# KaranSankla/Lidar_Object_Detection

Hardware: AMD Instinct MI355X
Metric: LiDAR points/sec projected+instance-labelled (higher is better)
Workload: dtype f64

## Files before the change

include/lpf.h:

```cpp
#ifndef LPF_H
#define LPF_H

#include <stddef.h>
#include <stdint.h>

#ifdef __cplusplus
extern "C" {
#endif

#define LPF_MAX_MASKS 32
#define LPF_ABI_VERSION 8
#define LPF_MAX_MASKS_WIDE 256
#define LPF_MAX_CAMS 4

typedef enum lpf_status {
    LPF_OK = 0,
    LPF_ERR_ARG = -1,
    LPF_ERR_HIP = -2,
    LPF_ERR_STATE = -3,
    LPF_ERR_NOMEM = -4,
    LPF_ERR_IO = -5
} lpf_status;

typedef struct lpf_ctx lpf_ctx;
// ... 323 lines not shown
    double  *avg_depth;
    double  *near_bbox2d;
    int32_t *front;
    double  *bbox2d;
    double  *front_avg_depth;
    int32_t *kept_pos;
    int32_t *frame_counts;
    double  *corners_velo;
    int32_t  on_device, reserved;
} lpf_box_views_outputs;
int lpf_box_views(lpf_ctx *ctx, int F, const lpf_box_views_input *in, const lpf_box_views_outputs *out);

int lpf_resize_masks_u8(lpf_ctx *ctx, const uint8_t *src, int n, int h, int w, uint8_t *dst, int on_device);

int lpf_erode_masks_u8(lpf_ctx *ctx, const uint8_t *src, int n, int h, int w, int iters, uint8_t *dst, int on_device);

int lpf_prepare_boxes(lpf_ctx *ctx, const double *corners_cam0, int nbox, const double T_cam_to_velo[16],
                      uint8_t *visible, double *corners_velo, double *bbox2d, int32_t *front);

typedef struct lpf_graph lpf_graph;
int  lpf_graph_begin(lpf_ctx *ctx);
int  lpf_graph_end(lpf_ctx *ctx, lpf_graph **out);
int  lpf_graph_launch(lpf_ctx *ctx, lpf_graph *g);
void lpf_graph_destroy(lpf_graph *g);

int lpf_profile_enable(lpf_ctx *ctx, int on);
int lpf_profile_read(lpf_ctx *ctx, double *k1_ms_sum, int64_t *k1_launches, int reset);
int lpf_profile_overhead(lpf_ctx *ctx, double *empty_bracket_ms);

int lpf_get_stats(lpf_ctx *ctx, int64_t *out, int n, int reset);

int lpf_allreduce_metrics(lpf_ctx *ctx, int64_t *vec, int n, int op, void *rccl_comm);

typedef struct lpf_first_match_input {
    const void   *masks;
    const double *colors;
    int32_t M;
    int32_t mh, mw;
    int32_t f32;
    int32_t on_device;
    int32_t reserved;
} lpf_first_match_input;
typedef struct lpf_first_match_outputs {
    int32_t *first_mask;
    int64_t *car_idx;
    int32_t *car_mask;
    float   *car_xyz;
    double  *car_rgb;
    int64_t *bg_idx;
    float   *bg_xyz;
    int64_t *n_valid, *n_car, *n_bg;
    int64_t *mask_count;
    int32_t  on_device, reserved;
} lpf_first_match_outputs;
int lpf_first_match(lpf_ctx *ctx, const float *pts, const int64_t *frame_off, int F, int pts_on_device,
                    const lpf_first_match_input *in, const lpf_first_match_outputs *out);
typedef struct lpf_first_match_rle_input {
    const lpf_rle_masks *masks;
    const double *colors;
    int32_t mh, mw;
    int32_t colors_on_device;
    int32_t reserved;
} lpf_first_match_rle_input;
int lpf_first_match_rle(lpf_ctx *ctx, const float *pts, const int64_t *frame_off, int F, int pts_on_device,
                        const lpf_first_match_rle_input *in, const lpf_first_match_outputs *out);

typedef struct lpf_reader lpf_reader;
int  lpf_reader_create(lpf_ctx *ctx, lpf_reader **out, int n_buffers, int64_t max_points);
int  lpf_reader_submit(lpf_reader *rd, const char *path);
int  lpf_reader_next(lpf_reader *rd, const float **d_pts, const float **h_pts, int64_t *n_points);
int  lpf_reader_wait(lpf_reader *rd);
void lpf_reader_destroy(lpf_reader *rd);

enum lpf_boxes_state {
    LPF_BOXES_PARSED = 0,
    LPF_BOXES_ABSENT = 1,
    LPF_BOXES_OTHER = 2,
    LPF_BOXES_NONE = 3
};
int  lpf_reader_submit_frame(lpf_reader *rd, const char *scan_path, const char *boxes_path);
int  lpf_reader_boxes(lpf_reader *rd, const double **corners_cam0, const int32_t **index, int *nbox, int *state);
int  lpf_parse_boxes_json(const char *path, double *corners_cam0, int32_t *index, int cap, int *nbox, int *state);

#ifdef __cplusplus
}
#endif
#endif
```

lidar_object_detection_amd/_build.py:

```python
import hashlib
import os
import shutil
import subprocess

_HERE = os.path.dirname(os.path.abspath(__file__))
CSRC = os.path.join(_HERE, "csrc")
LIB = os.path.join(_HERE, "liblpf.so")
LAB_LIB = os.path.join(_HERE, "liblpf_lab.so")
SOURCES = ("lpf_api.hip", "lpf_kernels.hip.h", "lpf_reader.hip.h", "lpf_wide.hip.h", "lpf_cams.hip.h", "lpf_cams_wide.hip.h",
           "lpf_frame_wide.hip.h", "lpf_depth_maps.hip.h", "lpf_depth_overlays.hip.h",
           "lpf_match2d.hip.h", "lpf_inside.hip.h", "lpf_box_points.hip.h", "lpf_box_views.hip.h", "lpf_assign.hip.h",
           "lpf_first_match.hip.h", "lpf_rle.hip.h", "lpf_ids.hip.h")
ARCH = "gfx950"

FLAGS = ["--offload-arch=" + ARCH, "-O3", "-std=c++17", "-fPIC", "-shared", "-pthread", "-ldl",
         "-ffp-contract=off", "-fno-fast-math", "-Wall", "-Wno-unused-function"]


def hipcc():
    exe = shutil.which("hipcc") or "/opt/rocm/bin/hipcc"
    if not os.path.exists(exe):
        raise RuntimeError("hipcc not found (looked on PATH and in /opt/rocm/bin)")
    return exe


HEADER = os.path.join(os.path.dirname(_HERE), "include", "lpf.h")
_MARKER = b"LPF_BUILD_ID="


def source_id(lab=False):
    h = hashlib.sha256()
    for path in [os.path.join(CSRC, s) for s in SOURCES] + [HEADER]:
        with open(path, "rb") as f:
            h.update(os.path.basename(path).encode() + b"\0" + f.read() + b"\0")
    h.update(" ".join(FLAGS + (["-DLPF_LAB"] if lab else [])).encode())
    return h.hexdigest()[:16]


def library_id(lib):
    try:
        with open(lib, "rb") as f:
            data = f.read()
    except OSError:
        return None
    i = data.find(_MARKER)
    if i < 0:
        return None
    tail = data[i + len(_MARKER):i + len(_MARKER) + 16]
    return tail.decode("ascii", "replace") if len(tail) == 16 and all(c in b"0123456789abcdef" for c in tail) else None


def needs_build(lib=None):
    lib = lib or LIB
    return library_id(lib) != source_id(lab=os.path.abspath(lib) == os.path.abspath(LAB_LIB))


def torch_lib_dir():
    try:
        import importlib.util
        spec = importlib.util.find_spec("torch")
        tl = os.path.join(os.path.dirname(spec.origin), "lib") if spec and spec.origin else None
    except Exception:
        tl = None
    return tl if tl and os.path.exists(os.path.join(tl, "libamdhip64.so")) else None


def build(force=False, verbose=False, lab=False):
    lib = LAB_LIB if lab else LIB
    if not force and not needs_build(lib):
        return lib
    work = os.path.join(_HERE, "build", "lab" if lab else "lib")
    os.makedirs(os.path.join(work, "stub"), exist_ok=True)
    obj = os.path.join(work, "lpf_api.o")
    compile_flags = [f for f in FLAGS if f not in ("-shared", "-pthread", "-ldl")]
    cmds = [[hipcc()] + compile_flags + (["-DLPF_LAB"] if lab else []) + ['-DLPF_BUILD_ID_STR="%s"' % source_id(lab),
                                                                          "-c", os.path.join(CSRC, "lpf_api.hip"), "-o", obj]]
    if verbose:
        print(" ".join(cmds[0]))
    subprocess.check_call(cmds[0], cwd=CSRC)
    undefined = subprocess.run(["nm", "-u", obj], check=True, capture_output=True, text=True).stdout.split()
    names = sorted({n for n in undefined if n.startswith(("hip", "__hip"))})
    stub_c = os.path.join(work, "stub", "stub.c")
    with open(stub_c, "w") as f:
        f.write("/* link-time stand-in for the HIP runtime: only its SONAME is recorded in liblpf.so */\n")
        f.write("".join("void %s(void) {}\n" % n for n in names))
    subprocess.check_call(["gcc", "-shared", "-fPIC", "-Wl,-soname,libamdhip64.so", stub_c, "-o", os.path.join(work, "stub", "libamdhip64.so")])
    rpath = ":".join([d for d in (torch_lib_dir(), "/opt/rocm/lib") if d])
    link = [hipcc(), "--offload-arch=" + ARCH, "-shared", "-fPIC", "-no-hip-rt", obj, "-L" + os.path.join(work, "stub"), "-lamdhip64",
            "-Wl,-rpath," + rpath, "-Wl,--disable-new-dtags", "-pthread", "-ldl", "-o", lib]
    if verbose:
        print(" ".join(link))
    subprocess.check_call(link)
    return lib


# ... 4 lines not shown
```

lidar_object_detection_amd/_native.py:

```python
import collections
import ctypes
import os
import sys
import weakref

import numpy as np

from . import _build
from .idmap import IdMasks
from .rle import RleMasks

LPF_MAX_MASKS = 32
LPF_ASSIGN_MAX = 1024
LPF_MAX_MASKS_WIDE = 256
_P = ctypes.c_void_p
_I64 = ctypes.c_int64


class LpfError(RuntimeError):

    def __init__(self, code, msg):
        super().__init__("liblpf error %d: %s" % (code, msg))
        self.code = code

# ... 212 lines not shown
    M = max([r.shape[0] for r in frames], default=0)
    sel = np.full((F, M), LPF_ID_NONE, np.int32)
    for f, r in enumerate(frames):
        sel[f, :r.shape[0]] = check_sel(r.sel, "%s: frame %d" % (who, f))
    if F == 0:
        return None, sel, 0, M, 2, False
    dts = {np.dtype(r.id_dtype) for r in frames}
    if len(dts) != 1:
        raise ValueError("%s: the frames' maps have differing ID dtypes %s: one dtype per call" % (who, sorted(d.name for d in dts)))
    dt = dts.pop()
    dev = [r.on_device for r in frames]
    if any(dev) != all(dev):
        raise ValueError("%s: host and GPU maps in one call: one place per call" % who)
    if not dev[0]:
        maps = np.ascontiguousarray(frames[0].ids[None] if F == 1 else np.stack([r.ids for r in frames]), dtype=dt)
        return maps, sel, F, M, dt.itemsize, False
    t0 = frames[0].ids
    for f, r in enumerate(frames):
        if not r.ids.is_cuda or not r.ids.is_contiguous() or r.ids.data_ptr() != t0.data_ptr() + f * H * W * dt.itemsize:
            raise ValueError("%s: GPU maps must be the frames of ONE contiguous [F,H,W] tensor (IdMasks(t[f], sel)), or F = 1: frame %d "
                             "is not where frame 0 + %d frames is" % (who, f, f))
    return [r.ids for r in frames], sel, F, M, dt.itemsize, True


def _ids_input(maps, sel, F, M, id_bytes, on_device, erode_iters):
    if F == 0:
        ptr = None
    elif on_device:
        ptr = maps[0].data_ptr()
    else:
        ptr = maps.ctypes.data
    return IdMasksInput(ptr, sel.ctypes.data if sel.size else None, F, M, id_bytes, int(erode_iters), 1 if on_device else 0, 0)


MaskForm = collections.namedtuple("MaskForm", "name cls where mixes batch struct")
MASK_FORMS = (
    MaskForm("rle", RleMasks, "the runs say where the masks are",
             "the list mixes RleMasks and arrays: one form per call (.to_dense() or RleMasks.from_dense)",
             lambda *a: LpfContext.rle_batch(*a), RleMasksInput.of),
    MaskForm("ids", IdMasks, "the map says where the masks are",
             "the list mixes IdMasks with another form of masks: one form per call (.to_dense())", ids_batch, _ids_input))


def compact_frames(masks, who, forms):
    frames = list(masks) if isinstance(masks, (list, tuple)) else [masks]
    for form in (f for name in forms for f in MASK_FORMS if f.name == name):
        if any(isinstance(m, form.cls) for m in frames):
            if not all(isinstance(m, form.cls) for m in frames):
                raise ValueError("%s: %s" % (who, form.mixes))
            return form, frames
    return None


def compact_mask_batch(masks, F, H, W, rects=None, erode_iters=0, binarize="astype", max_masks=LPF_MAX_MASKS_WIDE, who="run_wide",
                       default_binarize="astype", *, forms):
    found = compact_frames(masks, who, forms)
    if found is None:
        return None
    form, frames = found
    noun = form.cls.__name__
    if rects is not None:
        raise ValueError("%s: rects given with %s (%s)" % (who, noun, form.where))
    if binarize != default_binarize:
        raise ValueError("%s: binarize=%r with %s (a pixel is a member or it is not)" % (who, binarize, noun))
    _check_erode_iters(erode_iters)
    tables = form.batch(frames, H, W, max_masks, who)
    if tables[2] != F:
        raise ValueError("%s: %s for %d frames, the batch has %d" % (who, noun, tables[2], F))
    struct = form.struct(*tables, erode_iters)
    gpu = tables[0][0] if getattr(struct, "on_device", 0) else None
    return MaskBatch(None, tables[3], False, gpu is not None, None, form.name, struct, tables[:2], gpu)


class FrameJob(ctypes.Structure):
    _fields_ = [("pts", _P), ("n_points", _I64), ("masks", _P), ("mask_rects", _P), ("corners_cam0", _P), ("T_cam_to_velo", _P),
                ("n_masks", ctypes.c_int32), ("n_boxes", ctypes.c_int32), ("filter_visible", ctypes.c_int32), ("oriented", ctypes.c_int32),
                ("out", Outputs)]


class FrameJobWide(ctypes.Structure):
    _fields_ = [("pts", _P), ("n_points", _I64), ("masks", _P), ("mask_rects", _P), ("corners_cam0", _P), ("T_cam_to_velo", _P),
                ("n_masks", ctypes.c_int32), ("n_boxes", ctypes.c_int32), ("filter_visible", ctypes.c_int32), ("oriented", ctypes.c_int32),
                ("out", WideOutputs)]


_libs = {}


def library_path():
    env = os.environ.get("LPF_LIBRARY")
    if env:
        if os.environ.get("LPF_LAB") != "1":
            raise LpfError(-3, "LPF_LIBRARY=%s is set but this is not a lab run (LPF_LAB=1; bench.py --lab ...): refusing to load another "
                               "library in place of %s" % (env, _build.LIB))
        return env
    return _build.LIB


def _own(path):
    for lib, lab in ((_build.LIB, False), (_build.LAB_LIB, True)):
        if os.path.abspath(path) == os.path.abspath(lib):
            return lab
    return None


def load(path=None):
    path = os.path.abspath(path or library_path())
    if path in _libs:
        return _libs[path]
    lab = _own(path)
    if lab is not None and _build.needs_build(path):
        have = _build.library_id(path)
        try:
            import fcntl
            with open(path + ".lock", "w") as lk:
                fcntl.flock(lk, fcntl.LOCK_EX)
                if _build.needs_build(path):
                    _build.build(lab=lab)
        except Exception as e:
            raise LpfError(-2, "%s is %s and cannot be rebuilt here (%s): run `python -c 'import __graft_entry__ as g; g.build()'` "
                               "(hipcc --offload-arch=gfx950); there is no CPU path" % (
                                   path, "missing" if not os.path.exists(path) else "stale (built from sources %s, these are %s)" % (have, _build.source_id(lab)), e))
    if not os.path.exists(path):
        raise LpfError(-2, "%s is missing: run `python -c 'import __graft_entry__ as g; g.build()'` "
                           "(hipcc --offload-arch=gfx950); there is no CPU path" % path)
    lib = ctypes.CDLL(path)
    build_id = None
    if hasattr(lib, "lpf_build_id"):
        lib.lpf_build_id.restype = ctypes.c_char_p
        build_id = (lib.lpf_build_id() or b"").decode()
    if lab is not None and build_id != _build.source_id(lab):
        raise LpfError(-2, "%s reports build id %s, the sources beside it are %s: refusing a library that is not built from them" % (
            path, build_id, _build.source_id(lab)))
    lib._lpf_info = {"path": path, "build_id": build_id}
    if hasattr(lib, "lpf_host_alloc"):
        lib.lpf_host_alloc.restype = _P
        lib.lpf_host_alloc.argtypes = [ctypes.c_size_t]
        lib.lpf_host_free.restype = None
        lib.lpf_host_free.argtypes = [_P]
    lib.lpf_last_error.restype = ctypes.c_char_p
    lib.lpf_last_error.argtypes = [_P]
    lib.lpf_create.argtypes = [ctypes.POINTER(_P), ctypes.c_int]
    lib.lpf_destroy.argtypes = [_P]
    lib.lpf_destroy.restype = None
    lib.lpf_set_stream.argtypes = [_P, _P]
    lib.lpf_use_own_stream.argtypes = [_P]
    lib.lpf_wait_for_stream.argtypes = [_P, _P]
    lib.lpf_release_to_stream.argtypes = [_P, _P]
    lib.lpf_sync.argtypes = [_P]
    lib.lpf_set_pipelined.argtypes = [_P, ctypes.c_int]
    if hasattr(lib, "lpf_set_geometry"):
        lib.lpf_set_geometry.argtypes = [_P, ctypes.c_int]
        lib.lpf_lab_role_clock.argtypes = [_P, _P, ctypes.c_int]
        lib.lpf_lab_set_range_limits.argtypes = [_P, ctypes.c_longlong, ctypes.c_int]
        lib.lpf_lab_last_ranges.argtypes = [_P]
    lib.lpf_allreduce_metrics.argtypes = [_P, _P, ctypes.c_int, ctypes.c_int, _P]
    lib.lpf_set_camera.argtypes = [_P, _P, _P, ctypes.c_int, ctypes.c_int, ctypes.c_double, ctypes.c_double]
    lib.lpf_set_masks_u8.argtypes = [_P, _P, ctypes.c_int, ctypes.c_int, ctypes.c_int, ctypes.c_int]
    lib.lpf_set_mask_rects.argtypes = [_P, _P, ctypes.c_int, ctypes.c_int, ctypes.c_int]
    lib.lpf_set_masks_rle.argtypes = [_P, ctypes.POINTER(RleMasksInput)]
    lib.lpf_set_masks_ids.argtypes = [_P, ctypes.POINTER(IdMasksInput)]
    lib.lpf_run_wide_ids.argtypes = [_P, _P, _P, ctypes.c_int, ctypes.c_int, ctypes.POINTER(IdMasksInput), ctypes.POINTER(WideOutputs)]
    lib.lpf_set_erosion_element.argtypes = [_P, ctypes.c_int]
    lib.lpf_resize_masks_u8.argtypes = [_P, _P, ctypes.c_int, ctypes.c_int, ctypes.c_int, _P, ctypes.c_int]
    lib.lpf_erode_masks_u8.argtypes = [_P, _P, ctypes.c_int, ctypes.c_int, ctypes.c_int, ctypes.c_int, _P, ctypes.c_int]
    lib.lpf_set_masks_f32.argtypes = [_P, _P, ctypes.c_int, ctypes.c_int, ctypes.c_int, ctypes.c_int, ctypes.c_int]
    lib.lpf_set_label_image.argtypes = [_P, _P, ctypes.c_int, ctypes.c_int, ctypes.c_int]
    lib.lpf_get_label_image.argtypes = [_P, _P, ctypes.c_int]
    lib.lpf_set_boxes.argtypes = [_P, _P, _P, ctypes.c_int, ctypes.c_int]
    lib.lpf_set_boxes_ex.argtypes = [_P, _P, ctypes.c_int, _P, ctypes.c_int, ctypes.c_int]
    lib.lpf_set_boxes_cam0.argtypes = [_P, _P, ctypes.c_int, _P, ctypes.c_int, _P, ctypes.c_int, ctypes.c_int, _P, _P, _P, _P]
    lib.lpf_run.argtypes = [_P, _P, _I64, ctypes.c_int, ctypes.POINTER(Outputs)]
    lib.lpf_run_batch.argtypes = [_P, _P, _P, ctypes.c_int, ctypes.c_int, ctypes.POINTER(Outputs)]
    lib.lpf_run_frame.argtypes = [_P, ctypes.POINTER(FrameJob)]
    lib.lpf_run_frame_wide.argtypes = [_P, ctypes.POINTER(FrameJobWide)]
    lib.lpf_run_wide.argtypes = [_P, _P, _P, ctypes.c_int, ctypes.c_int, ctypes.POINTER(WideInput), ctypes.POINTER(WideOutputs)]
    lib.lpf_depth_maps.argtypes = [_P, _P, _P, ctypes.c_int, ctypes.c_int, ctypes.POINTER(WideInput), ctypes.POINTER(DepthMapsOutputs)]
    lib.lpf_depth_overlays.argtypes = [_P, ctypes.c_int, ctypes.POINTER(DepthOverlayInput), ctypes.POINTER(DepthOverlayOutputs)]
    lib.lpf_match_2d.argtypes = [_P, ctypes.c_int, ctypes.POINTER(Match2dInput), ctypes.POINTER(Match2dOutputs)]
    lib.lpf_assign_costs.argtypes = [_P, ctypes.c_int, ctypes.POINTER(AssignInput), ctypes.POINTER(AssignOutputs)]
    lib.lpf_assign_2d.argtypes = [_P, ctypes.c_int, ctypes.POINTER(Match2dInput), ctypes.POINTER(Assign2dParams), ctypes.POINTER(Assign2dOutputs)]
    lib.lpf_inside_masks.argtypes = [_P, _P, _P, ctypes.c_int, ctypes.c_int, ctypes.POINTER(InsideInput), ctypes.POINTER(InsideOutputs)]
    lib.lpf_box_points.argtypes = [_P, _P, _P, ctypes.c_int, ctypes.c_int, ctypes.POINTER(BoxPointsInput), ctypes.POINTER(BoxPointsOutputs)]
    lib.lpf_box_views.argtypes = [_P, ctypes.c_int, ctypes.POINTER(BoxViewsInput), ctypes.POINTER(BoxViewsOutputs)]
    lib.lpf_first_match.argtypes = [_P, _P, _P, ctypes.c_int, ctypes.c_int, ctypes.POINTER(FirstMatchInput), ctypes.POINTER(FirstMatchOutputs)]
    lib.lpf_depth_maps_rle.argtypes = [_P, _P, _P, ctypes.c_int, ctypes.c_int, ctypes.POINTER(RleMasksInput), ctypes.POINTER(DepthMapsOutputs)]
    lib.lpf_first_match_rle.argtypes = [_P, _P, _P, ctypes.c_int, ctypes.c_int, ctypes.POINTER(FirstMatchRleInput),
                                        ctypes.POINTER(FirstMatchOutputs)]
    lib.lpf_run_cams.argtypes = [_P, _P, _P, ctypes.c_int, ctypes.c_int, ctypes.POINTER(CamInput), ctypes.c_int, ctypes.POINTER(Outputs)]
    lib.lpf_run_cams_wide.argtypes = [_P, _P, _P, ctypes.c_int, ctypes.c_int, ctypes.POINTER(CamInput), ctypes.c_int, ctypes.POINTER(WideOutputs)]
    lib.lpf_points_in_boxes.argtypes = [_P, _P, _I64, ctypes.c_int, _P, ctypes.c_int, ctypes.c_int, _P, ctypes.c_int]
    lib.lpf_depth_image.argtypes = [_P, _P, _I64, ctypes.c_int, _P, _P]
    lib.lpf_prepare_boxes.argtypes = [_P, _P, ctypes.c_int, _P, _P, _P, _P, _P]
    lib.lpf_graph_begin.argtypes = [_P]
    lib.lpf_graph_end.argtypes = [_P, ctypes.POINTER(_P)]
    lib.lpf_graph_launch.argtypes = [_P, _P]
    lib.lpf_graph_destroy.argtypes = [_P]
    lib.lpf_graph_destroy.restype = None
    lib.lpf_get_stats.argtypes = [_P, _P, ctypes.c_int, ctypes.c_int]
    lib.lpf_profile_enable.argtypes = [_P, ctypes.c_int]
    lib.lpf_profile_read.argtypes = [_P, ctypes.POINTER(ctypes.c_double), ctypes.POINTER(_I64), ctypes.c_int]
    lib.lpf_profile_overhead.argtypes = [_P, ctypes.POINTER(ctypes.c_double)]
    lib.lpf_reader_create.argtypes = [_P, ctypes.POINTER(_P), ctypes.c_int, _I64]
    lib.lpf_reader_submit.argtypes = [_P, ctypes.c_char_p]
    lib.lpf_reader_next.argtypes = [_P, ctypes.POINTER(_P), ctypes.POINTER(_P), ctypes.POINTER(_I64)]
    lib.lpf_reader_submit_frame.argtypes = [_P, ctypes.c_char_p, ctypes.c_char_p]
    lib.lpf_reader_boxes.argtypes = [_P, ctypes.POINTER(_P), ctypes.POINTER(_P), ctypes.POINTER(ctypes.c_int), ctypes.POINTER(ctypes.c_int)]
    lib.lpf_parse_boxes_json.argtypes = [ctypes.c_char_p, _P, _P, ctypes.c_int, ctypes.POINTER(ctypes.c_int), ctypes.POINTER(ctypes.c_int)]
    lib.lpf_reader_wait.argtypes = [_P]
    lib.lpf_reader_destroy.argtypes = [_P]
    lib.lpf_reader_destroy.restype = None
    _libs[path] = lib
    return lib


EXPORTED = ("lpf_abi_version", "lpf_build_id", "lpf_host_alloc", "lpf_host_free", "lpf_create", "lpf_destroy", "lpf_last_error", "lpf_set_stream", "lpf_use_own_stream", "lpf_wait_for_stream",
            "lpf_release_to_stream", "lpf_sync",
            "lpf_set_pipelined", "lpf_allreduce_metrics",
            "lpf_set_camera", "lpf_set_masks_u8", "lpf_set_masks_f32", "lpf_set_mask_rects", "lpf_set_label_image",
            "lpf_get_label_image", "lpf_set_boxes", "lpf_set_boxes_ex", "lpf_set_boxes_cam0", "lpf_run", "lpf_run_batch", "lpf_run_frame",
            "lpf_points_in_boxes", "lpf_prepare_boxes", "lpf_depth_image", "lpf_resize_masks_u8", "lpf_erode_masks_u8", "lpf_get_stats", "lpf_profile_enable", "lpf_profile_read", "lpf_profile_overhead",
            "lpf_graph_begin", "lpf_graph_end", "lpf_graph_launch", "lpf_graph_destroy",
            "lpf_reader_create", "lpf_reader_submit", "lpf_reader_next", "lpf_reader_wait", "lpf_reader_destroy",
            "lpf_reader_submit_frame", "lpf_reader_boxes", "lpf_parse_boxes_json", "lpf_run_wide", "lpf_run_cams",
            "lpf_run_cams_wide", "lpf_run_frame_wide", "lpf_depth_maps", "lpf_depth_overlays", "lpf_match_2d",
            "lpf_inside_masks", "lpf_set_erosion_element", "lpf_box_points", "lpf_box_views", "lpf_assign_costs", "lpf_assign_2d",
            "lpf_first_match", "lpf_set_masks_rle", "lpf_depth_maps_rle", "lpf_first_match_rle", "lpf_set_masks_ids", "lpf_run_wide_ids")

BOXES_PARSED, BOXES_ABSENT, BOXES_OTHER, BOXES_NONE = 0, 1, 2, 3


def parse_boxes_file(path):
    lib = load()
    path = os.fspath(path)
    try:
        cap = os.path.getsize(path) // 64 + 1
    except OSError:
        cap = 0
    corners, index = np.empty((cap, 8, 3), np.float64), np.empty(cap, np.int32)
    n, st = ctypes.c_int(0), ctypes.c_int(0)
    rc = lib.lpf_parse_boxes_json(path.encode(), corners.ctypes.data if cap else None, index.ctypes.data if cap else None, cap,
                                  ctypes.byref(n), ctypes.byref(st))
    if rc != 0:
        raise LpfError(rc, "lpf_parse_boxes_json(%s): %d boxes, room for %d" % (path, n.value, cap))
    if st.value != BOXES_PARSED:
        return st.value, np.empty(0, np.int32), np.empty((0, 8, 3), np.float64)
    return BOXES_PARSED, index[:n.value], corners[:n.value]


def _is_torch(x):
    return type(x).__module__.startswith("torch")


def _dev_ptr(t, dtype_name=None):
    if t is None:
        return None
    if not t.is_cuda or not t.is_contiguous():
        raise ValueError("device buffers must be contiguous torch tensors on the GPU")
    if dtype_name is not None and str(t.dtype) != "torch." + dtype_name:
        raise ValueError("expected torch.%s, got %s" % (dtype_name, t.dtype))
    return t.data_ptr()


def _ptr(a):
    if a is None:
        return None
    if _is_torch(a):
        return _dev_ptr(a) if a.numel() else None
    return a.ctypes.data if a.size else None


class Scan:
    __slots__ = ("path", "n", "points", "dev_ptr", "_reader", "_ticket", "boxes_state", "box_index", "boxes_cam0")

    def __init__(self, path, n, points, dev_ptr, reader, ticket, boxes_state=BOXES_NONE, box_index=None, boxes_cam0=None):
        self.path, self.n, self.points, self.dev_ptr, self._reader, self._ticket = path, n, points, dev_ptr, reader, ticket
        self.boxes_state, self.box_index, self.boxes_cam0 = boxes_state, box_index, boxes_cam0

    def _check_live(self):
        if self._reader._ticket != self._ticket or self._reader._h is None:
            raise LpfError(-3, "this Scan's buffers were recycled (a later scan has been fetched from its reader)")


class ScanReader:

    def __init__(self, ctx, paths, n_buffers=3, max_points=1 << 21, box_paths=None):
        self._ctx, self._lib = ctx, ctx._lib
        self._h = None
        self._ticket = 0
        self._paths = [os.fspath(p) for p in paths]
        self._box_paths = None if box_paths is None else [None if b is None else os.fspath(b) for b in box_paths]
        if self._box_paths is not None and len(self._box_paths) != len(self._paths):
            raise ValueError("box_paths: one entry per scan")
        self._next_submit = 0
        self._delivered = 0
        self._depth = int(n_buffers)
        h = _P()
        ctx._check(self._lib.lpf_reader_create(ctx._h, ctypes.byref(h), int(n_buffers), int(max_points)))
        self._h = h
        ctx._readers.add(self)
        self._top_up()

    def _top_up(self):
        while self._next_submit < len(self._paths) and self._next_submit - self._delivered < self._depth:
            bp = self._box_paths[self._next_submit] if self._box_paths is not None else None
            self._ctx._check(self._lib.lpf_reader_submit_frame(self._h, self._paths[self._next_submit].encode(), bp.encode() if bp else None))
            self._next_submit += 1

    def __iter__(self):
        return self

    def __len__(self):
        return len(self._paths)

    def __next__(self):
        if self._h is None or self._delivered >= len(self._paths):
            raise StopIteration
        path = self._paths[self._delivered]
        d, hp, n = _P(), _P(), _I64(0)
        self._ticket += 1
        rc = self._lib.lpf_reader_next(self._h, ctypes.byref(d), ctypes.byref(hp), ctypes.byref(n))
        self._delivered += 1
        self._top_up()
        self._ctx._check(rc)
        cnt = int(n.value)
        if cnt:
            buf = (ctypes.c_float * (cnt * 4)).from_address(hp.value)
            pts = np.frombuffer(buf, dtype=np.float32).reshape(cnt, 4)
        else:
            pts = np.zeros((0, 4), np.float32)
        state, bidx, bcam = BOXES_NONE, None, None
        if self._box_paths is not None:
            pc, pi, nb, st = _P(), _P(), ctypes.c_int(0), ctypes.c_int(BOXES_NONE)
            self._ctx._check(self._lib.lpf_reader_boxes(self._h, ctypes.byref(pc), ctypes.byref(pi), ctypes.byref(nb), ctypes.byref(st)))
            state = int(st.value)
            if state == BOXES_PARSED:
                b = int(nb.value)
                if b:
                    bcam = np.frombuffer((ctypes.c_double * (b * 24)).from_address(pc.value), dtype=np.float64).reshape(b, 8, 3).copy()
                    bidx = np.frombuffer((ctypes.c_int32 * b).from_address(pi.value), dtype=np.int32).copy()
                else:
                    bcam, bidx = np.empty((0, 8, 3), np.float64), np.empty(0, np.int32)
        return Scan(path, cnt, pts, d.value, self, self._ticket, state, bidx, bcam)

    def wait(self):
        self._ctx._check(self._lib.lpf_reader_wait(self._h))

    def close(self):
        if self._h is not None:
            self._lib.lpf_reader_destroy(self._h)
            self._h = None

    def __enter__(self):
        return self

    def __exit__(self, *a):
        self.close()

    def __del__(self):
        try:
            self.close()
        except Exception:
            pass


class LpfContext:

    def __init__(self, device=0, library=None):
        self._lib = load(library)
        self.library = dict(self._lib._lpf_info)
        h = _P()
        rc = self._lib.lpf_create(ctypes.byref(h), int(device))
        if rc != 0:
            raise LpfError(rc, (self._lib.lpf_last_error(None) or b"").decode())
        self._h = h
        self._readers = weakref.WeakSet()
        self.device = int(device)
        self.W = self.H = 0
        self.M = 0
        self.F_masks = 0
        self.box_off = None
        self._depth = 1
        self.erosion_kernel_size = 3
        self._pin = {}
        self._lent = collections.deque(maxlen=4)

    def _check(self, rc):
        if rc != 0:
            raise LpfError(rc, (self._lib.lpf_last_error(self._h) or b"").decode())

    def close(self):
        if getattr(self, "_h", None):
            for r in list(getattr(self, "_readers", ())):
                r.close()
            self._lib.lpf_destroy(self._h)
            self._h = None
            for p, _, _ in self._pin.values():
                self._lib.lpf_host_free(p)
            self._pin = {}

    def __del__(self):
        try:
            self.close()
        except Exception:
            pass

    def __enter__(self):
        return self

    def __exit__(self, *a):
        self.close()

    def set_stream(self, stream_ptr):
        if stream_ptr is None:
            self._check(self._lib.lpf_use_own_stream(self._h))
        else:
            self._check(self._lib.lpf_set_stream(self._h, _P(int(stream_ptr))))

    def wait_for_stream(self, stream_ptr):
        self._check(self._lib.lpf_wait_for_stream(self._h, _P(int(stream_ptr))))

    def release_to_stream(self, stream_ptr):
        self._check(self._lib.lpf_release_to_stream(self._h, _P(int(stream_ptr))))

    def _call_in_order(self, device, fn, *args):
        if device is None:
            self._check(fn(self._h, *args))
            return
        import torch
        ts = torch.cuda.current_stream(device).cuda_stream
        self.wait_for_stream(ts)
        self._check(fn(self._h, *args))
        self.release_to_stream(ts)

    def sync(self):
        self._check(self._lib.lpf_sync(self._h))
        self._lent.clear()

    PIPELINED = {False: 0, 0: 0, None: 0, "off": 0, "fused": 2, 2: 2, "fused-pack": 4, 4: 4}

    def set_pipelined(self, on="fused-pack"):
        if on is True:
            raise ValueError('set_pipelined(True) meant the stream-pipelined modes 1 / 3, removed in ABI 5: use "fused" or "fused-pack"')
        if on not in self.PIPELINED:
            raise ValueError('set_pipelined: False, "fused" or "fused-pack"')
        self._check(self._lib.lpf_set_pipelined(self._h, self.PIPELINED[on]))
        self._depth = 3 if self.PIPELINED[on] else 1
        self._lent = collections.deque(self._lent, maxlen=2 * self._depth + 2)

    def set_geometry(self, mode="auto"):
        if not hasattr(self._lib, "lpf_set_geometry"):
            raise LpfError(-3, "lpf_set_geometry exists in lab builds only (python -m lidar_object_detection_amd._build lab; LPF_LIBRARY=...)")
        self._check(self._lib.lpf_set_geometry(self._h, {"auto": 0, "small": 1, "large": 2, "large-scan": 3, "small-narrow": 4, "small-1024": 5}[mode]))

    def set_range_limits(self, budget=0, max_items=0):
        if not hasattr(self._lib, "lpf_lab_set_range_limits"):
            raise LpfError(-3, "lpf_lab_set_range_limits exists in lab builds only (python -m lidar_object_detection_amd._build lab; LPF_LIBRARY=...)")
        self._check(self._lib.lpf_lab_set_range_limits(self._h, int(budget), int(max_items)))

    def last_ranges(self):
        if not hasattr(self._lib, "lpf_lab_last_ranges"):
            raise LpfError(-3, "lpf_lab_last_ranges exists in lab builds only (python -m lidar_object_detection_amd._build lab; LPF_LIBRARY=...)")
        return int(self._lib.lpf_lab_last_ranges(self._h))

    ROLES = ("summaries", "box job", "lists", "box counts", "mask pack", "project+label tiles")

    def role_clock(self, reset=True):
# ... 362 lines not shown
            raise ValueError("no frames")
        off = np.zeros(len(pts) + 1, np.int64)
        off[1:] = np.cumsum([len(p.points) if isinstance(p, Scan) else int(p.shape[0]) for p in pts])
        n = int(off[-1])
        one = pts[0] if len(pts) == 1 else None
        if isinstance(one, Scan):
            return off, (one.dev_ptr if n else None), 1, one
        if _is_torch(one):
            import torch
            self.wait_for_stream(torch.cuda.current_stream(one.device).cuda_stream)
            return off, (_dev_ptr(one, "float32") if n else None), 1, one
        pts = [p.points if isinstance(p, Scan) else p for p in pts]
        if len(pts) > 1 and n:
            try:
                import torch
                if torch.cuda.is_available():
                    batch = torch.empty((n, 4), dtype=torch.float32, device=torch.device("cuda", self.device))
                    for f, p in enumerate(pts):
                        if p.shape[0]:
                            batch[int(off[f]):int(off[f + 1])].copy_(p if _is_torch(p) else torch.from_numpy(p))
                    self.wait_for_stream(torch.cuda.current_stream(batch.device).cuda_stream)
                    return off, batch.data_ptr(), 1, batch
            except ImportError:
                pass
        host = np.concatenate([p.cpu().numpy() if _is_torch(p) else p for p in pts], axis=0) if len(pts) > 1 else pts[0]
        return off, (host.ctypes.data if n else None), 0, host

    @staticmethod
    def _until_lists_fit(launch, inst_cap, off):
        o = off.tolist()
        cap = max(max(b - a for a, b in zip(o, o[1:])), 1) if inst_cap is None else inst_cap
        while True:
            out, need = launch(cap)
            if not need:
                return out
            cap = need

    _BOXES_IN_FORCE = object()

    def _frame_results(self, off, M, summ, per_point, per_valid, iidx, cmb, box_off=_BOXES_IN_FORCE):
        if box_off is self._BOXES_IN_FORCE:
            box_off = self.box_off
        nv, nl, ic, io, bb, bc = (summ[k] for k in ("n_valid", "n_labelled", "inst_count", "inst_off", "best_box", "best_cnt"))
        res = []
        for f in range(len(off) - 1):
            a, b = int(off[f]), int(off[f + 1])
            n_valid = int(nv[f])
            r = dict(n_valid=n_valid, n_labelled=int(nl[f]), inst_count=ic[f, :M].copy(), best_box=bb[f, :M].copy(),
                     best_cnt=bc[f, :M].copy())
            for k, x in per_point.items():
                r[k] = x[a:b]
            for k, x in per_valid.items():
                r[k] = x[a:a + n_valid]
            if per_valid:
                o = io[f].tolist()
                r["inst_lists"] = [iidx[f, o[m]:o[m + 1]] for m in range(M)] if iidx is not None else []
            if box_off is not None:
                b0, b1 = int(box_off[f]), int(box_off[f + 1])
                r["count_mb"] = cmb[M * b0:M * b1].reshape(M, b1 - b0).astype(np.int64)
            else:
                r["count_mb"] = np.zeros((M, 0), np.int64)
            res.append(r)
        return res

    def stage_points(self, frames):
        return self._stage_points(frames)

    def run_batch(self, frames, want_uv=True, want_label=True, want_float=False, want_lists=True,
                  inst_cap=None, want_valid_uv=False, pinned=False, staged=None):
        off, pts_ptr, pts_dev, _keep = staged or self._stage_points(frames)
        F, n = len(off) - 1, int(off[-1])
        M = self.M if self.F_masks else 0
        Btot = int(self.box_off[-1]) if self.box_off is not None else 0
        wants = dict(want_uv=want_uv, want_label=want_label, want_float=want_float, want_lists=want_lists, want_valid_uv=want_valid_uv)

        def launch(inst_cap):
            o = Outputs()
            finish = self._host_outputs(o, "", pinned, n, F, M, Btot, inst_cap, **wants)
            self._check(self._lib.lpf_run_batch(self._h, pts_ptr, off.ctypes.data, F, pts_dev, ctypes.byref(o)))
            return finish()

        out = self._until_lists_fit(launch, inst_cap, off)
        return self._frame_results(off, M, *out)

    _PER_POINT = {"uv": None, "label_bits": "label_bits", "label_words": "label_words", "depth": "depth", "u_f": "uf", "v_f": "vf"}
    _PER_VALID = ("valid_idx", "uv_valid", "label_valid", "label_valid_words")

    def _run_outputs(self, o, table, pinned, tag, inst_cap, null_if_empty):
        a = {}
        for field, shape, dt, fill, wanted in table:
            if not wanted:
                arr = None
            elif pinned:
                arr = self._pinned(tag + field, shape, dt)
                if fill is not None:
                    arr[...] = fill
            else:
                arr = np.empty(shape, dt) if fill is None else np.full(shape, fill, dt)
            a[field] = arr
            setattr(o, field, arr.ctypes.data if (arr is not None and (arr.size or not null_if_empty)) else None)
        o.on_device, o.inst_cap = 0, inst_cap

        def finish(summ, last_off, overflow):
            per_point, per_valid = {}, {}
            for field, arr in a.items():
                if arr is None:
                    continue
                if field == "uv":
                    per_point.update(u=arr[:, 0], v=arr[:, 1])
                elif field == "uv_valid":
                    per_valid.update(uv_valid=arr, u_valid=arr[:, 0], v_valid=arr[:, 1])
                elif field in self._PER_POINT:
                    per_point[self._PER_POINT[field]] = arr
                elif field in self._PER_VALID:
                    per_valid[field] = arr
            need = int(last_off.max()) if (a["inst_idx"] is not None and overflow.any()) else 0
            return (summ, per_point, per_valid, a["inst_idx"], a["count_mb"]), need
        return a, finish

    def _host_outputs(self, o, tag, pinned, n, F, M, Btot, inst_cap, want_uv, want_label, want_float, want_lists, want_valid_uv):
        vu = want_valid_uv and want_lists
        a, finish = self._run_outputs(o, (
            ("uv", (n, 2), np.int32, None, want_uv), ("label_bits", (n,), np.uint32, None, want_label),
            ("depth", (n,), np.float64, None, want_float), ("u_f", (n,), np.float64, None, want_float),
            ("v_f", (n,), np.float64, None, want_float), ("valid_idx", (n,), np.int64, None, want_lists),
            ("uv_valid", (n, 2), np.int32, None, vu), ("label_valid", (n,), np.uint32, None, vu),
            ("inst_idx", (F, inst_cap), np.int64, None, want_lists and M), ("count_mb", (max(M * Btot, 1),), np.int32, 0, True),
            ("summary", (F,), SUMMARY_DTYPE, 0, True)), pinned, tag, inst_cap, False)
        summ = a["summary"]
        return lambda: finish(summ, summ["inst_off"][:, 32], summ["inst_overflow"])

    def _cam_inputs(self, frames, cams, max_masks, who):
        C = len(cams)
        if not 1 <= C <= LPF_MAX_CAMS:
            raise ValueError("%s takes 1 to %d cameras, got %d" % (who, LPF_MAX_CAMS, C))
        F = len(frames)
        if F == 0:
            raise ValueError("no frames")
        cin = (CamInput * C)()
        keep, Ms, box_offs = [], [], []
        for k, cam in enumerate(cams):
            W, H = int(cam["width"]), int(cam["height"])
            T = np.ascontiguousarray(cam["T_velo_to_rect"], dtype=np.float64).reshape(-1)
            K = np.asarray(cam["K"], dtype=np.float64)
            if T.size != 16 or K.ndim != 2 or K.shape[0] < 3 or K.shape[1] < 3 or W <= 0 or H <= 0:
                raise ValueError("camera %d: T_velo_to_rect must be 4x4, K at least 3x3, width and height positive" % k)
            binarize = cam.get("binarize") or ("v3" if cam.get("v3_pipeline") else "astype")
            masks = cam.get("masks")
            if masks is None:
                masks = np.zeros((F, 0, H, W), np.uint8)
            erode = cam.get("erode_iters", 0)
            batch = compact_mask_batch(masks, F, H, W, cam.get("rects"), erode, binarize, max_masks, "%s: camera %d" % (who, k),
                                       forms=("rle",)) or \
                wide_mask_batch(masks, F, H, W, cam.get("rects"), erode, binarize, self.BINARIZE)
            M = batch.M
            if M > max_masks:
                raise ValueError("camera %d has %d masks per frame: a multi-camera pass takes at most %d per camera (run_wide takes more)"
                                 % (k, M, max_masks))
            ci = cin[k]
            ci.T_velo_to_rect[:] = T.tolist()
            ci.K[:] = np.ascontiguousarray(K[:3, :3]).reshape(9).tolist()
            ci.W, ci.H = W, H
            ci.depth_min_excl, ci.depth_max_excl = float(cam.get("depth_min", 0.0)), float(cam.get("depth_max", 50.0))
            self._wide_input(ci.masks, batch, binarize, erode)
            boxes, box_off = cam.get("boxes"), None
            if boxes is not None:
# ... 894 lines not shown
```

lidar_object_detection_amd/csrc/lpf_api.hip:

```cpp
#include "lpf_kernels.hip.h"
#include "lpf_wide.hip.h"
#include "lpf_cams.hip.h"
#include "lpf_cams_wide.hip.h"
#include "lpf_frame_wide.hip.h"
#include "lpf_depth_maps.hip.h"
#include "lpf_depth_overlays.hip.h"
#include "lpf_match2d.hip.h"
#include "lpf_assign.hip.h"
#include "lpf_inside.hip.h"
#include "lpf_box_points.hip.h"
#include "lpf_box_views.hip.h"
#include "lpf_first_match.hip.h"
#include "lpf_rle.hip.h"
#include "lpf_ids.hip.h"
#include "../../include/lpf.h"

#include <algorithm>
#include <cmath>
#include <cstdarg>
#include <cstdio>
#include <cstdlib>
#include <cstring>
#include <dlfcn.h>
#include <initializer_list>
#include <mutex>
#include <string>
#include <type_traits>
#include <vector>

#define LPF_SMALL_LAUNCH (7ll << 19)
#define LPF_WIDE_BELOW 480
#define LPF_FEW_BLOCKS 64
#ifndef LPF_TAIL_SPREAD_20THS
#define LPF_TAIL_SPREAD_20THS 13
#endif

#define LPF_RECT_FUSED_TILE 1024

static_assert(sizeof(lpf_frame_summary) == LPF_SUMMARY_BYTES, "summary layout is shared with lpf_finalize_frame");

namespace {

thread_local std::string g_create_error;

struct DevBuf {
    void *p = nullptr;
    size_t cap = 0;
};

struct TileSource {
    enum Kind { NONE, PACKED, DIRECT, DIRECT_RECT } kind = NONE;
    bool f32 = false;
    int rule = 0;
    int label_bytes = 4;
    const void *img = nullptr;
    const int4 *rects = nullptr;
    bool ride_pack = false;
    bool reads_masks() const { return kind == DIRECT || kind == DIRECT_RECT; }
};

}

struct lpf_graph {
    hipGraph_t graph = nullptr;
    hipGraphExec_t exec = nullptr;
    unsigned long long generation = 0;
};

#define LPF_NSETS 4

struct lpf_ctx {
    bool capturing = false;
    unsigned long long generation = 0;
    int device = 0;
    hipStream_t stream = nullptr;
    bool own_stream = false;
    std::string err;

    bool have_camera = false;
    double T[12], K[9], dmin = 0, dmax = 0;
    int W = 0, H = 0;

    int erode_k = 3, erode_r = 1;
    uint32_t erode_spans = 0x01u;

    DevBuf mask_stage;
    DevBuf ids_stage;
    DevBuf rle_stage;
    struct RleIn {
        const lpf_rle_masks *in = nullptr;
        long long Rtot = 0;
        std::vector<int2> units;
    } rle_in[LPF_NSETS];
    struct RleSlice {
        lpf_rle_masks sub;
        std::vector<int64_t> off;
        RleIn R;
    };
    std::vector<RleSlice> rle_slices;
    struct Unpacked {
        bool valid = false;
        bool pipelined = false;
        const void *masks = nullptr;
        bool f32 = false, can_ride = false;
        int rule = 0, F = 0, M = 0;
        const int4 *rects = nullptr;
        void *label = nullptr;
    };
    struct Masks {
        int F = 0, M = 0;
        int set = 0;
        void *img = nullptr;
        int bytes = 4;
        Unpacked unpacked;
        void forget_unpacked() { unpacked = Unpacked(); }
        void drop() { F = 0; M = 0; forget_unpacked(); }
        void begin(int s) { F = 0; M = 0; img = nullptr; set = s; if (!unpacked.pipelined) forget_unpacked(); }
        void packed(int F_, int M_, void *image, int b) { F = F_; M = M_; img = image; bytes = b; }
        void left_unpacked(void *image, int b) { F = unpacked.F; M = unpacked.M; img = image; bytes = b; }
    } masks;

    struct BoxSet {
        int F = 0, oriented = 1;
        std::vector<int32_t> box_off;
        std::vector<LpfBoxFrame> h_bframes, h_bframes_dev;
        std::vector<long long> cand_off;
        size_t cand_words = 0;
        int max_words = 1;
        DevBuf boxp;
        DevBuf boxq;
        DevBuf cand;
        DevBuf corners;
        DevBuf enabled;
        DevBuf aux;
        DevBuf bframes;
        DevBuf stage;
        bool used = false;
        long long last_ref = -1;
        bool job_valid = false;
        LpfBoxJob job;
        void clear() { F = 0; box_off.clear(); job_valid = false; }
        void begin() { clear(); used = false; last_ref = -1; }
        void shaped(const int32_t *off, int F_, int oriented_) { box_off.assign(off, off + F_ + 1); F = F_; oriented = oriented_ ? 1 : 0; }
        int total() const { return F ? box_off[(size_t)F] : 0; }
        LpfBoxJob &new_job(const double *src)
        {
            memset(&job, 0, sizeof job);
            job.src = src; job.oriented = oriented; job.F = F; job.chunks = max_words;
            job.bframes = (const LpfBoxFrame *)bframes.p;
            if (F > 0) job.frame0 = h_bframes[0];
            job.boxp = (double *)boxp.p; job.boxq = (float *)boxq.p; job.cand = (unsigned long long *)cand.p;
            job.corners_keep = (double *)corners.p;
            job_valid = true;
            return job;
        }
// ... 25 lines not shown
        DevBuf vbal, mbal, seg_tab, grp_tab, frm_tab, seg_pre, cnt, mlist;
        DevBuf label_a, label_b;
        DevBuf rgrid;
        DevBuf rects;
        DevBuf out_stage;
        DevBuf tab;
        std::vector<LpfFrame> tab_frames;
        int tab_csplit = 0;
        size_t o_segs = 0, o_blks = 0, o_cblks = 0;
    } sc[LPF_NSETS];
    struct Pending {
        bool valid = false;
        LpfParams P;
        bool pre = false;
        int ntail = 0;
        int nk1 = 0;
        TileSource src;
    };
    struct Pipeline {
        bool fused = false;
        bool defer = false;
        int parity = 0;
        Pending k1, tail, fin;
        bool owes() const { return k1.valid || tail.valid || fin.valid; }
        int sets() const { return defer ? 4 : 3; }
        int depth() const { return defer ? 2 : 1; }
        int set_now() const { return fused ? parity : 0; }
        int run_set(bool run_fused) const { return run_fused ? parity : 0; }
        bool must_drain_before(const TileSource &src) const { return defer && k1.valid && src.ride_pack && (k1.src.reads_masks() || k1.src.label_bytes != src.label_bytes); }
        bool next_carries_tiles() const { return !defer || (k1.valid && k1.nk1 > 0); }
    } pipe;
    long long stats[8] = {0, 0, 0, 0, 0, 0, 0, 0};
    DevBuf resize_buf;
    const int4 *rects_pending = nullptr; int rects_F = 0, rects_M = 0;
    DevBuf lab_clk;
    long long lab_budget = 0;
    int lab_max_items = 0, lab_ranges = 0;
    int geometry = 0;

    struct PinRing { char *base = nullptr; size_t cap = 0, head = 0; hipEvent_t ev[4] = {nullptr, nullptr, nullptr, nullptr}; bool rec[4] = {false, false, false, false}; } ring;

    struct PinBack { char *p = nullptr; size_t cap = 0; } pin_back;

    DevBuf pib_box, pib_pts, pib_out, boxprep, dimg, coll;
    DevBuf st_pts;
    DevBuf out_stage;
    std::vector<LpfFrame> h_frames;
    std::vector<char> h_tab;

    struct Wide { DevBuf tab, masks, rects, rle, ids, planes_a, planes_b, flags, ccnt, cpre, fcnt, midx, mwords, mpts, cnt, pts, out; } wide;
    struct Cams { BoxSet bx[LPF_NSETS]; DevBuf label_a[LPF_NSETS], label_b[LPF_NSETS], masks[LPF_NSETS], rects[LPF_NSETS], rle[LPF_NSETS], out[LPF_NSETS], pts; } cams;
    struct CamsWide { Wide cam[LPF_NSETS]; DevBuf tab, pts; } camsw;
    struct DepthMaps { Wide pack; DevBuf foff, win, cnt, in, pts, out; } dmaps;
    struct CallBufs { DevBuf tab, pts, in, out; } dovl, m2d, insd, bpts, bviews;
    CallBufs asgn;
    struct FirstMatch : CallBufs { DevBuf code, tiles; Wide pack; } fmat;

    bool profiling = false;
    std::vector<hipEvent_t> ev;
    size_t ev_used = 0;
};

namespace {

int fail(lpf_ctx *c, int code, const char *fmt, ...)
{
    char buf[512];
    va_list ap;
    va_start(ap, fmt);
    vsnprintf(buf, sizeof buf, fmt, ap);
    va_end(ap);
    if (c) c->err = buf; else g_create_error = buf;
    if (c && c->capturing) {
        c->capturing = false;
        hipGraph_t g = nullptr;
        (void)hipStreamEndCapture(c->stream, &g);
        if (g) (void)hipGraphDestroy(g);
        (void)hipGetLastError();
        c->err += " [the graph capture in progress was abandoned]";
    }
    return code;
}

#define LPF_HIP(c, call)                                                                         \
    do {                                                                                         \
        hipError_t e_ = (call);                                                                  \
        if (e_ != hipSuccess)                                                                    \
            return fail((c), LPF_ERR_HIP, "%s failed: %s (%s:%d)", #call, hipGetErrorString(e_), \
                        __FILE__, __LINE__);                                                     \
    } while (0)

template <typename T, int RULE> struct MaskKind { typedef T elem; static constexpr int rule = RULE; };
template <typename T> struct TypeTag { typedef T type; };
template <int N> using Rows = std::integral_constant<int, N>;
template <bool B> using Flag = std::integral_constant<bool, B>;

template <typename Fn> auto with_rule(bool f32, int rule, Fn &&fn)
{
    if (!f32) return fn(MaskKind<uint8_t, 0>());
    if (rule == 1) return fn(MaskKind<float, 1>());
    if (rule == 2) return fn(MaskKind<float, 2>());
    return fn(MaskKind<float, 3>());
}

template <typename Fn> auto with_label(int bytes, Fn &&fn)
{
    if (bytes == 1) return fn(TypeTag<uint8_t>());
    if (bytes == 2) return fn(TypeTag<uint16_t>());
    return fn(TypeTag<uint32_t>());
}

template <typename Fn> auto with_flag(bool on, Fn &&fn)
{
    if (on) return fn(Flag<true>());
    return fn(Flag<false>());
}

static_assert(LPF_RECT_FUSED_TILE == 1024, "LpfDirectRect tiles are instantiated for 1024 points only");
template <bool STEP, typename Fn> void with_tile_form(const TileSource &src, int rows, bool scan_tail, Fn &&fn)
{
    auto tail = [&](auto lt, auto rw) {
        if (STEP && scan_tail) fn(lt, rw, Flag<STEP>()); else fn(lt, rw, Flag<false>());
    };
    if (src.kind == TileSource::DIRECT_RECT) {
        if (!src.f32) fn(TypeTag<LpfDirectRect<uint8_t, 0>>(), Rows<4>(), Flag<false>());
        else fn(TypeTag<LpfDirectRect<float, 1>>(), Rows<4>(), Flag<false>());
    } else if (src.kind == TileSource::DIRECT) {
        with_rule(src.f32, src.rule, [&](auto kind) { tail(TypeTag<LpfDirect<typename decltype(kind)::elem, decltype(kind)::rule>>(), Rows<2>()); });
    } else {
        with_label(src.label_bytes, [&](auto lt) {
            if (rows == 2) tail(lt, Rows<2>());
            else if (STEP && rows == 8) tail(lt, Rows<STEP ? 8 : 4>());
            else tail(lt, Rows<4>());
        });
    }
}

hipError_t host_wait(lpf_ctx *c)
{
    ++c->stats[0];
    return hipStreamSynchronize(c->stream);
}

void launch_tail(hipStream_t st, const LpfParams &P, int ntail, bool pre)
{
    if (pre) hipLaunchKernelGGL((lpf_tail_t<true>), dim3((unsigned)ntail), dim3(LPF_BLOCK), 0, st, P);
    else hipLaunchKernelGGL((lpf_tail_t<false>), dim3((unsigned)ntail), dim3(LPF_BLOCK), 0, st, P);
}

void box_job_camera(LpfBoxJob &J, const double K[9], int W, int H)
{
    memcpy(J.K, K, sizeof J.K);
    J.W = W; J.H = H;
}

int box_job_blocks(const lpf_ctx::BoxSet &B) { return B.F * B.job.chunks; }

int launch_box_job(lpf_ctx *c, lpf_ctx::BoxSet &B, const double K[9], int W, int H)
{
    if (!B.take_job()) return LPF_OK;
    box_job_camera(B.job, K, W, H);
    ++c->stats[4];
    hipLaunchKernelGGL(lpf_box_job_kernel, dim3((unsigned)box_job_blocks(B)), dim3(LPF_BLOCK), 0, c->stream, B.job);
    LPF_HIP(c, hipGetLastError());
    return LPF_OK;
}
// ... 405 lines not shown
        for (int k = 0; k < 3; ++k) {
            double a = c[k], b = c[k];
            for (int j = 1; j < 8; ++j) {
                const double w = c[3 * j + k];
                if (w < a) a = w;
                if (w > b) b = w;
            }
            o[k] = a; o[3 + k] = b;
        }
    }
}

int box_shape(lpf_ctx *c, lpf_ctx::BoxSet &B, const int32_t *box_off, int F, int oriented);

int box_layout(lpf_ctx *c, const int32_t *box_off, int F, int oriented, const char *who, lpf_ctx::BoxSet **out)
{
    if (F < 0 || (F > 0 && !box_off)) return fail(c, LPF_ERR_ARG, "%s: F=%d box_off=%p", who, F, (const void *)box_off);
    if (F > 0 && box_off[0] != 0) return fail(c, LPF_ERR_ARG, "%s: box_off[0] must be 0", who);
    for (int f = 0; f < F; ++f)
        if (box_off[f + 1] < box_off[f]) return fail(c, LPF_ERR_ARG, "%s: box_off not ascending at %d", who, f);
    if (!c->have_camera) return fail(c, LPF_ERR_STATE, "%s: lpf_set_camera must be called first (cam-0 boxes are filtered with its K, W, H)", who);
    int rc;
    bool owed;
    lpf_ctx::BoxSet *B = &c->boxes.set_for_write(c->pipe.fused, c->pipe.depth(), &owed);
    if (owed && (rc = flush_pending(c))) return rc;
    if ((rc = box_shape(c, *B, box_off, F, oriented))) return rc;
    *out = B;
    return LPF_OK;
}

int box_shape(lpf_ctx *c, lpf_ctx::BoxSet &BS, const int32_t *box_off, int F, int oriented)
{
    int rc;
    lpf_ctx::BoxSet *B = &BS;
    B->begin();
    B->h_bframes.resize((size_t)F);
    B->cand_off.assign((size_t)F, 0);
    B->max_words = 1;
    size_t total = 0;
    for (int f = 0; f < F; ++f) {
        const int nb = box_off[f + 1] - box_off[f];
        B->h_bframes[f].box_off = box_off[f]; B->h_bframes[f].B = nb; B->h_bframes[f].cand_off = (long long)total;
        B->cand_off[f] = (long long)total;
        total += (size_t)LPF_GRID_WORDS * (size_t)((nb + 63) / 64);
        if ((nb + 63) / 64 > B->max_words) B->max_words = (nb + 63) / 64;
    }
    const int Btot = F ? box_off[F] : 0;
    const size_t nb = (size_t)(Btot ? Btot : 1);
    if ((rc = reserve(c, B->boxp, nb * 16 * sizeof(double)))) return rc;
    if ((rc = reserve(c, B->boxq, nb * 8 * sizeof(float)))) return rc;
    if ((rc = reserve(c, B->cand, (total ? total : 1) * 8))) return rc;
    if ((rc = reserve(c, B->corners, nb * 24 * sizeof(double)))) return rc;
    if ((rc = reserve(c, B->enabled, nb))) return rc;
    if (F > 1) {
        if ((rc = reserve(c, B->bframes, (size_t)F * sizeof(LpfBoxFrame)))) return rc;
        if (B->h_bframes_dev.size() != B->h_bframes.size() ||
            memcmp(B->h_bframes_dev.data(), B->h_bframes.data(), (size_t)F * sizeof(LpfBoxFrame)) != 0) {
            if ((rc = upload(c, B->bframes.p, B->h_bframes.data(), (size_t)F * sizeof(LpfBoxFrame)))) return rc;
            B->h_bframes_dev = B->h_bframes;
            ++c->generation;
        }
    }
    B->cand_words = total;
    B->shaped(box_off, F, oriented);
    return LPF_OK;
}

int stage_corners(lpf_ctx *c, lpf_ctx::BoxSet &B, const double *corners, int on_device, size_t nb, const double **src)
{
    int rc;
    *src = corners;
    if (on_device == 2) return LPF_OK;
    if ((rc = reserve(c, B.stage, nb * 192))) return rc;
    if (on_device) LPF_HIP(c, hipMemcpyAsync(B.stage.p, corners, nb * 192, hipMemcpyDeviceToDevice, c->stream));
    else if ((rc = upload(c, B.stage.p, corners, nb * 192))) return rc;
    *src = (const double *)B.stage.p;
    return LPF_OK;
}

int set_boxes_impl(lpf_ctx *c, const double *corners, int on_device, const int32_t *box_off, int F, int oriented, bool cam0, const double *Tcv,
                   int filter_visible, uint8_t *visible, double *corners_velo, double *bbox2d, int32_t *front, const char *who)
{
    if (!c) return LPF_ERR_ARG;
    if (use_device(c)) return LPF_ERR_HIP;
    if (on_device < 0 || on_device > 2) return fail(c, LPF_ERR_ARG, "%s: on_device=%d (0 host, 1 device, 2 device and lent)", who, on_device);
    if (F == 0) { c->boxes.in_force().clear(); return LPF_OK; }
    if (cam0 && !Tcv) return fail(c, LPF_ERR_ARG, "%s: T_cam_to_velo is NULL", who);
    if (box_off && F > 0 && box_off[F] > 0 && !corners) return fail(c, LPF_ERR_ARG, "%s: corners is NULL", who);
    int rc;
    lpf_ctx::BoxSet *B = nullptr;
    if ((rc = box_layout(c, box_off, F, oriented, who, &B))) return rc;
    const int Btot = box_off[F];
    if (Btot == 0) return LPF_OK;
    const size_t nb = (size_t)Btot;
    const double *src;
    if ((rc = stage_corners(c, *B, corners, on_device, nb, &src))) { B->clear(); return rc; }
    const bool host_out = !on_device && (visible || corners_velo || bbox2d || front);
    if (host_out && (rc = reserve(c, B->aux, nb * 36))) { B->clear(); return rc; }
    LpfBoxJob &J = B->new_job(src);
    J.filter_visible = filter_visible ? 1 : 0;
    if (cam0) {
        J.cam0 = 1;
        memcpy(J.Tcv, Tcv, sizeof J.Tcv);
        J.enabled_out = (uint8_t *)B->enabled.p;
        if (on_device) { J.visible = visible; J.corners_out = corners_velo; J.bbox2d = bbox2d; J.front = front; }
        else if (host_out) { J.bbox2d = (double *)B->aux.p; J.front = (int32_t *)((char *)B->aux.p + nb * 32); }
    }
    if (host_out && (rc = launch_box_job(c, *B))) return rc;
    if (host_out) {
        if (visible) LPF_HIP(c, hipMemcpyAsync(visible, B->enabled.p, nb, hipMemcpyDeviceToHost, c->stream));
        if (corners_velo) LPF_HIP(c, hipMemcpyAsync(corners_velo, B->corners.p, nb * 192, hipMemcpyDeviceToHost, c->stream));
        if (bbox2d) LPF_HIP(c, hipMemcpyAsync(bbox2d, B->aux.p, nb * 32, hipMemcpyDeviceToHost, c->stream));
        if (front) LPF_HIP(c, hipMemcpyAsync(front, (char *)B->aux.p + nb * 32, nb * 4, hipMemcpyDeviceToHost, c->stream));
        LPF_HIP(c, host_wait(c));
    }
    return LPF_OK;
}

struct Erosion { int iters; bool element; };
Erosion erosion(const lpf_ctx *c, int iters)
{
    if (c->erode_k == 1) iters = 0;
    return Erosion{iters, iters > 0 && c->erode_k != 3};
}

template <typename LT> int erode_packed_iters(lpf_ctx *c, LT *&cur, DevBuf &lb_, const int W, const int H, const int F, hipStream_t ms, int left, bool element)
{
    if (left <= 0) return LPF_OK;
    int rc;
    if ((rc = reserve(c, lb_, (size_t)F * H * W * 4))) return rc;
    const dim3 grid((W + LPF_TW - 1) / LPF_TW, (H + LPF_TH - 1) / LPF_TH, F);
    LT *other = (LT *)lb_.p;
    for (int it = 0; it < left; ++it) {
        if (element) hipLaunchKernelGGL((lpf_erode_packed_k<LT>), grid, dim3(LPF_BLOCK), 0, ms, cur, other, H, W, c->erode_r, c->erode_spans);
        else hipLaunchKernelGGL((lpf_erode_packed<LT>), grid, dim3(LPF_BLOCK), 0, ms, cur, other, H, W);
        LPF_HIP(c, hipGetLastError());
        LT *t = cur; cur = other; other = t;
    }
    return LPF_OK;
}

int pack_masks(lpf_ctx *c, DevBuf &la, DevBuf &lb_, const int W, const int H, hipStream_t ms, const void *masks, bool f32, int rule,
               int label_bytes, int F, int M, int erode_iters, void **result, const int4 *rects = nullptr)
{
    return with_label(label_bytes, [&](auto lt) -> int {
        typedef typename decltype(lt)::type LT;
        const size_t hw = (size_t)H * W;
        dim3 grid((W + LPF_TW - 1) / LPF_TW, (H + LPF_TH - 1) / LPF_TH, F);
        LT *cur = (LT *)la.p;
        int rc;
        if (M == 0) {
            LPF_HIP(c, hipMemsetAsync(cur, 0, (size_t)F * hw * sizeof(LT), ms));
        } else {
            const Erosion E = erosion(c, erode_iters);
            int left = E.iters;
            const bool stream16 = !E.element && hw % 16 == 0 && ((uintptr_t)masks & 15) == 0;
            if (!stream16 && E.iters > 0) --left;
            with_rule(f32, rule, [&](auto kind) {
                typedef typename decltype(kind)::elem T;
                constexpr int RULE = decltype(kind)::rule;
                const int4 *r = RULE <= 1 ? rects : nullptr;
                if (stream16) {
                    const long long total16 = (long long)F * (long long)(hw / 16);
                    const unsigned nb = (unsigned)((total16 + LPF_BLOCK - 1) / LPF_BLOCK);
                    hipLaunchKernelGGL((lpf_pack16<T, RULE, LT>), dim3(nb), dim3(LPF_BLOCK), 0, ms, (const T *)masks, cur, M, (long long)hw, total16, r, W);
                } else if (E.element) {
                    hipLaunchKernelGGL((lpf_pack_erode_k<T, RULE, LT>), grid, dim3(LPF_BLOCK), 0, ms, (const T *)masks, cur, M, H, W, c->erode_r, c->erode_spans);
                } else {
                    hipLaunchKernelGGL((lpf_pack_erode<T, RULE, LT>), grid, dim3(LPF_BLOCK), 0, ms, (const T *)masks, cur, M, H, W, E.iters > 0 ? 1 : 0, r);
                }
            });
            LPF_HIP(c, hipGetLastError());
            if ((rc = erode_packed_iters(c, cur, lb_, W, H, F, ms, left, E.element))) return rc;
        }
        *result = cur;
        return LPF_OK;
    });
}

int too_many_masks(lpf_ctx *c, int M)
{
    return fail(c, LPF_ERR_ARG, "set_masks: M=%d masks per frame, a run takes at most LPF_MAX_MASKS = %d (one bit each in label_bits): run the frame "
                                "once per group of %d masks -- everything per point is the same in every pass (pipeline.run_frames does so)",
                M, LPF_MAX_MASKS, LPF_MAX_MASKS);
}

template <typename T>
int set_masks_impl(lpf_ctx *c, const T *masks, int F, int M, int mode, int erode_iters, int on_device)
{
    if (!c) return LPF_ERR_ARG;
    if (use_device(c)) return LPF_ERR_HIP;
    if (!c->have_camera) return fail(c, LPF_ERR_STATE, "lpf_set_camera must be called before masks (W, H)");
    if (M > LPF_MAX_MASKS) return too_many_masks(c, M);
    if (F < 0 || M < 0 || erode_iters < 0 || (F > 0 && M > 0 && !masks))
        return fail(c, LPF_ERR_ARG, "set_masks: F=%d M=%d erode_iters=%d masks=%p", F, M, erode_iters, (const void *)masks);
    const bool per_set = c->pipe.fused && on_device;
    int rc;
    if (!per_set && c->pipe.owes() && (rc = sync_all(c))) return rc;
    lpf_ctx::Masks &MK = c->masks;
    lpf_ctx::Scratch &S = c->sc[c->pipe.set_now()];
    MK.begin(c->pipe.set_now());
    if (F == 0) return LPF_OK;
    const size_t hw = (size_t)c->H * c->W;
    if ((rc = reserve(c, S.label_a, (size_t)F * hw * 4))) return rc;
    const T *d_masks = masks;
    if (M > 0 && !on_device) {
        const size_t bytes = (size_t)F * M * hw * sizeof(T);
        if ((rc = reserve(c, c->mask_stage, bytes))) return rc;
        LPF_HIP(c, hipMemcpyAsync(c->mask_stage.p, masks, bytes, hipMemcpyHostToDevice, c->stream));
        d_masks = (const T *)c->mask_stage.p;
    }
    const int lb = (M <= 8) ? 1 : (M <= 16) ? 2 : 4;
    const int4 *rects = (((sizeof(T) == 1 && mode == 0) || (sizeof(T) == 4 && mode == 1)) && erode_iters == 0 && c->rects_F == F && c->rects_M == M &&
                         c->W >= 16) ? c->rects_pending : nullptr;
    c->rects_pending = nullptr;
    MK.forget_unpacked();
    const bool lent_pipelined = per_set && on_device == 2, kept_serial = !c->pipe.fused && on_device != 1;
    if (M > 0 && erode_iters == 0 && (lent_pipelined || kept_serial)) {
        lpf_ctx::Unpacked &U = MK.unpacked;
        U.valid = true; U.pipelined = lent_pipelined; U.masks = d_masks; U.f32 = sizeof(T) == 4; U.rule = mode; U.F = F; U.M = M;
        U.rects = rects; U.label = S.label_a.p;
        U.can_ride = lent_pipelined && c->pipe.defer && sizeof(T) == 1 && hw % 16 == 0 && ((uintptr_t)d_masks & 15) == 0;
        if (!on_device) LPF_HIP(c, host_wait(c));
        MK.left_unpacked(lent_pipelined ? S.label_a.p : nullptr, lb);
        return LPF_OK;
    }
    void *cur = nullptr;
    if ((rc = pack_masks(c, S.label_a, S.label_b, c->W, c->H, c->stream, d_masks, sizeof(T) == 4, mode, lb, F, M, erode_iters, &cur, rects))) return rc;
    if (!on_device) LPF_HIP(c, host_wait(c));
    MK.packed(F, M, cur, lb);
    return LPF_OK;
}

int pack_unpacked(lpf_ctx *c)
{
    lpf_ctx::Masks &MK = c->masks;
    const lpf_ctx::Unpacked &U = MK.unpacked;
    if (!U.valid) return LPF_OK;
    lpf_ctx::Scratch &S = c->sc[MK.set];
    void *cur = nullptr;
    int rc = pack_masks(c, S.label_a, S.label_b, c->W, c->H, c->stream, U.masks, U.f32, U.rule, MK.bytes, U.F, U.M, 0, &cur, U.rects);
    if (rc) return rc;
    MK.packed(MK.F, MK.M, cur, MK.bytes);
    MK.forget_unpacked();
    return LPF_OK;
}

int plan_tile_source(lpf_ctx *c, bool fused, bool small, bool sparse_frames, int M, TileSource &src)
{
    src = TileSource();
    int rc;
    const lpf_ctx::Masks &MK = c->masks;
    const lpf_ctx::Unpacked &U = MK.unpacked;
    const bool readable = U.valid && U.pipelined == fused && M > 0 && sparse_frames;
    if (readable && !small && U.rects && ((!U.f32 && U.rule == 0) || (U.f32 && U.rule == 1))) src.kind = TileSource::DIRECT_RECT;
    else if (readable && small) src.kind = TileSource::DIRECT;
    else {
        src.ride_pack = U.valid && U.pipelined && fused && U.can_ride && M > 0;
        if (!src.ride_pack && (rc = pack_unpacked(c))) return rc;
        if (M > 0) src.kind = TileSource::PACKED;
    }
    if (M > 0 && fused && MK.set != c->pipe.run_set(fused))
        return fail(c, LPF_ERR_STATE, "the masks were set for another scratch set: in the pipelined modes the label images rotate with the scratch sets -- call lpf_set_masks_* before every lpf_run* (and after switching modes)");
    if (src.reads_masks()) {
        src.f32 = U.f32; src.rule = U.rule; src.img = U.masks;
        src.rects = U.rects;
    } else if (M > 0) {
        src.img = MK.img;
    }
    if (M > 0 && !src.img) return fail(c, LPF_ERR_STATE, "no masks for this run's scratch set: in the pipelined modes the label images rotate with the scratch sets -- call lpf_set_masks_* before every lpf_run* (and after switching modes)");
    src.label_bytes = (M > 0) ? MK.bytes : 4;
    return LPF_OK;
}
// ... 570 lines not shown
    }
    if (o.summary) memcpy(o.summary, hs, (size_t)P.F * sizeof(lpf_frame_summary));
    return LPF_OK;
}

int wide_frames(const int64_t *frame_off, int F, const lpf_ctx::BoxSet &BX, LpfWideFrame *fr, int *nbw)
{
    int nchunk = 0, maxB = 0;
    for (int f = 0; f < F; ++f) {
        LpfWideFrame &e = fr[f];
        e.pt_off = frame_off[f];
        e.N = (int)(frame_off[f + 1] - frame_off[f]);
        e.chunk_off = nchunk;
        e.nchunk = (e.N + LPF_WIDE_CHUNK - 1) / LPF_WIDE_CHUNK;
        e.box_off = BX.F ? BX.box_off[f] : 0;
        e.B = BX.F ? BX.box_off[f + 1] - BX.box_off[f] : 0;
        e.pad = 0;
        nchunk += e.nchunk;
        maxB = std::max(maxB, e.B);
    }
    *nbw = (maxB + 63) / 64;
    return nchunk;
}

void wide_params(LpfWideParams &W, const Cam &cam, int F, int M, int nchunk, int nbw, const lpf_ctx::BoxSet &BX, long long inst_cap,
                 const LpfWideFrame *frames)
{
    memset(&W, 0, sizeof W);
    set_cam(W.cam, cam);
    W.F = F; W.M = M; W.LW = (M + 31) / 32; W.nchunk = nchunk; W.nbw = nbw;
    W.oriented = BX.F ? BX.oriented : 1; W.inst_cap = inst_cap;
    W.frames = frames;
    W.boxp = (const double *)BX.boxp.p; W.boxq = (const float *)BX.boxq.p;
}

}

extern "C" {

int lpf_abi_version(void) { return LPF_ABI_VERSION; }

#ifndef LPF_BUILD_ID_STR
#define LPF_BUILD_ID_STR "unknown"
#endif
static const char lpf_build_marker[] = "LPF_BUILD_ID=" LPF_BUILD_ID_STR;
const char *lpf_build_id(void) { return lpf_build_marker + 13; }

void *lpf_host_alloc(size_t bytes)
{
    void *p = nullptr;
    const hipError_t e = hipHostMalloc(&p, bytes ? bytes : 1, hipHostMallocDefault);
    if (e != hipSuccess) { fail(nullptr, LPF_ERR_NOMEM, "lpf_host_alloc(%zu): %s", bytes, hipGetErrorString(e)); return nullptr; }
    return p;
}

void lpf_host_free(void *p) { if (p) (void)hipHostFree(p); }

int lpf_create(lpf_ctx **out, int device_id)
{
    if (!out) return fail(nullptr, LPF_ERR_ARG, "lpf_create: out is NULL");
    *out = nullptr;
    int n = 0;
    hipError_t e = hipGetDeviceCount(&n);
    if (e != hipSuccess || n <= 0)
        return fail(nullptr, LPF_ERR_HIP, "no HIP device: %s", e == hipSuccess ? "device count is 0" : hipGetErrorString(e));
    if (device_id < 0 || device_id >= n) return fail(nullptr, LPF_ERR_ARG, "device_id %d out of range [0,%d)", device_id, n);
    lpf_ctx *c = new (std::nothrow) lpf_ctx();
    if (!c) return fail(nullptr, LPF_ERR_NOMEM, "out of host memory");
    c->device = device_id;
    if ((e = hipSetDevice(device_id)) != hipSuccess || (e = hipStreamCreateWithFlags(&c->stream, hipStreamNonBlocking)) != hipSuccess) {
        fail(nullptr, LPF_ERR_HIP, "stream creation failed: %s", hipGetErrorString(e));
        delete c;
        return LPF_ERR_HIP;
    }
    c->own_stream = true;
    *out = c;
    return LPF_OK;
}

void lpf_destroy(lpf_ctx *c)
{
    if (!c) return;
    (void)hipSetDevice(c->device);
    (void)hipStreamSynchronize(c->stream);
    for (auto &S : c->sc) {
        DevBuf *sb[] = {&S.vbal, &S.mbal, &S.seg_tab, &S.grp_tab, &S.frm_tab, &S.seg_pre, &S.cnt, &S.mlist, &S.label_a, &S.label_b, &S.tab, &S.rects, &S.rgrid, &S.out_stage};
        for (DevBuf *b : sb) release(*b);
    }
    for (auto *ring : {c->boxes.ring, c->cams.bx})
        for (int k = 0; k < LPF_NSETS; ++k) {
            lpf_ctx::BoxSet &B = ring[k];
            DevBuf *bb[] = {&B.boxp, &B.boxq, &B.cand, &B.corners, &B.enabled, &B.aux, &B.bframes, &B.stage};
            for (DevBuf *b : bb) release(*b);
        }
    for (int k = 0; k < LPF_NSETS; ++k) {
        DevBuf *cb[] = {&c->cams.label_a[k], &c->cams.label_b[k], &c->cams.masks[k], &c->cams.rects[k], &c->cams.rle[k], &c->cams.out[k]};
        for (DevBuf *b : cb) release(*b);
    }
    release(c->cams.pts);
    for (lpf_ctx::Wide *D : {&c->wide, &c->camsw.cam[0], &c->camsw.cam[1], &c->camsw.cam[2], &c->camsw.cam[3]}) {
        DevBuf *wb[] = {&D->tab, &D->masks, &D->rects, &D->rle, &D->ids, &D->planes_a, &D->planes_b, &D->flags, &D->ccnt, &D->cpre, &D->fcnt, &D->midx, &D->mwords,
                        &D->mpts, &D->cnt, &D->pts, &D->out};
        for (DevBuf *b : wb) release(*b);
    }
    release(c->camsw.tab);
    release(c->camsw.pts);
    for (DevBuf *b : {&c->dmaps.pack.planes_a, &c->dmaps.pack.planes_b, &c->dmaps.pack.rle, &c->fmat.pack.planes_a, &c->fmat.pack.planes_b,
                      &c->fmat.pack.rle, &c->dmaps.foff, &c->dmaps.win, &c->dmaps.cnt, &c->dmaps.in,
                      &c->dmaps.pts, &c->dmaps.out})
        release(*b);
    for (lpf_ctx::CallBufs *D : {&c->dovl, &c->m2d, &c->insd, &c->bpts, &c->bviews, &c->asgn, (lpf_ctx::CallBufs *)&c->fmat})
        for (DevBuf *b : {&D->tab, &D->pts, &D->in, &D->out}) release(*b);
    release(c->fmat.code);
    release(c->fmat.tiles);
    DevBuf *all[] = {&c->resize_buf, &c->lab_clk, &c->mask_stage, &c->rle_stage, &c->ids_stage, &c->pib_box, &c->pib_pts, &c->pib_out, &c->boxprep, &c->dimg, &c->coll, &c->st_pts, &c->out_stage};
    for (DevBuf *b : all) release(*b);
    for (hipEvent_t e : c->ev) (void)hipEventDestroy(e);
    for (hipEvent_t e : c->ring.ev) if (e) (void)hipEventDestroy(e);
    if (c->ring.base) (void)hipHostFree(c->ring.base);
    if (c->pin_back.p) (void)hipHostFree(c->pin_back.p);
    if (c->own_stream) (void)hipStreamDestroy(c->stream);
    delete c;
}

const char *lpf_last_error(const lpf_ctx *c) { return c ? c->err.c_str() : g_create_error.c_str(); }

int lpf_set_stream(lpf_ctx *c, void *s)
{
    if (!c) return LPF_ERR_ARG;
    if (use_device(c)) return LPF_ERR_HIP;
    { int rc_ = sync_all(c); if (rc_) return rc_; }
    if (c->own_stream) { (void)hipStreamDestroy(c->stream); c->own_stream = false; }
    c->stream = (hipStream_t)s;
    ++c->generation;
    return LPF_OK;
}

int lpf_use_own_stream(lpf_ctx *c)
{
    if (!c) return LPF_ERR_ARG;
    if (use_device(c)) return LPF_ERR_HIP;
    { int rc_ = sync_all(c); if (rc_) return rc_; }
    if (c->own_stream) return LPF_OK;
    c->stream = nullptr;
    LPF_HIP(c, hipStreamCreateWithFlags(&c->stream, hipStreamNonBlocking));
    c->own_stream = true;
    ++c->generation;
    return LPF_OK;
}

int lpf_wait_for_stream(lpf_ctx *c, void *producer)
{
    if (!c) return LPF_ERR_ARG;
    if (use_device(c)) return LPF_ERR_HIP;
    if (c->capturing) return fail(c, LPF_ERR_STATE, "lpf_wait_for_stream inside graph capture");
    if ((hipStream_t)producer == c->stream) return LPF_OK;
    hipEvent_t e;
    LPF_HIP(c, hipEventCreateWithFlags(&e, hipEventDisableTiming));
    hipError_t r = hipEventRecord(e, (hipStream_t)producer);
    if (r == hipSuccess) r = hipStreamWaitEvent(c->stream, e, 0);
    (void)hipEventDestroy(e);
    if (r != hipSuccess) return fail(c, LPF_ERR_HIP, "lpf_wait_for_stream: %s", hipGetErrorString(r));
    return LPF_OK;
}

int lpf_release_to_stream(lpf_ctx *c, void *consumer)
{
    if (!c) return LPF_ERR_ARG;
    if (use_device(c)) return LPF_ERR_HIP;
    if (c->capturing) return fail(c, LPF_ERR_STATE, "lpf_release_to_stream inside graph capture");
    { int rc_ = flush_pending(c); if (rc_) return rc_; }
    if (c->stream == (hipStream_t)consumer) return LPF_OK;
    hipEvent_t e;
    LPF_HIP(c, hipEventCreateWithFlags(&e, hipEventDisableTiming));
    hipError_t r = hipEventRecord(e, c->stream);
    if (r == hipSuccess) r = hipStreamWaitEvent((hipStream_t)consumer, e, 0);
    (void)hipEventDestroy(e);
    if (r != hipSuccess) return fail(c, LPF_ERR_HIP, "lpf_release_to_stream: %s", hipGetErrorString(r));
    return LPF_OK;
}

int lpf_sync(lpf_ctx *c)
{
    if (!c) return LPF_ERR_ARG;
    if (use_device(c)) return LPF_ERR_HIP;
    return sync_all(c);
}

#ifdef LPF_LAB
int lpf_set_geometry(lpf_ctx *c, int mode)
{
    if (!c) return LPF_ERR_ARG;
    if (mode < 0 || mode > 5) return fail(c, LPF_ERR_ARG, "lpf_set_geometry: mode=%d (0 by launch size, 1 small with the wide tail, 2 large, 3 large with scan-kernel prefixes, 4 small with the narrow tail, 5 small with 1024-point tiles)", mode);
    c->geometry = mode;
    ++c->generation;
    return LPF_OK;
}

int lpf_lab_role_clock(lpf_ctx *c, unsigned long long *out, int reset)
{
    if (!c) return LPF_ERR_ARG;
    if (use_device(c)) return LPF_ERR_HIP;
    int rc = sync_all(c);
    if (rc) return rc;
    unsigned long long init[30];
    for (int r = 0; r < 6; ++r) { init[5 * r] = ~0ull; init[5 * r + 1] = init[5 * r + 2] = init[5 * r + 3] = init[5 * r + 4] = 0ull; }
    if (!c->lab_clk.p) {
        if ((rc = reserve(c, c->lab_clk, sizeof init))) return rc;
        if (hipMemcpy(c->lab_clk.p, init, sizeof init, hipMemcpyHostToDevice) != hipSuccess) return fail(c, LPF_ERR_HIP, "lpf_lab_role_clock: hipMemcpy");
    }
    if (out && hipMemcpy(out, c->lab_clk.p, sizeof init, hipMemcpyDeviceToHost) != hipSuccess) return fail(c, LPF_ERR_HIP, "lpf_lab_role_clock: hipMemcpy");
    if (reset && hipMemcpy(c->lab_clk.p, init, sizeof init, hipMemcpyHostToDevice) != hipSuccess) return fail(c, LPF_ERR_HIP, "lpf_lab_role_clock: hipMemcpy");
    return LPF_OK;
}

int lpf_lab_set_range_limits(lpf_ctx *c, long long stage_budget_bytes, int max_items)
{
    if (!c) return LPF_ERR_ARG;
    if (stage_budget_bytes < 0 || max_items < 0)
        return fail(c, LPF_ERR_ARG, "lpf_lab_set_range_limits: stage_budget_bytes=%lld max_items=%d (neither may be negative; 0 = the product's value)", stage_budget_bytes, max_items);
    c->lab_budget = stage_budget_bytes;
    c->lab_max_items = max_items;
    return LPF_OK;
}

int lpf_lab_last_ranges(lpf_ctx *c) { return c ? c->lab_ranges : LPF_ERR_ARG; }
#endif

int lpf_set_mask_rects(lpf_ctx *c, const int32_t *rects, int on_device, int F, int M)
{
    if (!c) return LPF_ERR_ARG;
    c->rects_pending = nullptr; c->rects_F = 0; c->rects_M = 0;
    if (!rects || F <= 0 || M <= 0) return LPF_OK;
    if (M > LPF_MAX_MASKS) return fail(c, LPF_ERR_ARG, "lpf_set_mask_rects: M=%d (at most %d)", M, LPF_MAX_MASKS);
    if (use_device(c)) return LPF_ERR_HIP;
    const size_t bytes = (size_t)F * M * sizeof(int4);
    if (on_device) {
        if (((uintptr_t)rects & 15) != 0) return fail(c, LPF_ERR_ARG, "lpf_set_mask_rects: the device array must be 16-byte aligned");
        c->rects_pending = (const int4 *)rects;
    } else {
        if (c->capturing) return LPF_OK;
        DevBuf &rb = c->sc[c->pipe.set_now()].rects;
        int rc = reserve(c, rb, bytes);
        if (rc) return rc;
        if ((rc = upload(c, rb.p, rects, bytes))) return rc;
        c->rects_pending = (const int4 *)rb.p;
    }
    c->rects_F = F; c->rects_M = M;
    return LPF_OK;
}

static const uint8_t LPF_ELLIPSE_DX[8][8] = {{0}, {1, 0}, {2, 2, 0}, {3, 3, 2, 0}, {4, 4, 3, 3, 0}, {5, 5, 5, 4, 3, 0}, {6, 6, 6, 5, 4, 3, 0},
                                             {7, 7, 7, 6, 6, 5, 4, 0}};
int lpf_set_erosion_element(lpf_ctx *c, int ksize)
{
    if (!c) return LPF_ERR_ARG;
    if (ksize < 1 || ksize > 15 || ksize % 2 == 0)
        return fail(c, LPF_ERR_ARG, "lpf_set_erosion_element: ksize=%d (the k x k MORPH_ELLIPSE for odd k, 1 .. 15)", ksize);
    const int r = ksize / 2;
    uint32_t spans = 0;
    for (int j = 0; j <= r; ++j) spans |= (uint32_t)LPF_ELLIPSE_DX[r][j] << (4 * j);
    c->erode_k = ksize; c->erode_r = r; c->erode_spans = spans;
    return LPF_OK;
}

int lpf_set_pipelined(lpf_ctx *c, int on)
{
    if (!c) return LPF_ERR_ARG;
    if (use_device(c)) return LPF_ERR_HIP;
    if (on == 1 || on == 3)
        return fail(c, LPF_ERR_ARG, "lpf_set_pipelined: modes 1 and 3 (tail kernels / mask pack on side streams) were removed in ABI 5 -- "
                                    "they measured slower than 2 and 4 on every workload (DESIGN.md section 8); use 2 or 4");
    if (on != 0 && on != 2 && on != 4) return fail(c, LPF_ERR_ARG, "lpf_set_pipelined: mode %d (0 off, 2 the tail rides in the next run's launch, "
                                                                   "4 = 2 + the mask pack rides as well)", on);
    int rc = sync_all(c);
    if (rc) return rc;
    if ((rc = pack_unpacked(c))) return rc;
    c->pipe.fused = on != 0;
    c->pipe.defer = on == 4;
    c->pipe.parity = 0;
    if (c->masks.F && c->masks.set != 0) c->masks.drop();
    ++c->generation;
    return LPF_OK;
}

int lpf_set_camera(lpf_ctx *c, const double T[16], const double K[9], int W, int H, double dmin, double dmax)
{
    if (!c) return LPF_ERR_ARG;
    if (!T || !K || W <= 0 || H <= 0 || (long long)W * H > (1ll << 30))
        return fail(c, LPF_ERR_ARG, "set_camera: T=%p K=%p W=%d H=%d", (const void *)T, (const void *)K, W, H);
    if (!c->capturing && (c->pipe.owes() || c->boxes.in_force().job_valid)) {
        if (use_device(c)) return LPF_ERR_HIP;
        int rc_ = sync_all(c);
        if (rc_) return rc_;
    }
    if (W != c->W || H != c->H) {
        c->masks.drop();
        c->boxes.drop();
    }
    memcpy(c->T, T, sizeof c->T);
    memcpy(c->K, K, sizeof c->K);
    c->W = W; c->H = H; c->dmin = dmin; c->dmax = dmax;
    c->have_camera = true;
    ++c->generation;
    return LPF_OK;
}

int lpf_set_masks_u8(lpf_ctx *c, const uint8_t *masks, int F, int M, int erode_iters, int on_device)
{
    return set_masks_impl<uint8_t>(c, masks, F, M, 0, erode_iters, on_device);
}

int lpf_set_masks_f32(lpf_ctx *c, const float *masks, int F, int M, int binarize, int erode_iters, int on_device)
{
    if (c && (binarize < 0 || binarize > 2)) return fail(c, LPF_ERR_ARG, "lpf_set_masks_f32: binarize=%d (0, 1 or 2)", binarize);
    return set_masks_impl<float>(c, masks, F, M, binarize + 1, erode_iters, on_device);
}

int lpf_set_masks_rle(lpf_ctx *c, const lpf_rle_masks *in)
{
    if (!c) return LPF_ERR_ARG;
    if (use_device(c)) return LPF_ERR_HIP;
    if (!c->have_camera) return fail(c, LPF_ERR_STATE, "lpf_set_camera must be called before masks (W, H)");
    if (c->capturing)
        return fail(c, LPF_ERR_STATE, "lpf_set_masks_rle cannot be captured into a graph (the run counts size its launch: call it outside "
                                      "lpf_graph_begin ... lpf_graph_end)");
    if (!in) return fail(c, LPF_ERR_ARG, "lpf_set_masks_rle: in=NULL");
    if (in->M > LPF_MAX_MASKS) return too_many_masks(c, in->M);
    RleCall R(c);
    int rc;
    if ((rc = R.walk("lpf_set_masks_rle", in, c->W, c->H))) return rc;
    return set_masks_compact(c, in->F, in->M, [&](lpf_ctx::Scratch &S, int lb, void **cur, bool *host_in) {
        return rle_label_image(c, S.label_a, S.label_b, c->rle_stage, R.A, c->W, c->H, lb, cur, host_in);
    });
}

int lpf_set_masks_ids(lpf_ctx *c, const lpf_id_masks *in)
{
    if (!c) return LPF_ERR_ARG;
    if (use_device(c)) return LPF_ERR_HIP;
    if (!c->have_camera) return fail(c, LPF_ERR_STATE, "lpf_set_camera must be called before masks (W, H)");
    if (c->capturing)
        return fail(c, LPF_ERR_STATE, "lpf_set_masks_ids cannot be captured into a graph (the table of selected IDs is a host copy: call it "
                                      "outside lpf_graph_begin ... lpf_graph_end)");
    if (!in) return fail(c, LPF_ERR_ARG, "lpf_set_masks_ids: in=NULL");
    if (in->M > LPF_MAX_MASKS) return too_many_masks(c, in->M);
    int rc;
    if ((rc = check_ids(c, "lpf_set_masks_ids", in, (size_t)c->W * c->H))) return rc;
    return set_masks_compact(c, in->F, in->M, [&](lpf_ctx::Scratch &S, int lb, void **cur, bool *host_in) {
        return ids_label_image(c, S.label_a, S.label_b, c->ids_stage, in, c->W, c->H, lb, cur, host_in);
    });
}

int lpf_set_label_image(lpf_ctx *c, const uint32_t *label, int F, int M, int on_device)
{
    if (!c) return LPF_ERR_ARG;
    if (use_device(c)) return LPF_ERR_HIP;
    if (!c->have_camera) return fail(c, LPF_ERR_STATE, "lpf_set_camera must be called first");
    if (F < 0 || M < 0 || M > LPF_MAX_MASKS || (F > 0 && !label)) return fail(c, LPF_ERR_ARG, "set_label_image: F=%d M=%d", F, M);
    int rc;
    if ((rc = sync_all(c))) return rc;
    lpf_ctx::Scratch &S = c->sc[c->pipe.set_now()];
    c->masks.begin(c->pipe.set_now());
    if (F == 0) return LPF_OK;
    const size_t bytes = (size_t)F * c->H * c->W * 4;
    if ((rc = reserve(c, S.label_a, bytes))) return rc;
    LPF_HIP(c, hipMemcpyAsync(S.label_a.p, label, bytes, on_device ? hipMemcpyDeviceToDevice : hipMemcpyHostToDevice, c->stream));
    LPF_HIP(c, host_wait(c));
    c->masks.packed(F, M, S.label_a.p, 4);
    return LPF_OK;
}

int lpf_get_label_image(lpf_ctx *c, uint32_t *out, int on_device)
{
    if (!c || !out) return LPF_ERR_ARG;
    if (use_device(c)) return LPF_ERR_HIP;
    { int rc_ = sync_all(c); if (rc_) return rc_; }
    { int rc_ = pack_unpacked(c); if (rc_) return rc_; }
    const lpf_ctx::Masks &MK = c->masks;
    if (!MK.img || !MK.F) return fail(c, LPF_ERR_STATE, "no masks set");
    const size_t npix = (size_t)MK.F * c->H * c->W;
    if (MK.bytes == 4) {
        LPF_HIP(c, hipMemcpyAsync(out, MK.img, npix * 4, on_device ? hipMemcpyDeviceToDevice : hipMemcpyDeviceToHost, c->stream));
        LPF_HIP(c, host_wait(c));
        return LPF_OK;
    }
    std::vector<uint8_t> raw(npix * (size_t)MK.bytes);
    LPF_HIP(c, hipMemcpyAsync(raw.data(), MK.img, raw.size(), hipMemcpyDeviceToHost, c->stream));
    LPF_HIP(c, host_wait(c));
    std::vector<uint32_t> wide(npix);
    for (size_t i = 0; i < npix; ++i)
        wide[i] = MK.bytes == 1 ? (uint32_t)raw[i] : (uint32_t)reinterpret_cast<const uint16_t *>(raw.data())[i];
    LPF_HIP(c, hipMemcpyAsync(out, wide.data(), npix * 4, on_device ? hipMemcpyHostToDevice : hipMemcpyHostToHost, c->stream));
    LPF_HIP(c, host_wait(c));
    return LPF_OK;
}

int lpf_set_boxes(lpf_ctx *c, const double *corners, const int32_t *box_off, int F, int oriented)
{
    return lpf_set_boxes_ex(c, corners, 0, box_off, F, oriented);
}

int lpf_set_boxes_ex(lpf_ctx *c, const double *corners, int on_device, const int32_t *box_off, int F, int oriented)
{
    return set_boxes_impl(c, corners, on_device, box_off, F, oriented, false, nullptr, 0, nullptr, nullptr, nullptr, nullptr, "set_boxes");
}

int lpf_set_boxes_cam0(lpf_ctx *c, const double *corners_cam0, int on_device, const int32_t *box_off, int F, const double Tcv[16],
                       int filter_visible, int oriented, uint8_t *visible, double *corners_velo, double *bbox2d, int32_t *front)
{
    return set_boxes_impl(c, corners_cam0, on_device, box_off, F, oriented, true, Tcv, filter_visible, visible, corners_velo, bbox2d, front,
                          "set_boxes_cam0");
}

int lpf_run_batch(lpf_ctx *c, const float *pts, const int64_t *frame_off, int F, int pts_on_device, const lpf_outputs *out)
{
    if (!c) return LPF_ERR_ARG;
    if (use_device(c)) return LPF_ERR_HIP;
    if (!c->have_camera) return fail(c, LPF_ERR_STATE, "lpf_set_camera has not been called");
    if (!out || !frame_off || F <= 0) return fail(c, LPF_ERR_ARG, "run: out=%p frame_off=%p F=%d", (const void *)out, (const void *)frame_off, F);
    int rc;
    if ((rc = check_frames(c, "run", pts, frame_off, F, LPF_SEG_QUANTUM))) return rc;
    const int64_t Ntot = frame_off[F];
    lpf_ctx::BoxSet &BX = c->boxes.in_force();
    if (c->masks.F != 0 && c->masks.F != F) return fail(c, LPF_ERR_STATE, "masks were set for %d frames, run has %d", c->masks.F, F);
    if (BX.F != 0 && BX.F != F) return fail(c, LPF_ERR_STATE, "boxes were set for %d frames, run has %d", BX.F, F);
    if (out->inst_idx && out->inst_cap <= 0) return fail(c, LPF_ERR_ARG, "run: inst_idx given with inst_cap=%lld", (long long)out->inst_cap);
    if ((out->uv_valid || out->label_valid) && !out->valid_idx)
        return fail(c, LPF_ERR_ARG, "run: uv_valid / label_valid need valid_idx as well (they share its order)");
    const int M = c->masks.F ? c->masks.M : 0;
    const int Btot = BX.total();
    const bool host_io = !out->on_device;

    const bool small = c->geometry == 1 || c->geometry == 4 || c->geometry == 5 || (c->geometry == 0 && Ntot <= LPF_SMALL_LAUNCH);
    NarrowLayout L;
    narrow_layout(c, frame_off, F, BX, out->inst_cap, small, L);
    const bool fused = c->pipe.fused && !host_io && pts_on_device;
    L.split(fused && L.few ? 4 : 1);
    if (c->geometry == 3) L.pre_scan = true;
    if (!fused && c->pipe.owes() && (rc = sync_all(c))) return rc;
    lpf_ctx::Scratch &S = c->sc[c->pipe.run_set(fused)];
    if ((rc = narrow_reserve(c, S, L, M, Btot))) return rc;
    if ((rc = narrow_tables(c, S, L, false))) return rc;
    LpfParams P;
    narrow_params(P, c, ctx_cam(c), L, S, BX, M, out->inst_cap);
    const bool sparse_frames = Ntot * 2 <= (int64_t)F * c->W * c->H;
    TileSource src;
    if ((rc = plan_tile_source(c, fused, small, sparse_frames, M, src))) return rc;
    P.label_img = src.img;
    P.rects = src.rects;
    LpfRectJob RG;
    memset(&RG, 0, sizeof RG);
    const bool rect_tiles = src.kind == TileSource::DIRECT_RECT;
    if (rect_tiles) {
        RG.rects = P.rects; RG.F = F; RG.M = M;
        RG.cw = (c->W + LPF_RG_CELL - 1) / LPF_RG_CELL; RG.ch = (c->H + LPF_RG_CELL - 1) / LPF_RG_CELL;
        RG.cells = RG.cw * RG.ch; RG.bpf = (RG.cells + LPF_BLOCK - 1) / LPF_BLOCK;
        if ((rc = reserve(c, S.rgrid, (size_t)F * RG.cells * sizeof(uint32_t)))) return rc;
        RG.grid = (uint32_t *)S.rgrid.p;
        P.rect_grid = RG.grid; P.rg_cw = RG.cw; P.rg_cells = RG.cells;
    }

    const size_t n = (size_t)Ntot;
    if (pts_on_device) {
        P.pts = (const float4 *)pts;
    } else {
        if ((rc = reserve(c, c->st_pts, n * 16))) return rc;
        if (n) LPF_HIP(c, hipMemcpyAsync(c->st_pts.p, pts, n * 16, hipMemcpyHostToDevice, c->stream));
        P.pts = (const float4 *)c->st_pts.p;
    }
    if ((rc = narrow_bind(c, fused ? S.out_stage : c->out_stage, *out, n, F, M, Btot, P))) return rc;
    if (M > 0) {
        if ((rc = reserve(c, S.mlist, n * 16))) return rc;
        P.mlist = (float4 *)S.mlist.p;
    }

    c->boxes.claimed_by_run();

    const bool small_1024 = small && src.kind != TileSource::DIRECT && (c->geometry == 5 || (c->geometry == 0 && Ntot > 1792ll * 512));
    P.tile_pts = small ? (small_1024 ? 1024 : 512) : 1024;
    if (fused && !small) P.tile_pts = rect_tiles ? LPF_RECT_FUSED_TILE : 2048;
    const int nk1 = L.nseg_total * (int)(L.seg_pts / P.tile_pts);
    const bool want_lists = out->valid_idx || out->inst_idx;
    const int ntail = (P.count_boxes ? L.ncblk : 0) + (want_lists ? L.nblk : 0);
    hipEvent_t e0 = nullptr, e1 = nullptr;
    if (fused && c->pipe.must_drain_before(src) && (rc = flush_pending(c))) return rc;
    const bool tiles_wait = fused && c->pipe.defer;
    if (rect_tiles && nk1 > 0 && !tiles_wait) {
        hipLaunchKernelGGL(lpf_rect_grid_kernel, dim3((unsigned)(RG.F * RG.bpf)), dim3(LPF_BLOCK), 0, c->stream, RG);
        LPF_HIP(c, hipGetLastError());
    }
    const bool carries_k1 = fused ? c->pipe.next_carries_tiles() : nk1 > 0;
    if (carries_k1 && c->profiling && c->ev_used < (1u << 16)) {
        if (c->ev.size() < 2 * (c->ev_used + 1)) {
            hipEvent_t a, b;
            LPF_HIP(c, hipEventCreate(&a));
            LPF_HIP(c, hipEventCreate(&b));
            c->ev.push_back(a); c->ev.push_back(b);
        }
        e0 = c->ev[2 * c->ev_used]; e1 = c->ev[2 * c->ev_used + 1];
        ++c->ev_used;
        LPF_HIP(c, hipEventRecord(e0, c->stream));
    }
    if (fused) {
        const lpf_ctx::Pending cur = pending_run(P, L.pre_scan, ntail, nk1, src);
        if ((rc = queue_step(c, &cur, &BX, e1, (rect_tiles && tiles_wait) ? &RG : nullptr))) return rc;
        c->masks.forget_unpacked();
        c->pipe.parity = (c->pipe.parity + 1) % c->pipe.sets();
        return LPF_OK;
    }
    if (BX.job_ready() && nk1 > 0) {
        const lpf_ctx::Pending cur = pending_run(P, false, 0, nk1, src);
        lpf_ctx::Pending none;
        if ((rc = launch_step(c, cur, none, none, nullptr, &BX, e1))) return rc;
    } else {
    if ((rc = launch_box_job(c, BX))) return rc;
    if (nk1 > 0) {
        const dim3 g1((unsigned)nk1);
        with_tile_form<false>(src, P.tile_pts >> 8, false, [&](auto lt, auto rw, auto) {
            hipLaunchKernelGGL((lpf_k1_project_t<decltype(rw)::value, LPF_K1_FLAGS, typename decltype(lt)::type>), g1, dim3(LPF_BLOCK), 0, c->stream, P);
        });
        LPF_HIP(c, hipGetLastError());
        if (e1) LPF_HIP(c, hipEventRecord(e1, c->stream));
    }
    }
    if (L.pre_scan && L.nseg_total > 0) {
        hipLaunchKernelGGL(lpf_scan_segments, dim3(F), dim3(LPF_BLOCK), 0, c->stream, P);
        LPF_HIP(c, hipGetLastError());
    }
    if (ntail > 0) {
        if (small && P.count_boxes && c->geometry != 4 && (L.nblk <= LPF_WIDE_BELOW || c->geometry == 1)) {
            if (L.pre_scan) hipLaunchKernelGGL((lpf_tail_wide_t<true>), dim3((unsigned)ntail), dim3(64 * LPF_WIDE_WAVES), 0, c->stream, P);
            else hipLaunchKernelGGL((lpf_tail_wide_t<false>), dim3((unsigned)ntail), dim3(64 * LPF_WIDE_WAVES), 0, c->stream, P);
        } else {
            launch_tail(c->stream, P, ntail, L.pre_scan);
        }
        LPF_HIP(c, hipGetLastError());
    }
    hipLaunchKernelGGL(lpf_finalize, dim3(F), dim3(LPF_BLOCK), 0, c->stream, P);
    LPF_HIP(c, hipGetLastError());

    if (host_io) {
        std::vector<lpf_frame_summary> hs((size_t)F);
        bool lists = false;
        if ((rc = narrow_back_a(c, *out, P, n, M * Btot, hs.data(), &lists))) return rc;
        LPF_HIP(c, host_wait(c));
        if (lists) {
            if ((rc = narrow_back_b(c, *out, P, frame_off, hs.data()))) return rc;
            LPF_HIP(c, host_wait(c));
        }
    }
    return LPF_OK;
}

int lpf_points_in_boxes(lpf_ctx *c, const float *pts, int64_t k, int stride, const double *corners, int B, int oriented,
                        uint8_t *inside, int on_device)
{
    if (!c) return LPF_ERR_ARG;
    if (use_device(c)) return LPF_ERR_HIP;
    if (k < 0 || B < 0 || (stride != 3 && stride != 4) || (k > 0 && !pts) || (B > 0 && !corners) || (k > 0 && B > 0 && !inside))
        return fail(c, LPF_ERR_ARG, "points_in_boxes: k=%lld B=%d stride=%d", (long long)k, B, stride);
    if (k == 0 || B == 0) return LPF_OK;
    std::vector<double> bp((size_t)B * 16);
    for (int b = 0; b < B; ++b) box_params(corners + (size_t)b * 24, oriented, bp.data() + (size_t)b * 16);
    int rc;
    if ((rc = reserve(c, c->pib_box, bp.size() * 8))) return rc;
    LPF_HIP(c, hipMemcpyAsync(c->pib_box.p, bp.data(), bp.size() * 8, hipMemcpyHostToDevice, c->stream));
    const float *d_pts = pts;
    uint8_t *d_out = inside;
    if (!on_device) {
        if ((rc = reserve(c, c->pib_pts, (size_t)k * stride * 4))) return rc;
        if ((rc = reserve(c, c->pib_out, (size_t)k * B))) return rc;
        LPF_HIP(c, hipMemcpyAsync(c->pib_pts.p, pts, (size_t)k * stride * 4, hipMemcpyHostToDevice, c->stream));
        d_pts = (const float *)c->pib_pts.p; d_out = (uint8_t *)c->pib_out.p;
    }
    hipLaunchKernelGGL(lpf_points_in_boxes_kernel, dim3((unsigned)((k + LPF_BLOCK - 1) / LPF_BLOCK)), dim3(LPF_BLOCK), 0, c->stream,
                       d_pts, (long long)k, stride, (const double *)c->pib_box.p, B, oriented ? 1 : 0, d_out);
    LPF_HIP(c, hipGetLastError());
    if (!on_device) LPF_HIP(c, hipMemcpyAsync(inside, d_out, (size_t)k * B, hipMemcpyDeviceToHost, c->stream));
    LPF_HIP(c, host_wait(c));
    return LPF_OK;
}

static void resize_table(int n_dst, int n_src, bool clamp, std::vector<int4> &tab)
{
    tab.resize((size_t)n_dst);
    volatile double ratio = (double)n_dst / (double)n_src;
    volatile double scale = 1.0 / ratio;
    for (int d = 0; d < n_dst; ++d) {
        volatile double a = ((double)d + 0.5) * scale;
        volatile double b = a - 0.5;
        volatile float f = (float)b;
        int s = (int)floorf(f);
        volatile float fr = f - (float)s;
        if (clamp && s < 0) { s = 0; fr = 0.f; }
        if (clamp && s >= n_src - 1) { s = n_src - 1; fr = 0.f; }
        volatile float one_minus = 1.0f - fr;
        volatile float p0 = one_minus * 2048.0f, p1 = fr * 2048.0f;
        long w0 = lrintf(p0), w1 = lrintf(p1);
        w0 = w0 < -32768 ? -32768 : w0 > 32767 ? 32767 : w0;
        w1 = w1 < -32768 ? -32768 : w1 > 32767 ? 32767 : w1;
        const int s0 = s < 0 ? 0 : s > n_src - 1 ? n_src - 1 : s, s1 = s + 1 < 0 ? 0 : s + 1 > n_src - 1 ? n_src - 1 : s + 1;
        tab[(size_t)d] = make_int4(s0, s1, (int)w0, (int)w1);
    }
}

int lpf_resize_masks_u8(lpf_ctx *c, const uint8_t *src, int n, int h, int w, uint8_t *dst, int on_device)
{
    if (!c) return LPF_ERR_ARG;
    if (use_device(c)) return LPF_ERR_HIP;
    if (!c->have_camera) return fail(c, LPF_ERR_STATE, "lpf_set_camera has not been called (the target size is the camera's)");
    if (n < 0 || h <= 0 || w <= 0 || (n > 0 && (!src || !dst)) || (long long)h * w > 0x7fffffffll || (long long)n * h * w > (1ll << 36) ||
        (long long)n * c->W * c->H > (1ll << 36))
        return fail(c, LPF_ERR_ARG, "resize_masks: n=%d h=%d w=%d src=%p dst=%p (a plane of at most 2^31 - 1 pixels -- the kernel indexes it with "
                                    "32-bit arithmetic -- and at most 2^36 pixels in all, in and out)", n, h, w, (const void *)src, (void *)dst);
    if (n == 0) return LPF_OK;
    const int W = c->W, H = c->H;
    const bool area2 = w == 2 * W && h == 2 * H;
    const size_t in_bytes = (size_t)n * h * w, out_bytes = (size_t)n * H * W;
    int rc;
    if (c->capturing) return fail(c, LPF_ERR_STATE, "resize_masks inside a graph capture");
    if (c->pipe.owes() && (rc = sync_all(c))) return rc;
    const uint8_t *dS = src;
    uint8_t *dD = dst;
    const bool linear = !area2 && !(h == H && w == W);
    std::vector<int4> xt, yt;
    const size_t tab_bytes = ((size_t)W + (size_t)H) * sizeof(int4);
    if ((rc = reserve(c, c->resize_buf, tab_bytes + (on_device ? 0 : in_bytes + out_bytes)))) return rc;
// ... 71 lines not shown
    if (!c) return LPF_ERR_ARG;
    if (use_device(c)) return LPF_ERR_HIP;
    if (!c->have_camera) return fail(c, LPF_ERR_STATE, "lpf_set_camera has not been called");
    if (N < 0 || N > 0x7ffffff0ll || (N > 0 && !pts) || !depth_img) return fail(c, LPF_ERR_ARG, "depth_image: N=%lld", (long long)N);
    const size_t hw = (size_t)c->W * c->H;
    int rc;
    if ((rc = reserve(c, c->dimg, hw * 12))) return rc;
    double *dD = on_device ? depth_img : (double *)c->dimg.p;
    unsigned *dW = (unsigned *)((char *)c->dimg.p + hw * 8);
    const float *dP = pts;
    if (!on_device && N > 0) {
        if ((rc = reserve(c, c->st_pts, (size_t)N * 16))) return rc;
        LPF_HIP(c, hipMemcpyAsync(c->st_pts.p, pts, (size_t)N * 16, hipMemcpyHostToDevice, c->stream));
        dP = (const float *)c->st_pts.p;
    }
    LPF_HIP(c, hipMemsetAsync(dD, 0, hw * 8, c->stream));
    LPF_HIP(c, hipMemsetAsync(dW, 0, hw * 4, c->stream));
    if (N > 0) {
        LpfCam P;
        set_cam(P, ctx_cam(c));
        const dim3 g((unsigned)((N + LPF_BLOCK - 1) / LPF_BLOCK));
        hipLaunchKernelGGL((lpf_depth_image_kernel<0>), g, dim3(LPF_BLOCK), 0, c->stream, P, (const float4 *)dP, (int)N, dW, dD);
        hipLaunchKernelGGL((lpf_depth_image_kernel<1>), g, dim3(LPF_BLOCK), 0, c->stream, P, (const float4 *)dP, (int)N, dW, dD);
        LPF_HIP(c, hipGetLastError());
    }
    if (!on_device) {
        LPF_HIP(c, hipMemcpyAsync(depth_img, dD, hw * 8, hipMemcpyDeviceToHost, c->stream));
        if (winner) {
            LPF_HIP(c, hipMemcpyAsync(winner, dW, hw * 4, hipMemcpyDeviceToHost, c->stream));
            LPF_HIP(c, host_wait(c));
            for (size_t i = 0; i < hw; ++i) winner[i] -= 1;
            return LPF_OK;
        }
        LPF_HIP(c, host_wait(c));
    } else if (winner) {
        return fail(c, LPF_ERR_ARG, "depth_image: the winner image is only returned to host callers");
    }
    return LPF_OK;
}

int lpf_prepare_boxes(lpf_ctx *c, const double *corners_cam0, int nbox, const double Tcv[16], uint8_t *visible, double *corners_velo,
                      double *bbox2d, int32_t *front)
{
    if (!c) return LPF_ERR_ARG;
    if (use_device(c)) return LPF_ERR_HIP;
    if (!c->have_camera) return fail(c, LPF_ERR_STATE, "lpf_set_camera has not been called");
    if (nbox < 0 || (nbox > 0 && (!corners_cam0 || !Tcv))) return fail(c, LPF_ERR_ARG, "prepare_boxes: nbox=%d", nbox);
    if (nbox == 0) return LPF_OK;
    const size_t nb = (size_t)nbox;
    const size_t o_in = 0, o_cv = o_in + nb * 192, o_bb = o_cv + nb * 192, o_fr = o_bb + nb * 32, o_vis = o_fr + nb * 4, total = o_vis + nb;
    int rc;
    if (c->capturing) return fail(c, LPF_ERR_STATE, "prepare_boxes inside a graph capture");
    if ((rc = reserve(c, c->boxprep, total))) return rc;
    char *base = (char *)c->boxprep.p;
    if ((rc = upload(c, base + o_in, corners_cam0, nb * 192))) return rc;
    const size_t back = total - o_cv;
    if (c->pin_back.cap < back) {
        if (c->pin_back.p) { LPF_HIP(c, hipStreamSynchronize(c->stream)); (void)hipHostFree(c->pin_back.p); c->pin_back.p = nullptr; c->pin_back.cap = 0; }
        const size_t cap = back + back / 2 + 4096;
        LPF_HIP(c, hipHostMalloc((void **)&c->pin_back.p, cap, hipHostMallocDefault));
        c->pin_back.cap = cap;
    }
    LpfBoxPrep A;
    memcpy(A.Tcv, Tcv, sizeof A.Tcv);
    memcpy(A.K, c->K, sizeof A.K);
    A.W = c->W; A.H = c->H;
    hipLaunchKernelGGL(lpf_box_prep_kernel, dim3((unsigned)((nb * 8 + LPF_BLOCK - 1) / LPF_BLOCK)), dim3(LPF_BLOCK), 0, c->stream, A,
                       (const double *)(base + o_in), nbox, (uint8_t *)(base + o_vis), (double *)(base + o_cv), (double *)(base + o_bb),
                       (int *)(base + o_fr));
    LPF_HIP(c, hipGetLastError());
    LPF_HIP(c, hipMemcpyAsync(c->pin_back.p, base + o_cv, back, hipMemcpyDeviceToHost, c->stream));
    LPF_HIP(c, host_wait(c));
    const char *h = c->pin_back.p - o_cv;
    if (visible) memcpy(visible, h + o_vis, nb);
    if (corners_velo) memcpy(corners_velo, h + o_cv, nb * 192);
    if (bbox2d) memcpy(bbox2d, h + o_bb, nb * 32);
    if (front) memcpy(front, h + o_fr, nb * 4);
    return LPF_OK;
}

int lpf_graph_begin(lpf_ctx *c)
{
    if (!c) return LPF_ERR_ARG;
    if (use_device(c)) return LPF_ERR_HIP;
    if (c->pipe.fused) return fail(c, LPF_ERR_STATE, "graph capture needs pipelining off");
    if (c->capturing) return fail(c, LPF_ERR_STATE, "already capturing");
    int rc = sync_all(c);
    if (rc) return rc;
    LPF_HIP(c, hipStreamBeginCapture(c->stream, hipStreamCaptureModeThreadLocal));
    c->capturing = true;
    return LPF_OK;
}

int lpf_graph_end(lpf_ctx *c, lpf_graph **out)
{
    if (!c || !out) return LPF_ERR_ARG;
    if (use_device(c)) return LPF_ERR_HIP;
    if (!c->capturing) return fail(c, LPF_ERR_STATE, "lpf_graph_end without lpf_graph_begin");
    { int rc_ = launch_box_job(c, c->boxes.in_force()); if (rc_) return rc_; }
    c->capturing = false;
    lpf_graph *g = new (std::nothrow) lpf_graph();
    if (!g) return fail(c, LPF_ERR_NOMEM, "out of host memory");
    hipError_t e = hipStreamEndCapture(c->stream, &g->graph);
    if (e == hipSuccess) e = hipGraphInstantiate(&g->exec, g->graph, nullptr, nullptr, 0);
    if (e != hipSuccess) {
        if (g->graph) (void)hipGraphDestroy(g->graph);
        delete g;
        return fail(c, LPF_ERR_HIP, "graph capture failed: %s (a call inside the capture allocated, copied from pageable memory or synchronised?)",
                    hipGetErrorString(e));
    }
    g->generation = c->generation;
    *out = g;
    return LPF_OK;
}

int lpf_graph_launch(lpf_ctx *c, lpf_graph *g)
{
    if (!c || !g || !g->exec) return LPF_ERR_ARG;
    if (use_device(c)) return LPF_ERR_HIP;
    if (g->generation != c->generation)
        return fail(c, LPF_ERR_STATE, "lpf_graph_launch: the graph is stale -- since its capture the context changed geometry, boxes, camera, "
                                      "stream or mode, or regrew a buffer the graph points into; capture it again");
    LPF_HIP(c, hipGraphLaunch(g->exec, c->stream));
    return LPF_OK;
}

void lpf_graph_destroy(lpf_graph *g)
{
    if (!g) return;
    if (g->exec) (void)hipGraphExecDestroy(g->exec);
    if (g->graph) (void)hipGraphDestroy(g->graph);
    delete g;
}

int lpf_get_stats(lpf_ctx *c, int64_t *out, int n, int reset)
{
    if (!c || (n > 0 && !out) || n < 0) return LPF_ERR_ARG;
    for (int i = 0; i < n; ++i) out[i] = i < 8 ? (int64_t)c->stats[i] : 0;
    if (reset) for (long long &v : c->stats) v = 0;
    return LPF_OK;
}

int lpf_profile_enable(lpf_ctx *c, int on)
{
    if (!c) return LPF_ERR_ARG;
    c->profiling = on != 0;
    return LPF_OK;
}

int lpf_allreduce_metrics(lpf_ctx *c, int64_t *vec, int n, int op, void *rccl_comm)
{
    if (!c) return LPF_ERR_ARG;
    if (use_device(c)) return LPF_ERR_HIP;
    if (!vec || n <= 0 || n > (1 << 20) || op < 0 || op > 2 || !rccl_comm)
        return fail(c, LPF_ERR_ARG, "allreduce_metrics: vec=%p n=%d op=%d (0 sum, 1 min, 2 max) comm=%p", (void *)vec, n, op, rccl_comm);
    if (c->capturing) return fail(c, LPF_ERR_STATE, "lpf_allreduce_metrics inside graph capture");
    typedef int (*allreduce_fn)(const void *, void *, size_t, int, int, void *, hipStream_t);
    typedef const char *(*errstr_fn)(int);
    static allreduce_fn p_allreduce = nullptr;
    static errstr_fn p_errstr = nullptr;
    static std::once_flag once;
    std::call_once(once, [] {
        void *h = nullptr;
        void *sym = dlsym(RTLD_DEFAULT, "ncclAllReduce");
        if (!sym) {
            for (const char *name : {"librccl.so", "librccl.so.1"}) {
// ... 136 lines not shown
    if ((rc = reserve(c, D.mwords, n * LW * 4))) return rc;
    if ((rc = reserve(c, D.mpts, n * 16))) return rc;
    if ((rc = reserve(c, D.cnt, nMB * 4))) return rc;
    W.flags = (uint32_t *)D.flags.p; W.chunk_cnt = (int2 *)D.ccnt.p; W.chunk_pre = (int2 *)D.cpre.p; W.fcnt = (int2 *)D.fcnt.p;
    W.m_idx = (int *)D.midx.p; W.m_words = (uint32_t *)D.mwords.p; W.m_pts = (float4 *)D.mpts.p; W.cnt = (unsigned *)D.cnt.p;
    return LPF_OK;
}

static int run_wide_impl(lpf_ctx *c, const char *who, const float *pts, const int64_t *frame_off, int F, int pts_on_device,
                         const PlaneSource &src, const lpf_wide_outputs *out, bool direct)
{
    int rc;
    const int M = src.M;
    const int64_t Ntot = frame_off[F];
    if (out->inst_idx && out->inst_cap <= 0) return fail(c, LPF_ERR_ARG, "%s: inst_idx given with inst_cap=%lld", who, (long long)out->inst_cap);
    lpf_ctx::BoxSet &BX = c->boxes.in_force();
    if (BX.F != 0 && BX.F != F) return fail(c, LPF_ERR_STATE, "boxes were set for %d frames, %s has %d", BX.F, who, F);
    if ((rc = flush_pending(c))) return rc;
    c->boxes.claimed_by_run();
    if ((rc = launch_box_job(c, BX))) return rc;

    const int LW = (M + 31) / 32;
    const int Btot = BX.total();
    const bool host_io = !out->on_device;
    const size_t n = (size_t)Ntot;
    lpf_ctx::Wide &D = c->wide;

    std::vector<LpfWideFrame> fr((size_t)F);
    int nbw = 0;
    const int nchunk = wide_frames(frame_off, F, BX, fr.data(), &nbw);
    if ((rc = reserve(c, D.tab, (size_t)F * sizeof(LpfWideFrame)))) return rc;
    if ((rc = upload(c, D.tab.p, fr.data(), (size_t)F * sizeof(LpfWideFrame)))) return rc;

    LpfWideParams W;
    wide_params(W, ctx_cam(c), F, M, nchunk, nbw, BX, out->inst_cap, (const LpfWideFrame *)D.tab.p);

    bool pts_in = false, masks_in = false;
    if ((rc = host_points(c, D.pts, pts, pts_on_device != 0, 0, n, n, &W.pts, &pts_in))) return rc;
    if (direct) W.planes = nullptr;
    else if ((rc = wide_pack(c, D, src, F, c->W, c->H, &W.planes, &masks_in))) return rc;

    const size_t nMB = (size_t)M * Btot;
    Stage S;
    if ((rc = wide_bind(c, D, out, n, F, Btot, W, S))) return rc;

    if (nchunk > 0) {
        if (direct)
            hipLaunchKernelGGL(lpf_wide_direct_project, dim3((unsigned)nchunk), dim3(LPF_BLOCK), 0, c->stream, W, (const uint8_t *)src.dense->masks,
                               (const int4 *)src.dense->rects);
        else
            hipLaunchKernelGGL(lpf_wide_project, dim3((unsigned)nchunk), dim3(LPF_BLOCK), 0, c->stream, W);
        LPF_HIP(c, hipGetLastError());
    }
    hipLaunchKernelGGL(lpf_wide_scan, dim3((unsigned)F), dim3(LPF_BLOCK), 0, c->stream, W);
    LPF_HIP(c, hipGetLastError());
    if (nchunk > 0) {
        hipLaunchKernelGGL(lpf_wide_scatter, dim3((unsigned)nchunk), dim3(LPF_BLOCK), 0, c->stream, W);
        LPF_HIP(c, hipGetLastError());
    }
    hipLaunchKernelGGL(lpf_wide_lists, dim3((unsigned)(F * std::max(LW, 1))), dim3(LPF_BLOCK), 0, c->stream, W);
    LPF_HIP(c, hipGetLastError());
    if (M > 0) {
        if (nMB > 0) {
            LPF_HIP(c, hipMemsetAsync(D.cnt.p, 0, nMB * 4, c->stream));
            hipLaunchKernelGGL(lpf_wide_boxes, dim3((unsigned)(F * LW * W.nbw), LPF_WIDE_PARTS), dim3(LPF_BLOCK), 0, c->stream, W);
            LPF_HIP(c, hipGetLastError());
        }
        hipLaunchKernelGGL(lpf_wide_best, dim3((unsigned)F), dim3(LPF_BLOCK), 0, c->stream, W);
        LPF_HIP(c, hipGetLastError());
    }

    if (host_io && (rc = S.back(c))) return rc;
    if (host_io || masks_in || pts_in) LPF_HIP(c, host_wait(c));
    if (direct) ++c->stats[7];
    return LPF_OK;
}

static int run_wide_input(lpf_ctx *c, const float *pts, const int64_t *frame_off, int F, int pts_on_device, const lpf_wide_input *in,
                          const lpf_wide_outputs *out, bool direct)
{
    int rc;
    const char *who = "run_wide";
    if ((rc = enter(c, "lpf_run_wide", true))) return rc;
    if (!in || !out || !frame_off || F <= 0) return fail(c, LPF_ERR_ARG, "%s: in=%p out=%p frame_off=%p F=%d", who, (const void *)in, (const void *)out, (const void *)frame_off, F);
    if ((rc = check_wide_input(c, who, -1, *in, LPF_MAX_MASKS_WIDE, "lpf_run_wide takes 0 .. LPF_MAX_MASKS_WIDE", "", true))) return rc;
    if ((rc = check_frames(c, who, pts, frame_off, F, LPF_WIDE_CHUNK))) return rc;
    lpf_ctx::RleIn &R = c->rle_in[0];
    if ((rc = check_wide_rle(c, who, -1, *in, F, (long long)c->W * c->H, R))) return rc;
    return run_wide_impl(c, who, pts, frame_off, F, pts_on_device, PlaneSource(*in, R), out, direct);
}

int lpf_run_wide(lpf_ctx *c, const float *pts, const int64_t *frame_off, int F, int pts_on_device, const lpf_wide_input *in,
                 const lpf_wide_outputs *out)
{
    return run_wide_input(c, pts, frame_off, F, pts_on_device, in, out, false);
}

int lpf_run_wide_ids(lpf_ctx *c, const float *pts, const int64_t *frame_off, int F, int pts_on_device, const lpf_id_masks *in,
                     const lpf_wide_outputs *out)
{
    int rc;
    const char *who = "run_wide_ids";
    if ((rc = enter(c, "lpf_run_wide_ids", true))) return rc;
    if (!in) return fail(c, LPF_ERR_ARG, "run_wide_ids: in=NULL");
    if (in->M > LPF_MAX_MASKS_WIDE)
        return fail(c, LPF_ERR_ARG, "run_wide_ids: M=%d masks per frame, lpf_run_wide_ids takes 0 .. LPF_MAX_MASKS_WIDE = %d", in->M, LPF_MAX_MASKS_WIDE);
    if ((rc = check_ids(c, who, in, (size_t)c->W * c->H))) return rc;
    if (in->F != F) return fail(c, LPF_ERR_ARG, "run_wide_ids: the ID maps say F=%d, the call has F=%d", in->F, F);
    if (!out || !frame_off || F <= 0) return fail(c, LPF_ERR_ARG, "%s: in=%p out=%p frame_off=%p F=%d", who, (const void *)in, (const void *)out, (const void *)frame_off, F);
    if ((rc = check_frames(c, who, pts, frame_off, F, LPF_WIDE_CHUNK))) return rc;
    return run_wide_impl(c, who, pts, frame_off, F, pts_on_device, PlaneSource(*in), out, false);
}


static void dm_raster(lpf_ctx *c, const LpfDmParams &P, dim3 g, bool planes, const lpf_wide_input *in, bool scatter)
{
    with_flag(scatter, [&](auto sc) {
        constexpr bool S = decltype(sc)::value;
        if (planes) hipLaunchKernelGGL((lpf_dm_raster<uint32_t, 0, true, S>), g, dim3(LPF_BLOCK), 0, c->stream, P);
        else with_rule(in->f32 != 0, in->binarize + 1, [&](auto kind) {
            hipLaunchKernelGGL((lpf_dm_raster<typename decltype(kind)::elem, decltype(kind)::rule, false, S>), g, dim3(LPF_BLOCK), 0, c->stream, P);
        });
    });
}

static int depth_maps_impl(lpf_ctx *c, const char *who, const float *pts, const int64_t *frame_off, int F, int pts_on_device,
                           const lpf_wide_input *in, const lpf_rle_masks *rle, const lpf_depth_maps_outputs *out)
{
    int rc;
    const int M = in->M;
    if (out->cap < 0 || !out->car_off || !out->need || (out->cap > 0 && !out->pix))
        return fail(c, LPF_ERR_ARG, "%s: cap=%lld pix=%p car_off=%p need=%p (car_off and need are required, pix with cap > 0)", who,
                    (long long)out->cap, (void *)out->pix, (void *)out->car_off, (void *)out->need);
    if (F == 0) return LPF_OK;
    if ((rc = check_frames(c, who, pts, frame_off, F, LPF_BLOCK))) return rc;
    RleCall R(c);
    if (rle && (rc = R.walk(who, rle, c->W, c->H))) return rc;
    const bool runs = R.active();
    long long maxN = 0;
    for (int f = 0; f < F; ++f) maxN = std::max(maxN, (long long)(frame_off[f + 1] - frame_off[f]));
    const int64_t Ntot = frame_off[F];
    if ((rc = flush_pending(c))) return rc;

    lpf_ctx::DepthMaps &D = c->dmaps;
    const size_t hw = (size_t)c->W * c->H, esz = in->f32 ? 4 : 1;
    const int ntile = (int)((hw + LPF_DM_TILE - 1) / LPF_DM_TILE), LW = (M + 31) / 32;
    const size_t hwp = (size_t)ntile * LPF_DM_TILE;
    const bool planes = M > 0 && (runs || in->erode_iters > 0);
    const bool host_masks = M > 0 && !runs && !in->on_device, host_pts = Ntot > 0 && !pts_on_device, host_io = !out->on_device;
    const bool use_rects = M > 0 && !runs && rects_hold(*in);
    const size_t plane_sets = in->erode_iters > (runs ? 0 : 1) ? 2 : 1;
    const size_t per_frame = hwp * 4 + (size_t)M * ntile * 12 + (planes ? (size_t)LW * hw * 4 * plane_sets : 0) +
                             (host_masks ? (size_t)M * (hw * esz + 16) : 0) + (host_pts ? (size_t)maxN * 16 : 0);
    const std::vector<Span> chunks = plan_ranges(c, (size_t)F, (size_t)F, [&](size_t f0, size_t n) {
        return n * per_frame + R.bytes(f0, n);
    });
    const size_t Fc = largest(chunks, [](size_t, size_t n) { return n; });
    const size_t most_pts = largest(chunks, [&](size_t f0, size_t n) { return frame_off[f0 + n] - frame_off[f0]; });

    if ((rc = reserve(c, D.foff, (size_t)(F + 1) * 8))) return rc;
    if ((rc = reserve(c, D.win, Fc * hwp * 4))) return rc;
    if (M > 0 && (rc = reserve(c, D.cnt, Fc * M * (2 * ntile + 1) * 4))) return rc;
    if (host_pts && (rc = reserve(c, D.pts, most_pts * 16))) return rc;
    if (runs && (rc = R.reserve_ranges(D.pack, chunks))) return rc;
    const void *masks_k = nullptr;
    const int32_t *rects_k = nullptr;
    Stage I(host_masks);
    I.add(masks_k, M > 0 && !runs ? in->masks : nullptr, (size_t)M * hw * esz, Fc);
    I.add(rects_k, M > 0 && !runs ? in->rects : nullptr, (size_t)M * 16, Fc);
    if ((rc = I.commit(c, D.in))) return rc;
    const size_t cap = (size_t)out->cap, nF = (size_t)F;
    if ((rc = upload(c, D.foff.p, frame_off, (size_t)(F + 1) * 8))) return rc;

    LpfDmParams P;
    memset(&P, 0, sizeof P);
    set_cam(P.cam, ctx_cam(c));
    P.M = M; P.LW = LW; P.ntile = ntile; P.hwp = (long long)hwp; P.cap = out->cap;
    P.foff = (const long long *)D.foff.p;
    P.win = (unsigned *)D.win.p;
    P.cnt = (unsigned *)D.cnt.p;
    P.toff = P.cnt + Fc * M * ntile;
    P.tot = P.toff + Fc * M * ntile;
    const bool lists = cap > 0 || !host_io;
    Stage S(host_io);
    S.add(P.pix, lists ? out->pix : nullptr, 8, nF * cap);
    S.add(P.depth, lists ? out->depth : nullptr, 8, nF * cap);
// ... 710 lines not shown
        if (nc == 0) P.pts = nullptr;
        if (M > 0) {
            if ((rc = I.in(c, {{r.first, r.count}, {r.first, r.count}}))) return rc;
            P.masks = host_masks || runs ? masks_k : masks_k + r.first * nM * plane * esz;
            P.colors = host_in || !colors_k ? colors_k : colors_k + r.first * nM * 3;
            const uint32_t *decoded = nullptr;
            if (runs && (rc = R.pack(D.pack, k, &decoded, &runs_in))) return rc;
            if (runs) P.masks = decoded;
        }
        const Span sp = {(size_t)a, (size_t)nc}, sf = {r.first, r.count}, none = {0, 0};
        if (host_io && lists && (rc = S.in(c, {none, sp, sp, sp, sp, sp, sp, none, none, none, none}))) return rc;
        if (P.mask_count && M > 0)
            LPF_HIP(c, hipMemsetAsync(P.mask_count + (size_t)(f0 - P.fr_base) * nM, 0, (size_t)fc * nM * 8, c->stream));
        const dim3 g((unsigned)((mc + LPF_FM_TILE - 1) / LPF_FM_TILE), (unsigned)fc);
        if (mc > 0) {
            if (rle) hipLaunchKernelGGL(lpf_fm_count_planes, g, dim3(LPF_BLOCK), 0, c->stream, P);
            else with_flag(in->f32 != 0, [&](auto f32) {
                typedef typename std::conditional<decltype(f32)::value, float, uint8_t>::type T;
                hipLaunchKernelGGL(lpf_fm_count<T>, g, dim3(LPF_BLOCK), 0, c->stream, P);
            });
            LPF_HIP(c, hipGetLastError());
        }
        hipLaunchKernelGGL(lpf_fm_scan, dim3((unsigned)fc), dim3(LPF_BLOCK), 0, c->stream, P);
        LPF_HIP(c, hipGetLastError());
        if (mc > 0 && lists) {
            hipLaunchKernelGGL(lpf_fm_scatter, g, dim3(LPF_BLOCK), 0, c->stream, P);
            LPF_HIP(c, hipGetLastError());
        }
        if (host_io && (rc = S.back(c, {sp, sp, sp, sp, sp, sp, sp, sf, sf, sf, {r.first * nM, r.count * nM}}))) return rc;
    }
    if (host_io || host_in || pts_in || runs_in) LPF_HIP(c, host_wait(c));
    return LPF_OK;
}

int lpf_first_match(lpf_ctx *c, const float *pts, const int64_t *frame_off, int F, int pts_on_device, const lpf_first_match_input *in,
                    const lpf_first_match_outputs *out)
{
    int rc;
    if ((rc = enter(c, "lpf_first_match", true))) return rc;
    if (!in || !out || F < 0 || !frame_off)
        return fail(c, LPF_ERR_ARG, "first_match: in=%p out=%p frame_off=%p F=%d", (const void *)in, (const void *)out, (const void *)frame_off, F);
    const int M = in->M;
    if (M < 0 || M > LPF_MAX_MASKS_WIDE)
        return fail(c, LPF_ERR_ARG, "first_match: M=%d masks per frame, lpf_first_match takes 0 .. LPF_MAX_MASKS_WIDE = %d", M, LPF_MAX_MASKS_WIDE);
    if (in->f32 != LPF_MASKS_U8 && in->f32 != LPF_MASKS_F32)
        return fail(c, LPF_ERR_ARG, "first_match: f32=%d (LPF_MASKS_U8 = 0 or LPF_MASKS_F32 = 1: lpf_first_match takes dense masks only)", in->f32);
    if (M > 0 && (!in->masks || in->mh <= 0 || in->mw <= 0))
        return fail(c, LPF_ERR_ARG, "first_match: masks=%p mh=%d mw=%d (with M > 0 masks is required and mh, mw are > 0)", in->masks, in->mh, in->mw);
    return first_match_impl(c, "first_match", pts, frame_off, F, pts_on_device, in, nullptr, out);
}

int lpf_first_match_rle(lpf_ctx *c, const float *pts, const int64_t *frame_off, int F, int pts_on_device,
                        const lpf_first_match_rle_input *in, const lpf_first_match_outputs *out)
{
    int rc;
    if ((rc = enter(c, "lpf_first_match_rle", true))) return rc;
    if (!in || !in->masks || !out || F < 0 || !frame_off)
        return fail(c, LPF_ERR_ARG, "first_match_rle: in=%p masks=%p out=%p frame_off=%p F=%d", (const void *)in,
                    (const void *)(in ? in->masks : nullptr), (const void *)out, (const void *)frame_off, F);
    const lpf_rle_masks *masks = in->masks;
    const int M = masks->M;
    if (masks->F != F) return fail(c, LPF_ERR_ARG, "first_match_rle: the run-length masks say F=%d, the call has F=%d", masks->F, F);
    if (M < 0 || M > LPF_MAX_MASKS_WIDE)
        return fail(c, LPF_ERR_ARG, "first_match_rle: M=%d masks per frame, lpf_first_match_rle takes 0 .. LPF_MAX_MASKS_WIDE = %d", M,
                    LPF_MAX_MASKS_WIDE);
    if (masks->erode_iters != 0)
        return fail(c, LPF_ERR_ARG, "first_match_rle: erode_iters=%d (the first-mask labelling has no erosion: 0)", masks->erode_iters);
    if (in->reserved != 0 || masks->reserved != 0)
        return fail(c, LPF_ERR_ARG, "first_match_rle: reserved=%d, the masks' reserved=%d (both 0)", in->reserved, masks->reserved);
    if (M > 0 && (in->mh <= 0 || in->mw <= 0))
        return fail(c, LPF_ERR_ARG, "first_match_rle: mh=%d mw=%d (with M > 0 both are > 0)", in->mh, in->mw);
    lpf_first_match_input fin;
    memset(&fin, 0, sizeof fin);
    fin.colors = in->colors; fin.M = M; fin.mh = in->mh; fin.mw = in->mw; fin.on_device = in->colors_on_device;
    return first_match_impl(c, "first_match_rle", pts, frame_off, F, pts_on_device, &fin, masks, out);
}

static int cams_check(lpf_ctx *c, const char *who, const float *pts, const int64_t *frame_off, int F, const lpf_cam_input *cams, int C,
                      const void *out, int64_t slack, int max_M, const char *takes, const char *more)
{
    const char *w = who + 4;
    int rc;
    if ((rc = enter(c, who, false))) return rc;
    if (C < 1 || C > LPF_MAX_CAMS) return fail(c, LPF_ERR_ARG, "%s: C=%d cameras, a pass takes 1 .. LPF_MAX_CAMS = %d", w, C, LPF_MAX_CAMS);
    if (!cams || !out || !frame_off || F <= 0)
        return fail(c, LPF_ERR_ARG, "%s: cams=%p out=%p frame_off=%p F=%d", w, (const void *)cams, out, (const void *)frame_off, F);
    if ((rc = check_frames(c, w, pts, frame_off, F, slack))) return rc;
    for (int k = 0; k < C; ++k) {
        const lpf_cam_input &I = cams[k];
        if (I.W <= 0 || I.H <= 0 || (long long)I.W * I.H > (1ll << 30))
            return fail(c, LPF_ERR_ARG, "%s: camera %d is %d x %d", w, k, I.W, I.H);
        if ((rc = check_wide_input(c, w, k, I.masks, max_M, takes, more, true))) return rc;
        if ((rc = check_wide_rle(c, w, k, I.masks, F, (long long)I.W * I.H, c->rle_in[k]))) return rc;
        if (I.corners_velo) {
            if (!I.box_off || I.box_off[0] != 0) return fail(c, LPF_ERR_ARG, "%s: camera %d: box_off must be given and start at 0", w, k);
            for (int f = 0; f < F; ++f)
                if (I.box_off[f + 1] < I.box_off[f]) return fail(c, LPF_ERR_ARG, "%s: camera %d: box_off not ascending at %d", w, k, f);
            if (I.boxes_on_device < 0 || I.boxes_on_device > 2) return fail(c, LPF_ERR_ARG, "%s: camera %d: boxes_on_device=%d", w, k, I.boxes_on_device);
        }
    }
    return LPF_OK;
}

static int cams_box_tables(lpf_ctx *c, const lpf_cam_input &I, int k, int F)
{
    int rc;
    lpf_ctx::BoxSet &B = c->cams.bx[k];
    B.clear();
    if (!I.corners_velo) return LPF_OK;
    if ((rc = box_shape(c, B, I.box_off, F, I.oriented))) return rc;
    const size_t nb = (size_t)B.total();
    if (nb == 0) return LPF_OK;
    const double *src;
    if ((rc = stage_corners(c, B, I.corners_velo, I.boxes_on_device, nb, &src))) { B.clear(); return rc; }
    B.new_job(src);
    return launch_box_job(c, B, I.K, I.W, I.H);
}

static_assert(LPF_MAX_CAMS == LPF_MAX_CAMS_DEV && LPF_MAX_CAMS <= LPF_NSETS, "a scratch set per camera");

int lpf_run_cams(lpf_ctx *c, const float *pts, const int64_t *frame_off, int F, int pts_on_device, const lpf_cam_input *cams, int C,
                 const lpf_outputs *out)
{
    int rc;
    if ((rc = cams_check(c, "lpf_run_cams", pts, frame_off, F, cams, C, out, LPF_SEG_QUANTUM, LPF_MAX_MASKS, "a pass takes 0 .. LPF_MAX_MASKS",
                         " per camera (more: lpf_run_wide for that camera)")))
        return rc;
    const int64_t Ntot = frame_off[F];
    for (int k = 0; k < C; ++k) {
        if (out[k].inst_idx && out[k].inst_cap <= 0) return fail(c, LPF_ERR_ARG, "run_cams: out[%d].inst_idx given with inst_cap=%lld", k, (long long)out[k].inst_cap);
        if ((out[k].uv_valid || out[k].label_valid) && !out[k].valid_idx)
            return fail(c, LPF_ERR_ARG, "run_cams: out[%d]: uv_valid / label_valid need valid_idx as well (they share its order)", k);
    }
    if ((rc = flush_pending(c))) return rc;
    const size_t n = (size_t)Ntot;
    bool host_in = false;

    const float4 *d_pts;
    if ((rc = host_points(c, c->cams.pts, pts, pts_on_device != 0, 0, n, n, &d_pts, &host_in))) return rc;

    int lb_all = 1;
    for (int k = 0; k < C; ++k) { const int M = cams[k].masks.M; lb_all = std::max(lb_all, M <= 8 ? 1 : M <= 16 ? 2 : 4); }
    const void *label_img[LPF_MAX_CAMS] = {nullptr, nullptr, nullptr, nullptr};
    for (int k = 0; k < C; ++k) {
        const lpf_cam_input &I = cams[k];
        if ((rc = cams_box_tables(c, I, k, F))) return rc;
        const lpf_wide_input &m = I.masks;
        if (m.M == 0) continue;
        const size_t hw = (size_t)I.W * I.H;
        const lpf_ctx::RleIn &R = c->rle_in[k];
        if (R.in) {
            void *cur = nullptr;
            if ((rc = rle_label_image(c, c->cams.label_a[k], c->cams.label_b[k], c->cams.rle[k], R, I.W, I.H, lb_all, &cur, &host_in))) return rc;
            label_img[k] = cur;
            continue;
        }
        const void *d_masks = nullptr;
        const int4 *rects = nullptr;
        if ((rc = stage_masks(c, m, F, hw, c->cams.masks[k], c->cams.rects[k], &d_masks, &rects, &host_in))) return rc;
        if (I.W < 16) rects = nullptr;
        if ((rc = reserve(c, c->cams.label_a[k], (size_t)F * hw * 4))) return rc;
        DevBuf &la = c->cams.label_a[k], &lb2 = c->cams.label_b[k];
        void *cur = nullptr;
        const int mode = m.f32 ? m.binarize + 1 : 0;
        rc = pack_masks(c, la, lb2, I.W, I.H, c->stream, d_masks, m.f32 != 0, mode, lb_all, F, m.M, m.erode_iters, &cur, rects);
        if (rc) return rc;
// ... 89 lines not shown
            return fail(c, LPF_ERR_ARG, "run_cams_wide: out[%d].inst_idx given with inst_cap=%lld", k, (long long)out[k].inst_cap);
    if ((rc = flush_pending(c))) return rc;
    const size_t n = (size_t)frame_off[F];
    bool host_in = false;

    const float4 *d_pts;
    if ((rc = host_points(c, c->camsw.pts, pts, pts_on_device != 0, 0, n, n, &d_pts, &host_in))) return rc;

    std::vector<LpfWideFrame> fr((size_t)C * F);
    int nchunk = 0, Btot[LPF_MAX_CAMS] = {0, 0, 0, 0}, nbw[LPF_MAX_CAMS] = {0, 0, 0, 0};
    for (int k = 0; k < C; ++k) {
        if ((rc = cams_box_tables(c, cams[k], k, F))) return rc;
        const lpf_ctx::BoxSet &BX = c->cams.bx[k];
        Btot[k] = BX.total();
        nchunk = wide_frames(frame_off, F, BX, fr.data() + (size_t)k * F, &nbw[k]);
    }
    if ((rc = reserve(c, c->camsw.tab, fr.size() * sizeof(LpfWideFrame)))) return rc;
    if ((rc = upload(c, c->camsw.tab.p, fr.data(), fr.size() * sizeof(LpfWideFrame)))) return rc;

    LpfCamsWideArgs A;
    memset(&A, 0, sizeof A);
    A.C = C;
    Stage S[LPF_MAX_CAMS];
    int max_lists = 0, max_boxes = 0;
    bool any_boxes = false, any_host = false;
    for (int k = 0; k < C; ++k) {
        const lpf_cam_input &I = cams[k];
        const lpf_ctx::BoxSet &BX = c->cams.bx[k];
        lpf_ctx::Wide &D = c->camsw.cam[k];
        LpfWideParams &W = A.P[k];
        const int M = I.masks.M, LW = (M + 31) / 32;
        wide_params(W, input_cam(I), F, M, nchunk, nbw[k], BX, out[k].inst_cap, (const LpfWideFrame *)c->camsw.tab.p + (size_t)k * F);
        W.pts = d_pts;
        if ((rc = wide_pack(c, D, PlaneSource(I.masks, c->rle_in[k]), F, I.W, I.H, &W.planes, &host_in))) return rc;
        if ((rc = wide_bind(c, D, &out[k], n, F, Btot[k], W, S[k]))) return rc;
        max_lists = std::max(max_lists, F * std::max(LW, 1));
        if (M > 0 && Btot[k] > 0) {
            any_boxes = true;
            max_boxes = std::max(max_boxes, F * LW * nbw[k]);
        }
        any_host |= !out[k].on_device;
    }

    if (nchunk > 0) {
        hipLaunchKernelGGL(lpf_cams_wide_project, dim3((unsigned)nchunk), dim3(LPF_BLOCK), 0, c->stream, A);
        LPF_HIP(c, hipGetLastError());
    }
    hipLaunchKernelGGL(lpf_cams_wide_scan, dim3((unsigned)F, (unsigned)C), dim3(LPF_BLOCK), 0, c->stream, A);
    LPF_HIP(c, hipGetLastError());
    if (nchunk > 0) {
        hipLaunchKernelGGL(lpf_cams_wide_scatter, dim3((unsigned)nchunk, (unsigned)C), dim3(LPF_BLOCK), 0, c->stream, A);
        LPF_HIP(c, hipGetLastError());
    }
    hipLaunchKernelGGL(lpf_cams_wide_lists, dim3((unsigned)max_lists, (unsigned)C), dim3(LPF_BLOCK), 0, c->stream, A);
    LPF_HIP(c, hipGetLastError());
    if (any_boxes) {
        for (int k = 0; k < C; ++k)
            if (A.P[k].M > 0 && Btot[k] > 0) LPF_HIP(c, hipMemsetAsync(A.P[k].cnt, 0, (size_t)A.P[k].M * Btot[k] * 4, c->stream));
        hipLaunchKernelGGL(lpf_cams_wide_boxes, dim3((unsigned)max_boxes, LPF_WIDE_PARTS, (unsigned)C), dim3(LPF_BLOCK), 0, c->stream, A);
        LPF_HIP(c, hipGetLastError());
    }
    bool any_masks = false;
    for (int k = 0; k < C; ++k) any_masks |= A.P[k].M > 0;
    if (any_masks) {
        hipLaunchKernelGGL(lpf_cams_wide_best, dim3((unsigned)F, (unsigned)C), dim3(LPF_BLOCK), 0, c->stream, A);
        LPF_HIP(c, hipGetLastError());
    }

    for (int k = 0; k < C; ++k)
        if (!out[k].on_device && (rc = S[k].back(c))) return rc;
    if (any_host || host_in) LPF_HIP(c, host_wait(c));
    return LPF_OK;
}

int lpf_run(lpf_ctx *c, const float *pts, int64_t N, int pts_on_device, const lpf_outputs *out)
{
    const int64_t off[2] = {0, N};
    return lpf_run_batch(c, pts, off, 1, pts_on_device, out);
}

int lpf_run_frame(lpf_ctx *c, const lpf_frame_job *j)
{
    if (!c) return LPF_ERR_ARG;
    if (!j) return fail(c, LPF_ERR_ARG, "lpf_run_frame: job is NULL");
    if (!j->out.on_device) return fail(c, LPF_ERR_ARG, "lpf_run_frame: device-mode outputs only (out.on_device = 1)");
    if (j->n_masks < 0 || j->n_boxes < 0) return fail(c, LPF_ERR_ARG, "lpf_run_frame: n_masks=%d n_boxes=%d", j->n_masks, j->n_boxes);
    int rc;
    if (j->masks) {
        if (j->mask_rects && (rc = lpf_set_mask_rects(c, j->mask_rects, 1, 1, j->n_masks))) return rc;
        if ((rc = lpf_set_masks_u8(c, j->masks, 1, j->n_masks, 0, 2))) return rc;
    }
    if (j->corners_cam0) {
        const int32_t boff[2] = {0, j->n_boxes};
        if ((rc = lpf_set_boxes_cam0(c, j->corners_cam0, 2, boff, 1, j->T_cam_to_velo, j->filter_visible, j->oriented, nullptr, nullptr, nullptr, nullptr)))
            return rc;
    }
    return lpf_run(c, j->pts, j->n_points, 1, &j->out);
}

#define LPF_FW_DIRECT_MAX 48
int lpf_run_frame_wide(lpf_ctx *c, const lpf_frame_job_wide *j)
{
    if (!c) return LPF_ERR_ARG;
    if (!j) return fail(c, LPF_ERR_ARG, "lpf_run_frame_wide: job is NULL");
    if (c->capturing) return fail(c, LPF_ERR_STATE, "lpf_run_frame_wide cannot be captured into a graph (call it outside lpf_graph_begin ... lpf_graph_end)");
    if (j->out.on_device != 1) return fail(c, LPF_ERR_ARG, "lpf_run_frame_wide: device-mode outputs only (out.on_device = 1)");
    if (j->n_masks < 0 || j->n_masks > LPF_MAX_MASKS_WIDE || j->n_boxes < 0)
        return fail(c, LPF_ERR_ARG, "lpf_run_frame_wide: n_masks=%d (0 .. LPF_MAX_MASKS_WIDE = %d) n_boxes=%d", j->n_masks, LPF_MAX_MASKS_WIDE,
                    j->n_boxes);
    if (j->n_masks > 0 && !j->masks) return fail(c, LPF_ERR_ARG, "lpf_run_frame_wide: masks is NULL with n_masks=%d", j->n_masks);
    if (!c->have_camera) return fail(c, LPF_ERR_STATE, "lpf_set_camera has not been called");
    int rc;
    if (j->corners_cam0) {
        const int32_t boff[2] = {0, j->n_boxes};
        if ((rc = lpf_set_boxes_cam0(c, j->corners_cam0, 2, boff, 1, j->T_cam_to_velo, j->filter_visible, j->oriented, nullptr, nullptr, nullptr, nullptr)))
            return rc;
    }
    lpf_wide_input in;
    memset(&in, 0, sizeof in);
    in.masks = j->masks;
    in.rects = j->mask_rects;
    in.M = j->n_masks;
    in.on_device = 2;
    const int64_t off[2] = {0, j->n_points};
    const bool direct = j->mask_rects && ((uintptr_t)j->mask_rects & 15) == 0 && j->n_masks > 0 && j->n_masks <= LPF_FW_DIRECT_MAX &&
                        2 * j->n_points <= (int64_t)c->W * c->H;
    return run_wide_input(c, j->pts, off, 1, 1, &in, &j->out, direct);
}

}

#include "lpf_reader.hip.h"
```

lidar_object_detection_amd/pipeline.py:

```python
import contextlib
import io
import os
import sys
from datetime import datetime

import numpy as np

from . import _native, kitti360
from ._native import LpfContext, LPF_MAX_CAMS, LPF_MAX_MASKS, LPF_MAX_MASKS_WIDE, Scan, ScanReader
from .idmap import IdMasks
from .rle import RleMasks

_CONTEXTS = {}


def get_context(device=0):
    ctx = _CONTEXTS.get(device)
    if ctx is None:
        ctx = _CONTEXTS[device] = LpfContext(device)
    return ctx


def _erosion_kernel_size(k):
    if isinstance(k, bool) or not isinstance(k, (int, np.integer)) or not 1 <= k <= 15 or k % 2 == 0:
        raise ValueError("erosion_kernel_size must be an odd integer from 1 to 15 (the k x k MORPH_ELLIPSE element), got %r" % (k,))
    return int(k)


def _f32_points(points, what="points"):
    p = np.asarray(points)
    if p.dtype == np.float32:
        return np.ascontiguousarray(p)
    q = np.ascontiguousarray(p, dtype=np.float32)
    if not np.array_equal(q.astype(np.float64), np.asarray(p, dtype=np.float64), equal_nan=True):
        raise TypeError("%s must hold float32-representable values (velodyne .bin format)" % what)
    return q


def _is_device_tensor(x):
    return type(x).__module__.startswith("torch") and getattr(x, "is_cuda", False)


def _mask_stack(masks, camera, resize_ctx=None, erode_iters=0, v3_pipeline=False, force_chain=False, erosion_kernel_size=3):
    erosion_kernel_size = _erosion_kernel_size(erosion_kernel_size)

    def chain(m):
        if resize_ctx is None:
            raise NotImplementedError("masks must already be %dx%d (retina_masks=True, V3:64) in this call" % (camera.height, camera.width))
        if not (erode_iters or v3_pipeline):
            return resize_ctx.resize_masks(m), False
        resize_ctx.set_erosion_element(erosion_kernel_size)
        dev = _is_device_tensor(m)
        if dev:
            import torch
            f = m.to(torch.float32)
            u8 = (f * 255).to(torch.uint8) if v3_pipeline else f.to(torch.uint8)
            er = resize_ctx.erode_masks(u8.contiguous(), erode_iters)
            back = (er == 255).to(torch.uint8) if v3_pipeline else er
        else:
            f = np.asarray(m)
            u8 = (f.astype(np.float32) * 255).astype(np.uint8) if v3_pipeline else f.astype(np.uint8)
            er = resize_ctx.erode_masks(u8, erode_iters)
            back = (er.astype(np.float32) / 255.0).astype(np.uint8) if v3_pipeline else er
        return resize_ctx.resize_masks(back), True
    if _is_device_tensor(masks):
        import torch
        if masks.ndim != 3:
            raise ValueError("device masks must be [M,h,w]")
        if tuple(masks.shape[1:]) != (camera.height, camera.width) or (force_chain and masks.shape[0]):
            return chain(masks)
        if masks.dtype == torch.bool:
            masks = masks.to(torch.uint8)
        elif masks.dtype not in (torch.float32, torch.uint8):
            masks = masks.to(torch.float32)
        return masks.contiguous(), False
    m = np.asarray(masks)
    if m.size == 0:
        return np.zeros((0, camera.height, camera.width), np.uint8), False
    if m.ndim != 3:
        raise ValueError("masks must be [M,h,w]")
    if m.shape[1:] != (camera.height, camera.width) or force_chain:
        return chain(m)
# ... 1610 lines not shown

def recall_rows(results, timestamp=None):
    rows = []
    for r in results:
        for row, s in zip(csv_rows(r["car_statistics"], r["frame"], timestamp), r["car_statistics"]):
            row["bbox_lidar_points"] = s["bbox_lidar_points"]
            row["recall_percentage"] = round(s["recall_percentage"], 2)
            rows.append(row)
    return rows


def _n_points(points):
    return len(points.points) if isinstance(points, Scan) else int(points.shape[0])


def run_frames_multicam(frames_per_cam, cams, depth_max=50.0, min_points=10, use_oriented=True, erode_iters=0, v3_pipeline=False,
                        device=0, ctx=None, gather_scans=True, erosion_kernel_size=3):
    erosion_kernel_size = _erosion_kernel_size(erosion_kernel_size)
    C = len(cams)
    if not 1 <= C <= LPF_MAX_CAMS:
        raise ValueError("run_frames_multicam takes 1 to %d cameras, got %d" % (LPF_MAX_CAMS, C))
    if len(frames_per_cam) != C:
        raise ValueError("frames for %d cameras, %d cameras given" % (len(frames_per_cam), C))
    F = len(frames_per_cam[0])
    for c, fs in enumerate(frames_per_cam):
        if len(fs) != F:
            raise ValueError("camera %d has %d frames, camera 0 has %d" % (c, len(fs), F))
        for i, (f, f0) in enumerate(zip(fs, frames_per_cam[0])):
            if f.frame != f0.frame or _n_points(f.points) != _n_points(f0.points):
                raise ValueError("frame %d of camera %d (frame %r, %d points) is not camera 0's (frame %r, %d points): every camera "
                                 "labels the same scans" % (i, c, f.frame, _n_points(f.points), f0.frame, _n_points(f0.points)))
    if F == 0:
        return [[] for _ in range(C)]
    ctx = ctx or get_context(device)
    ctx.set_erosion_element(erosion_kernel_size)
    results = [None] * C
    passes = []
    for c, (T, camera) in enumerate(cams):
        compact = _compact_frame_masks(frames_per_cam[c], camera, ("rle",))
        if compact is not None:
            rles = compact[1]
            counts = [r.shape[0] for r in rles]
            if max(counts) > LPF_MAX_MASKS:
                results[c] = run_frames(frames_per_cam[c], T, camera, depth_max, min_points, use_oriented, erode_iters, v3_pipeline, device,
                                        ctx, gather_scans, erosion_kernel_size)
            else:
                passes.append((c, rles, counts, max(counts), erode_iters, False))
            continue
        ctx.set_camera(T, camera.K, camera.width, camera.height, 0.0, float(depth_max))
        stacks, er, v3 = _frame_mask_stacks(frames_per_cam[c], camera, ctx, erode_iters, v3_pipeline, erosion_kernel_size)
        counts = [s.shape[0] for s in stacks]
        if max(counts) > LPF_MAX_MASKS:
            results[c] = run_frames(frames_per_cam[c], T, camera, depth_max, min_points, use_oriented, erode_iters, v3_pipeline, device,
                                    ctx, gather_scans, erosion_kernel_size)
            continue
        passes.append((c, stacks, counts, max(counts), er, v3))
    if not passes:
        return results
    specs, positions = [], []
    for c, stacks, counts, M, er, v3 in passes:
        T, camera = cams[c]
        corners, pos = zip(*(_corners_velo(f.bboxes_3d) for f in frames_per_cam[c]))
        positions.append(pos)
        specs.append(dict(T_velo_to_rect=T, K=camera.K, width=camera.width, height=camera.height, depth_min=0.0, depth_max=float(depth_max),
                          masks=stacks if isinstance(stacks[0], RleMasks) else _mask_batch(stacks, M, camera.height, camera.width, ctx),
                          binarize="v3" if v3 else "astype",
                          erode_iters=er, boxes=list(corners), oriented=use_oriented))
    pts = [f.points for f in frames_per_cam[passes[0][0]]]
    res = ctx.run_cams(pts, specs, want_uv=False, want_label=False, want_valid_uv=True, pinned=True)
    for (c, stacks, counts, M, er, v3), rc, pos in zip(passes, res, positions):
        results[c] = [_frame_result(f, r, m, p, min_points, gather_scans) for f, r, m, p in zip(frames_per_cam[c], rc, counts, pos)]
    return results


def stream_frames(scan_paths, inputs_for, TrVeloToRect, camera, depth_max=50.0, min_points=10, use_oriented=True,
                  erode_iters=0, v3_pipeline=False, device=0, n_buffers=3, max_points=None, box_paths=None, announce=None, gather=True,
                  erosion_kernel_size=3):
    erosion_kernel_size = _erosion_kernel_size(erosion_kernel_size)
    scan_paths = [os.fspath(p) for p in scan_paths]
    if max_points is None:
        sizes = [os.path.getsize(p) // 16 for p in scan_paths if os.path.isfile(p)]
        max_points = max(sizes + [1])
    ctx = get_context(device)
    with ScanReader(ctx, scan_paths, n_buffers=n_buffers, max_points=max_points, box_paths=box_paths) as reader:
        for i, path in enumerate(scan_paths):
            if announce is not None:
                announce(i, path)
            inputs = inputs_for(i, path) if box_paths is None else None
            try:
                scan = next(reader)
            except RuntimeError as e:
                print(f"Failed to load frame {os.path.basename(path)}: {e}")
                continue
            if box_paths is not None:
                inputs = inputs_for(i, path, scan)
            if inputs is None:
                continue
            frame_id, masks, boxes, colors = inputs
            yield run_frames([FrameInputs(frame_id, scan, masks, boxes, colors)], TrVeloToRect, camera, depth_max,
                             min_points, use_oriented, erode_iters, v3_pipeline, device, ctx, gather_scans=gather,
                             erosion_kernel_size=erosion_kernel_size)[0]


def sequence_setup(kitti360_path, seq=0, cam_id=0):
    sequence = "2013_05_28_drive_%04d_sync" % seq
    camera = kitti360.CameraPerspective(kitti360_path, sequence, cam_id)
    velo_to_cam, velo_to_rect = kitti360.velo_to_rect_transforms(kitti360_path, camera, cam_id)
    velo = kitti360.Kitti360Viewer3DRaw(seq=seq, root_dir=kitti360_path)
    return sequence, camera, velo_to_cam, velo_to_rect, velo


def _boxes_of_file(json_path, camera, velo_to_cam, keep_all=False, parsed=None):
    state, index, corners = parsed if parsed is not None else _native.parse_boxes_file(json_path)
    if state == _native.BOXES_PARSED:
        return prepare_boxes_from_arrays(index, corners, camera, velo_to_cam, keep_all=keep_all) if len(index) else None
    raw = kitti360.load_bounding_boxes(json_path)
    if not raw:
        return None
    return prepare_boxes(raw, camera, velo_to_cam, keep_all=keep_all, as_arrays=True)


def collect_frame_inputs(kitti360_path, seq, cam_id, segmenter, image_loader, camera, velo_to_cam, velo, frames=None,
                         keep_all_boxes=False, boxes_as_arrays=False):
    return list(iter_frame_inputs(kitti360_path, seq, cam_id, segmenter, image_loader, camera, velo_to_cam, velo, frames,
                                  keep_all_boxes, boxes_as_arrays))


def _batches(items, n):
    batch = []
    for it in items:
        batch.append(it)
        if len(batch) >= n:
            yield batch
            batch = []
    if batch:
        yield batch


def iter_frame_inputs(kitti360_path, seq, cam_id, segmenter, image_loader, camera, velo_to_cam, velo, frames=None,
                      keep_all_boxes=False, boxes_as_arrays=False):
    sequence = "2013_05_28_drive_%04d_sync" % seq
    bbox_dir = os.path.join(kitti360_path, "bboxes_3D_cam0")
    todo = velo.available_frames() if frames is None else list(frames)
    print(f"Found {len(todo)} frames to process")
    for frame in todo:
        print(f"\nProcessing frame {frame}...")
        try:
            points = velo.loadVelodyneData(frame)
        except Exception as e:
            print(f"Failed to load frame {frame}: {e}")
            continue
        if boxes_as_arrays:
            boxes = _boxes_of_file(os.path.join(bbox_dir, f"BBoxes_{frame}.json"), camera, velo_to_cam, keep_all_boxes)
            if boxes is None:
                continue
        else:
            raw = kitti360.load_bounding_boxes(os.path.join(bbox_dir, f"BBoxes_{frame}.json"))
            if not raw:
                continue
            boxes = prepare_boxes(raw, camera, velo_to_cam, keep_all=keep_all_boxes)
        image_path = os.path.join(kitti360_path, "data_2d_raw", sequence, f"image_{cam_id:02d}",
                                  "data_rect" if cam_id in [0, 1] else "data_rgb", f"{frame:010d}.png")
        if not os.path.isfile(image_path):
            continue
        seg = segmenter(image_loader(image_path) if image_loader else image_path)
        _, masks, colors, boxes_2d, _ = seg
        if masks is None or len(masks) == 0:
            continue
        yield FrameInputs(frame, points, masks, boxes, colors, boxes_2d)


def process_frames(seq=0, cam_id=0, segmenter=None, image_loader=None, kitti360_path=None,
                   master_csv_path="results/master_car_statistics.csv", frames=None, batch_frames=32,
                   erode_iters=0, v3_pipeline=False, device=0, timestamp=None, read_ahead=True, erosion_kernel_size=3):
    erosion_kernel_size = _erosion_kernel_size(erosion_kernel_size)
    if segmenter is None:
        raise ValueError("process_frames needs the segmentation callable (YOLO stays outside this package)")
    root = kitti360_path or os.environ["KITTI360_DATASET"]
    sequence, camera, velo_to_cam, velo_to_rect, velo = sequence_setup(root, seq, cam_id)
    if read_ahead:
        todo = velo.available_frames() if frames is None else list(frames)
        print(f"Found {len(todo)} frames to process")

        box_paths = [os.path.join(root, "bboxes_3D_cam0", f"BBoxes_{f}.json") for f in todo]
# ... 309 lines not shown
```

Before: 172.1 billion.

## Add asynchronous frame submit/collect API and pipeline stream_frames two deep

Adds lpf_frame_submit/poll/collect with two in-flight frame slots, host mask staging on a worker thread, and per-slot completion events. stream_frames keeps one frame in flight while preparing the next, so host-side work (mask packing, Python result building) overlaps GPU execution instead of synchronizing every frame. The ScanReader gains a keep parameter so scan buffers stay alive while their frames are in flight. The cost is extra slot buffers, added state checks on every setter, and a resubmit path when the instance list overflows.

```diff
diff --git a/include/lpf.h b/include/lpf.h
--- a/include/lpf.h
+++ b/include/lpf.h
@@ -429,6 +429,31 @@
 int  lpf_reader_boxes(lpf_reader *rd, const double **corners_cam0, const int32_t **index, int *nbox, int *state);
 int  lpf_parse_boxes_json(const char *path, double *corners_cam0, int32_t *index, int cap, int *nbox, int *state);
 
+#define LPF_FRAME_SLOTS 2
+typedef struct lpf_frame_extra {
+    const void   *masks;
+    const double *corners_velo;
+    int32_t       masks_where;
+    int32_t       f32;
+    int32_t       binarize;
+    int32_t       erode_iters;
+    int32_t       reserved;
+    int32_t       reserved2;
+} lpf_frame_extra;
+typedef struct lpf_frame_views {
+    const lpf_frame_summary *summary;
+    const int64_t  *valid_idx;
+    const int32_t  *uv_valid;
+    const uint32_t *label_valid;
+    const int64_t  *inst_idx;
+    const int32_t  *count_mb;
+    int64_t         n_points, inst_cap;
+    int32_t         n_masks, n_boxes;
+} lpf_frame_views;
+int lpf_frame_submit(lpf_ctx *ctx, const lpf_frame_job *job, const lpf_frame_extra *x, int64_t *ticket);
+int lpf_frame_collect(lpf_ctx *ctx, int64_t ticket, lpf_frame_views *views);
+int lpf_frame_poll(lpf_ctx *ctx, int64_t ticket, int *done);
+
 #ifdef __cplusplus
 }
 #endif
diff --git a/lidar_object_detection_amd/_build.py b/lidar_object_detection_amd/_build.py
--- a/lidar_object_detection_amd/_build.py
+++ b/lidar_object_detection_amd/_build.py
@@ -10,7 +10,7 @@
 SOURCES = ("lpf_api.hip", "lpf_kernels.hip.h", "lpf_reader.hip.h", "lpf_wide.hip.h", "lpf_cams.hip.h", "lpf_cams_wide.hip.h",
            "lpf_frame_wide.hip.h", "lpf_depth_maps.hip.h", "lpf_depth_overlays.hip.h",
            "lpf_match2d.hip.h", "lpf_inside.hip.h", "lpf_box_points.hip.h", "lpf_box_views.hip.h", "lpf_assign.hip.h",
-           "lpf_first_match.hip.h", "lpf_rle.hip.h", "lpf_ids.hip.h")
+           "lpf_first_match.hip.h", "lpf_rle.hip.h", "lpf_ids.hip.h", "lpf_async.hip.h")
 ARCH = "gfx950"
 
 FLAGS = ["--offload-arch=" + ARCH, "-O3", "-std=c++17", "-fPIC", "-shared", "-pthread", "-ldl",
diff --git a/lidar_object_detection_amd/_native.py b/lidar_object_detection_amd/_native.py
--- a/lidar_object_detection_amd/_native.py
+++ b/lidar_object_detection_amd/_native.py
@@ -318,6 +318,19 @@
     _fields_ = [("pts", _P), ("n_points", _I64), ("masks", _P), ("mask_rects", _P), ("corners_cam0", _P), ("T_cam_to_velo", _P),
                 ("n_masks", ctypes.c_int32), ("n_boxes", ctypes.c_int32), ("filter_visible", ctypes.c_int32), ("oriented", ctypes.c_int32),
                 ("out", WideOutputs)]
+
+
+LPF_FRAME_SLOTS = 2
+
+
+class FrameExtra(ctypes.Structure):
+    _fields_ = [("masks", _P), ("corners_velo", _P), ("masks_where", ctypes.c_int32), ("f32", ctypes.c_int32), ("binarize", ctypes.c_int32),
+                ("erode_iters", ctypes.c_int32), ("reserved", ctypes.c_int32), ("reserved2", ctypes.c_int32)]
+
+
+class FrameViews(ctypes.Structure):
+    _fields_ = [("summary", _P), ("valid_idx", _P), ("uv_valid", _P), ("label_valid", _P), ("inst_idx", _P), ("count_mb", _P),
+                ("n_points", _I64), ("inst_cap", _I64), ("n_masks", ctypes.c_int32), ("n_boxes", ctypes.c_int32)]
 
 
 _libs = {}
@@ -446,6 +459,9 @@
     lib.lpf_reader_wait.argtypes = [_P]
     lib.lpf_reader_destroy.argtypes = [_P]
     lib.lpf_reader_destroy.restype = None
+    lib.lpf_frame_submit.argtypes = [_P, ctypes.POINTER(FrameJob), ctypes.POINTER(FrameExtra), ctypes.POINTER(_I64)]
+    lib.lpf_frame_collect.argtypes = [_P, _I64, ctypes.POINTER(FrameViews)]
+    lib.lpf_frame_poll.argtypes = [_P, _I64, ctypes.POINTER(ctypes.c_int)]
     _libs[path] = lib
     return lib
 
@@ -461,7 +477,8 @@
             "lpf_reader_submit_frame", "lpf_reader_boxes", "lpf_parse_boxes_json", "lpf_run_wide", "lpf_run_cams",
             "lpf_run_cams_wide", "lpf_run_frame_wide", "lpf_depth_maps", "lpf_depth_overlays", "lpf_match_2d",
             "lpf_inside_masks", "lpf_set_erosion_element", "lpf_box_points", "lpf_box_views", "lpf_assign_costs", "lpf_assign_2d",
-            "lpf_first_match", "lpf_set_masks_rle", "lpf_depth_maps_rle", "lpf_first_match_rle", "lpf_set_masks_ids", "lpf_run_wide_ids")
+            "lpf_first_match", "lpf_set_masks_rle", "lpf_depth_maps_rle", "lpf_first_match_rle", "lpf_set_masks_ids", "lpf_run_wide_ids",
+            "lpf_frame_submit", "lpf_frame_collect", "lpf_frame_poll")
 
 BOXES_PARSED, BOXES_ABSENT, BOXES_OTHER, BOXES_NONE = 0, 1, 2, 3
 
@@ -507,20 +524,24 @@
 
 
 class Scan:
-    __slots__ = ("path", "n", "points", "dev_ptr", "_reader", "_ticket", "boxes_state", "box_index", "boxes_cam0")
+    __slots__ = ("path", "n", "points", "dev_ptr", "_reader", "_ticket", "boxes_state", "box_index", "boxes_cam0", "_released")
 
     def __init__(self, path, n, points, dev_ptr, reader, ticket, boxes_state=BOXES_NONE, box_index=None, boxes_cam0=None):
         self.path, self.n, self.points, self.dev_ptr, self._reader, self._ticket = path, n, points, dev_ptr, reader, ticket
         self.boxes_state, self.box_index, self.boxes_cam0 = boxes_state, box_index, boxes_cam0
+        self._released = False
 
     def _check_live(self):
-        if self._reader._ticket != self._ticket or self._reader._h is None:
+        if self._released or not 0 <= self._reader._ticket - self._ticket <= self._reader._keep or self._reader._h is None:
             raise LpfError(-3, "this Scan's buffers were recycled (a later scan has been fetched from its reader)")
 
 
 class ScanReader:
 
-    def __init__(self, ctx, paths, n_buffers=3, max_points=1 << 21, box_paths=None):
+    def __init__(self, ctx, paths, n_buffers=3, max_points=1 << 21, box_paths=None, keep=0):
+        if int(keep) and not 0 < int(keep) <= int(n_buffers) - 2:
+            raise ValueError("keep=%d needs n_buffers >= keep + 2 (n_buffers=%d)" % (keep, n_buffers))
+        self._keep = int(keep)
         self._ctx, self._lib = ctx, ctx._lib
         self._h = None
         self._ticket = 0
@@ -530,7 +551,7 @@
             raise ValueError("box_paths: one entry per scan")
         self._next_submit = 0
         self._delivered = 0
-        self._depth = int(n_buffers)
+        self._depth = int(n_buffers) if not self._keep else int(n_buffers) - 1 - self._keep
         h = _P()
         ctx._check(self._lib.lpf_reader_create(ctx._h, ctypes.byref(h), int(n_buffers), int(max_points)))
         self._h = h
@@ -619,6 +640,7 @@
         self._depth = 1
         self.erosion_kernel_size = 3
         self._pin = {}
+        self._frames = {}
         self._lent = collections.deque(maxlen=4)
 
     def _check(self, rc):
@@ -1147,6 +1169,91 @@
 
         out = self._until_lists_fit(launch, inst_cap, off)
         return self._frame_results(off, M, *out)
+
+    def frame_submit(self, points, masks=None, corners_velo=None, oriented=True, erode_iters=0, v3_pipeline=False, binarize=None,
+                     inst_cap=None):
+        if binarize is None:
+            binarize = "v3" if v3_pipeline else "astype"
+        if binarize not in self.BINARIZE:
+            raise ValueError("binarize must be one of %s" % sorted(self.BINARIZE))
+        job, x = FrameJob(), FrameExtra()
+        if isinstance(points, Scan):
+            points._check_live()
+            job.pts, n = (points.dev_ptr if points.n else None), points.n
+        elif _is_torch(points):
+            import torch
+            if points.ndim != 2 or points.shape[1] != 4:
+                raise ValueError("device points must be a float32 tensor [N,4]")
+            self.wait_for_stream(torch.cuda.current_stream(points.device).cuda_stream)
+            n = int(points.shape[0])
+            job.pts = _dev_ptr(points, "float32") if n else None
+        else:
+            raise ValueError("frame_submit takes a ScanReader's Scan or a float32 [N,4] GPU tensor (host points: run_batch)")
+        keep, M = None, 0
+        if masks is not None and not _is_torch(masks):
+            masks = np.asarray(masks)
+        if masks is not None and len(masks) and masks.ndim == 4 and masks.shape[0] == 1:
+            masks = masks[0]
+        if masks is not None and len(masks):
+            shape = tuple(masks.shape)
+            if len(shape) != 3 or shape[1:] != (self.H, self.W):
+                raise ValueError("masks must be [M,%d,%d], got %s" % (self.H, self.W, shape))
+            M = shape[0]
+            if _is_torch(masks):
+                is_f = str(masks.dtype) == "torch.float32"
+                if not is_f and str(masks.dtype) not in ("torch.uint8", "torch.bool"):
+                    raise ValueError("device masks must be float32, uint8 or bool")
+                keep, x.masks, x.masks_where = masks, _dev_ptr(masks), 1
+            else:
+                a = np.asarray(masks)
+                is_f = a.dtype.kind == "f"
+                keep = np.ascontiguousarray(a, dtype=np.float32 if is_f else np.uint8)
+                x.masks, x.masks_where = keep.ctypes.data, 0
+            _check_erode_iters(erode_iters)
+            x.f32, x.binarize, x.erode_iters = int(is_f), self.BINARIZE[binarize], int(erode_iters)
+        corners = None
+        if corners_velo is not None and len(corners_velo):
+            corners = np.ascontiguousarray(corners_velo, dtype=np.float64).reshape(-1, 8, 3)
+            x.corners_velo = corners.ctypes.data
+        B = 0 if corners is None else corners.shape[0]
+        job.n_points, job.n_masks, job.n_boxes, job.oriented = n, M, B, int(bool(oriented))
+        job.out.inst_cap = max(n, 1) if inst_cap is None else int(inst_cap)
+        t = _I64(0)
+        self._check(self._lib.lpf_frame_submit(self._h, ctypes.byref(job), ctypes.byref(x), ctypes.byref(t)))
+        self._frames[int(t.value)] = (points, keep)
+        self.F_masks = self.M = 0
+        self.box_off = np.array([0, B], np.int32)
+        return int(t.value)
+
+    def frame_done(self, ticket):
+        done = ctypes.c_int(0)
+        self._check(self._lib.lpf_frame_poll(self._h, int(ticket), ctypes.byref(done)))
+        return bool(done.value)
+
+    def frame_collect(self, ticket):
+        v = FrameViews()
+        rc = self._lib.lpf_frame_collect(self._h, int(ticket), ctypes.byref(v))
+        if rc != -3:
+            self._frames.pop(int(ticket), None)
+        self._check(rc)
+
+        def view(addr, dtype, count):
+            dt = np.dtype(dtype)
+            if not count or not addr:
+                return np.zeros(0, dt)
+            return np.frombuffer((ctypes.c_char * (count * dt.itemsize)).from_address(addr), dtype=dt)
+        s = view(v.summary, SUMMARY_DTYPE, 1)[0]
+        M, B, nv = int(v.n_masks), int(v.n_boxes), int(s["n_valid"])
+        uvv = view(v.uv_valid, np.int32, 2 * nv).reshape(nv, 2)
+        off = s["inst_off"].tolist()
+        cap = int(v.inst_cap)
+        iidx = view(v.inst_idx, np.int64, cap if M else 0)
+        return dict(n_valid=nv, n_labelled=int(s["n_labelled"]), inst_count=s["inst_count"][:M].copy(), best_box=s["best_box"][:M].copy(),
+                    best_cnt=s["best_cnt"][:M].copy(), valid_idx=view(v.valid_idx, np.int64, nv), uv_valid=uvv, u_valid=uvv[:, 0],
+                    v_valid=uvv[:, 1], label_valid=view(v.label_valid, np.uint32, nv),
+                    inst_lists=[iidx[min(off[m], cap):min(off[m + 1], cap)] for m in range(M)],
+                    count_mb=view(v.count_mb, np.int32, M * B).reshape(M, B).astype(np.int64),
+                    inst_overflow=bool(s["inst_overflow"]), inst_need=int(off[32]))
 
     _PER_POINT = {"uv": None, "label_bits": "label_bits", "label_words": "label_words", "depth": "depth", "u_f": "uf", "v_f": "vf"}
     _PER_VALID = ("valid_idx", "uv_valid", "label_valid", "label_valid_words")
diff --git a/lidar_object_detection_amd/csrc/lpf_api.hip b/lidar_object_detection_amd/csrc/lpf_api.hip
--- a/lidar_object_detection_amd/csrc/lpf_api.hip
+++ b/lidar_object_detection_amd/csrc/lpf_api.hip
@@ -69,8 +69,13 @@
 
 #define LPF_NSETS 4
 
+struct lpf_frames;
+
 struct lpf_ctx {
     bool capturing = false;
+    lpf_frames *frames = nullptr;
+    int frames_busy = 0;
+    bool frames_inside = false, frames_no_wait = false;
     unsigned long long generation = 0;
     int device = 0;
     hipStream_t stream = nullptr;
@@ -262,6 +267,15 @@
     return code;
 }
 
+#define LPF_NO_FRAMES_IN_FLIGHT(c, who)                                                                                        \
+    do {                                                                                                                       \
+        if ((c)->frames_busy && !(c)->frames_inside)                                                                           \
+            return fail((c), LPF_ERR_STATE, "%s: %d frame(s) of lpf_frame_submit in flight: lpf_frame_collect them first", (who), \
+                        (c)->frames_busy);                                                                                     \
+    } while (0)
+
+void frames_shutdown(lpf_ctx *c);
+
 #define LPF_HIP(c, call)                                                                         \
     do {                                                                                         \
         hipError_t e_ = (call);                                                                  \
@@ -833,6 +847,7 @@
                    int filter_visible, uint8_t *visible, double *corners_velo, double *bbox2d, int32_t *front, const char *who)
 {
     if (!c) return LPF_ERR_ARG;
+    LPF_NO_FRAMES_IN_FLIGHT(c, who);
     if (use_device(c)) return LPF_ERR_HIP;
     if (on_device < 0 || on_device > 2) return fail(c, LPF_ERR_ARG, "%s: on_device=%d (0 host, 1 device, 2 device and lent)", who, on_device);
     if (F == 0) { c->boxes.in_force().clear(); return LPF_OK; }
@@ -940,6 +955,7 @@
 int set_masks_impl(lpf_ctx *c, const T *masks, int F, int M, int mode, int erode_iters, int on_device)
 {
     if (!c) return LPF_ERR_ARG;
+    LPF_NO_FRAMES_IN_FLIGHT(c, "set_masks");
     if (use_device(c)) return LPF_ERR_HIP;
     if (!c->have_camera) return fail(c, LPF_ERR_STATE, "lpf_set_camera must be called before masks (W, H)");
     if (M > LPF_MAX_MASKS) return too_many_masks(c, M);
@@ -1676,6 +1692,7 @@
 {
     if (!c) return;
     (void)hipSetDevice(c->device);
+    frames_shutdown(c);
     (void)hipStreamSynchronize(c->stream);
     for (auto &S : c->sc) {
         DevBuf *sb[] = {&S.vbal, &S.mbal, &S.seg_tab, &S.grp_tab, &S.frm_tab, &S.seg_pre, &S.cnt, &S.mlist, &S.label_a, &S.label_b, &S.tab, &S.rects, &S.rgrid, &S.out_stage};
@@ -1722,6 +1739,7 @@
 int lpf_set_stream(lpf_ctx *c, void *s)
 {
     if (!c) return LPF_ERR_ARG;
+    LPF_NO_FRAMES_IN_FLIGHT(c, "lpf_set_stream");
     if (use_device(c)) return LPF_ERR_HIP;
     { int rc_ = sync_all(c); if (rc_) return rc_; }
     if (c->own_stream) { (void)hipStreamDestroy(c->stream); c->own_stream = false; }
@@ -1733,6 +1751,7 @@
 int lpf_use_own_stream(lpf_ctx *c)
 {
     if (!c) return LPF_ERR_ARG;
+    LPF_NO_FRAMES_IN_FLIGHT(c, "lpf_use_own_stream");
     if (use_device(c)) return LPF_ERR_HIP;
     { int rc_ = sync_all(c); if (rc_) return rc_; }
     if (c->own_stream) return LPF_OK;
@@ -1824,6 +1843,7 @@
 int lpf_set_mask_rects(lpf_ctx *c, const int32_t *rects, int on_device, int F, int M)
 {
     if (!c) return LPF_ERR_ARG;
+    LPF_NO_FRAMES_IN_FLIGHT(c, "lpf_set_mask_rects");
     c->rects_pending = nullptr; c->rects_F = 0; c->rects_M = 0;
     if (!rects || F <= 0 || M <= 0) return LPF_OK;
     if (M > LPF_MAX_MASKS) return fail(c, LPF_ERR_ARG, "lpf_set_mask_rects: M=%d (at most %d)", M, LPF_MAX_MASKS);
@@ -1849,6 +1869,7 @@
 int lpf_set_erosion_element(lpf_ctx *c, int ksize)
 {
     if (!c) return LPF_ERR_ARG;
+    LPF_NO_FRAMES_IN_FLIGHT(c, "lpf_set_erosion_element");
     if (ksize < 1 || ksize > 15 || ksize % 2 == 0)
         return fail(c, LPF_ERR_ARG, "lpf_set_erosion_element: ksize=%d (the k x k MORPH_ELLIPSE for odd k, 1 .. 15)", ksize);
     const int r = ksize / 2;
@@ -1861,6 +1882,7 @@
 int lpf_set_pipelined(lpf_ctx *c, int on)
 {
     if (!c) return LPF_ERR_ARG;
+    LPF_NO_FRAMES_IN_FLIGHT(c, "lpf_set_pipelined");
     if (use_device(c)) return LPF_ERR_HIP;
     if (on == 1 || on == 3)
         return fail(c, LPF_ERR_ARG, "lpf_set_pipelined: modes 1 and 3 (tail kernels / mask pack on side streams) were removed in ABI 5 -- "
@@ -1881,6 +1903,7 @@
 int lpf_set_camera(lpf_ctx *c, const double T[16], const double K[9], int W, int H, double dmin, double dmax)
 {
     if (!c) return LPF_ERR_ARG;
+    LPF_NO_FRAMES_IN_FLIGHT(c, "lpf_set_camera");
     if (!T || !K || W <= 0 || H <= 0 || (long long)W * H > (1ll << 30))
         return fail(c, LPF_ERR_ARG, "set_camera: T=%p K=%p W=%d H=%d", (const void *)T, (const void *)K, W, H);
     if (!c->capturing && (c->pipe.owes() || c->boxes.in_force().job_valid)) {
@@ -1914,6 +1937,7 @@
 int lpf_set_masks_rle(lpf_ctx *c, const lpf_rle_masks *in)
 {
     if (!c) return LPF_ERR_ARG;
+    LPF_NO_FRAMES_IN_FLIGHT(c, "lpf_set_masks_rle");
     if (use_device(c)) return LPF_ERR_HIP;
     if (!c->have_camera) return fail(c, LPF_ERR_STATE, "lpf_set_camera must be called before masks (W, H)");
     if (c->capturing)
@@ -1932,6 +1956,7 @@
 int lpf_set_masks_ids(lpf_ctx *c, const lpf_id_masks *in)
 {
     if (!c) return LPF_ERR_ARG;
+    LPF_NO_FRAMES_IN_FLIGHT(c, "lpf_set_masks_ids");
     if (use_device(c)) return LPF_ERR_HIP;
     if (!c->have_camera) return fail(c, LPF_ERR_STATE, "lpf_set_camera must be called before masks (W, H)");
     if (c->capturing)
@@ -1949,6 +1974,7 @@
 int lpf_set_label_image(lpf_ctx *c, const uint32_t *label, int F, int M, int on_device)
 {
     if (!c) return LPF_ERR_ARG;
+    LPF_NO_FRAMES_IN_FLIGHT(c, "lpf_set_label_image");
     if (use_device(c)) return LPF_ERR_HIP;
     if (!c->have_camera) return fail(c, LPF_ERR_STATE, "lpf_set_camera must be called first");
     if (F < 0 || M < 0 || M > LPF_MAX_MASKS || (F > 0 && !label)) return fail(c, LPF_ERR_ARG, "set_label_image: F=%d M=%d", F, M);
@@ -2010,6 +2036,7 @@
 int lpf_run_batch(lpf_ctx *c, const float *pts, const int64_t *frame_off, int F, int pts_on_device, const lpf_outputs *out)
 {
     if (!c) return LPF_ERR_ARG;
+    LPF_NO_FRAMES_IN_FLIGHT(c, "lpf_run_batch");
     if (use_device(c)) return LPF_ERR_HIP;
     if (!c->have_camera) return fail(c, LPF_ERR_STATE, "lpf_set_camera has not been called");
     if (!out || !frame_off || F <= 0) return fail(c, LPF_ERR_ARG, "run: out=%p frame_off=%p F=%d", (const void *)out, (const void *)frame_off, F);
@@ -2138,6 +2165,7 @@
         std::vector<lpf_frame_summary> hs((size_t)F);
         bool lists = false;
         if ((rc = narrow_back_a(c, *out, P, n, M * Btot, hs.data(), &lists))) return rc;
+        if (c->frames_no_wait && !lists) return LPF_OK;
         LPF_HIP(c, host_wait(c));
         if (lists) {
             if ((rc = narrow_back_b(c, *out, P, frame_off, hs.data()))) return rc;
@@ -2375,6 +2403,7 @@
 int lpf_graph_begin(lpf_ctx *c)
 {
     if (!c) return LPF_ERR_ARG;
+    LPF_NO_FRAMES_IN_FLIGHT(c, "lpf_graph_begin");
     if (use_device(c)) return LPF_ERR_HIP;
     if (c->pipe.fused) return fail(c, LPF_ERR_STATE, "graph capture needs pipelining off");
     if (c->capturing) return fail(c, LPF_ERR_STATE, "already capturing");
@@ -2677,6 +2706,7 @@
     int rc;
     const char *who = "run_wide";
     if ((rc = enter(c, "lpf_run_wide", true))) return rc;
+    LPF_NO_FRAMES_IN_FLIGHT(c, "lpf_run_wide");
     if (!in || !out || !frame_off || F <= 0) return fail(c, LPF_ERR_ARG, "%s: in=%p out=%p frame_off=%p F=%d", who, (const void *)in, (const void *)out, (const void *)frame_off, F);
     if ((rc = check_wide_input(c, who, -1, *in, LPF_MAX_MASKS_WIDE, "lpf_run_wide takes 0 .. LPF_MAX_MASKS_WIDE", "", true))) return rc;
     if ((rc = check_frames(c, who, pts, frame_off, F, LPF_WIDE_CHUNK))) return rc;
@@ -2697,6 +2727,7 @@
     int rc;
     const char *who = "run_wide_ids";
     if ((rc = enter(c, "lpf_run_wide_ids", true))) return rc;
+    LPF_NO_FRAMES_IN_FLIGHT(c, "lpf_run_wide_ids");
     if (!in) return fail(c, LPF_ERR_ARG, "run_wide_ids: in=NULL");
     if (in->M > LPF_MAX_MASKS_WIDE)
         return fail(c, LPF_ERR_ARG, "run_wide_ids: M=%d masks per frame, lpf_run_wide_ids takes 0 .. LPF_MAX_MASKS_WIDE = %d", in->M, LPF_MAX_MASKS_WIDE);
@@ -3573,6 +3604,7 @@
     const char *w = who + 4;
     int rc;
     if ((rc = enter(c, who, false))) return rc;
+    LPF_NO_FRAMES_IN_FLIGHT(c, who);
     if (C < 1 || C > LPF_MAX_CAMS) return fail(c, LPF_ERR_ARG, "%s: C=%d cameras, a pass takes 1 .. LPF_MAX_CAMS = %d", w, C, LPF_MAX_CAMS);
     if (!cams || !out || !frame_off || F <= 0)
         return fail(c, LPF_ERR_ARG, "%s: cams=%p out=%p frame_off=%p F=%d", w, (const void *)cams, out, (const void *)frame_off, F);
@@ -3828,6 +3860,7 @@
 int lpf_run_frame(lpf_ctx *c, const lpf_frame_job *j)
 {
     if (!c) return LPF_ERR_ARG;
+    LPF_NO_FRAMES_IN_FLIGHT(c, "lpf_run_frame");
     if (!j) return fail(c, LPF_ERR_ARG, "lpf_run_frame: job is NULL");
     if (!j->out.on_device) return fail(c, LPF_ERR_ARG, "lpf_run_frame: device-mode outputs only (out.on_device = 1)");
     if (j->n_masks < 0 || j->n_boxes < 0) return fail(c, LPF_ERR_ARG, "lpf_run_frame: n_masks=%d n_boxes=%d", j->n_masks, j->n_boxes);
@@ -3848,6 +3881,7 @@
 int lpf_run_frame_wide(lpf_ctx *c, const lpf_frame_job_wide *j)
 {
     if (!c) return LPF_ERR_ARG;
+    LPF_NO_FRAMES_IN_FLIGHT(c, "lpf_run_frame_wide");
     if (!j) return fail(c, LPF_ERR_ARG, "lpf_run_frame_wide: job is NULL");
     if (c->capturing) return fail(c, LPF_ERR_STATE, "lpf_run_frame_wide cannot be captured into a graph (call it outside lpf_graph_begin ... lpf_graph_end)");
     if (j->out.on_device != 1) return fail(c, LPF_ERR_ARG, "lpf_run_frame_wide: device-mode outputs only (out.on_device = 1)");
@@ -3877,3 +3911,4 @@
 }
 
 #include "lpf_reader.hip.h"
+#include "lpf_async.hip.h"
diff --git a/lidar_object_detection_amd/csrc/lpf_async.hip.h b/lidar_object_detection_amd/csrc/lpf_async.hip.h
--- /dev/null
+++ b/lidar_object_detection_amd/csrc/lpf_async.hip.h
@@ -0,0 +1,340 @@
+#pragma once
+
+#include <condition_variable>
+#include <deque>
+#include <mutex>
+#include <thread>
+
+static_assert(LPF_FRAME_SLOTS >= 1 && LPF_FRAME_SLOTS <= 4, "a small ring: at most four frames in flight");
+
+struct lpf_frames {
+    struct Slot {
+        enum State { FREE, STAGING, QUEUED, FAILED } state = FREE;
+        int64_t ticket = 0;
+        lpf_frame_job job;
+        lpf_frame_extra x;
+        bool host_masks = false, dev_masks = false;
+        std::vector<double> corners;
+        double Tcv[16];
+        int64_t inst_cap = 0;
+        int status = LPF_OK;
+        std::string err;
+        const void *src = nullptr;
+        size_t mask_bytes = 0;
+        void *d_masks = nullptr; size_t d_cap = 0;
+        hipEvent_t copied = nullptr, done = nullptr;
+        bool staged = false;
+        int w_status = LPF_OK;
+        std::string w_err;
+        struct Pin { void *p = nullptr; size_t cap = 0; } summary, valid_idx, uv_valid, label_valid, inst_idx, count_mb;
+    } slots[LPF_FRAME_SLOTS];
+    int64_t next_ticket = 1, next_collect = 1, next_queue = 1;
+    hipStream_t copy_stream = nullptr;
+    std::thread worker;
+    std::mutex mu;
+    std::condition_variable cv;
+    std::deque<int> posted;
+    bool stop = false;
+};
+
+namespace {
+
+lpf_frames::Slot &frame_slot(lpf_frames *A, int64_t ticket) { return A->slots[(size_t)(ticket % LPF_FRAME_SLOTS)]; }
+
+void frames_worker(lpf_frames *A, int device)
+{
+    (void)hipSetDevice(device);
+    for (;;) {
+        int s;
+        {
+            std::unique_lock<std::mutex> lk(A->mu);
+            A->cv.wait(lk, [A] { return A->stop || !A->posted.empty(); });
+            if (A->stop) return;
+            s = A->posted.front(); A->posted.pop_front();
+        }
+        lpf_frames::Slot &S = A->slots[s];
+        hipError_t e = hipMemcpyAsync(S.d_masks, S.src, S.mask_bytes, hipMemcpyHostToDevice, A->copy_stream);
+        if (e == hipSuccess) e = hipEventRecord(S.copied, A->copy_stream);
+        {
+            std::lock_guard<std::mutex> lk(A->mu);
+            if (e != hipSuccess) { S.w_status = LPF_ERR_HIP; S.w_err = std::string("lpf_frame_submit: the copy of the masks failed: ") + hipGetErrorString(e); }
+            S.staged = true;
+        }
+        A->cv.notify_all();
+    }
+}
+
+int frames_state(lpf_ctx *c)
+{
+    if (c->frames) return LPF_OK;
+    lpf_frames *A = new (std::nothrow) lpf_frames();
+    if (!A) return fail(c, LPF_ERR_NOMEM, "lpf_frame_submit: out of host memory");
+    hipError_t e = hipStreamCreateWithFlags(&A->copy_stream, hipStreamNonBlocking);
+    for (auto &S : A->slots) {
+        if (e == hipSuccess) e = hipEventCreateWithFlags(&S.copied, hipEventDisableTiming);
+        if (e == hipSuccess) e = hipEventCreateWithFlags(&S.done, hipEventDisableTiming);
+    }
+    c->frames = A;
+    if (e != hipSuccess) return fail(c, LPF_ERR_HIP, "lpf_frame_submit: %s", hipGetErrorString(e));
+    return LPF_OK;
+}
+
+int frames_pin(lpf_ctx *c, lpf_frames::Slot::Pin &b, size_t bytes)
+{
+    if (bytes == 0) bytes = 8;
+    if (b.p && bytes <= b.cap) return LPF_OK;
+    if (b.p) { (void)hipHostFree(b.p); b.p = nullptr; b.cap = 0; }
+    const size_t want = bytes + bytes / 4;
+    if (hipHostMalloc(&b.p, want, hipHostMallocDefault) != hipSuccess) { b.p = nullptr; (void)hipGetLastError(); return fail(c, LPF_ERR_NOMEM, "lpf_frame_submit: hipHostMalloc(%zu) failed", want); }
+    b.cap = want;
+    return LPF_OK;
+}
+
+int frames_mask_buffer(lpf_ctx *c, lpf_frames::Slot &S, size_t bytes)
+{
+    if (!S.d_masks || bytes > S.d_cap) {
+        if (S.d_masks) { (void)hipFree(S.d_masks); S.d_masks = nullptr; S.d_cap = 0; }
+        const size_t want = bytes + bytes / 4;
+        if (hipMalloc(&S.d_masks, want) != hipSuccess) { S.d_masks = nullptr; (void)hipGetLastError(); return fail(c, LPF_ERR_NOMEM, "lpf_frame_submit: hipMalloc(%zu) failed", want); }
+        S.d_cap = want;
+    }
+    return LPF_OK;
+}
+
+int frames_queue(lpf_ctx *c, lpf_frames::Slot &S)
+{
+    const lpf_frame_job &j = S.job;
+    int rc = LPF_OK;
+    c->frames_inside = true;
+    c->frames_no_wait = true;
+    do {
+        if (S.host_masks) {
+            hipError_t e = hipStreamWaitEvent(c->stream, S.copied, 0);
+            if (e != hipSuccess) { rc = fail(c, LPF_ERR_HIP, "lpf_frame_submit: hipStreamWaitEvent: %s", hipGetErrorString(e)); break; }
+        }
+        if (S.host_masks || S.dev_masks) {
+            const void *m = S.host_masks ? S.d_masks : S.x.masks;
+            rc = S.x.f32 == LPF_MASKS_F32 ? lpf_set_masks_f32(c, (const float *)m, 1, j.n_masks, S.x.binarize, S.x.erode_iters, 2)
+                                          : lpf_set_masks_u8(c, (const uint8_t *)m, 1, j.n_masks, S.x.erode_iters, 2);
+        } else if (j.n_masks > 0) {
+            if (j.mask_rects && (rc = lpf_set_mask_rects(c, j.mask_rects, 1, 1, j.n_masks))) break;
+            rc = lpf_set_masks_u8(c, j.masks, 1, j.n_masks, 0, 2);
+        } else {
+            rc = lpf_set_masks_u8(c, nullptr, 0, 0, 0, 0);
+        }
+        if (rc) break;
+        const int32_t boff[2] = {0, j.n_boxes};
+        if (!S.corners.empty()) rc = lpf_set_boxes(c, S.corners.data(), boff, 1, j.oriented);
+        else if (j.corners_cam0 && j.n_boxes > 0)
+            rc = lpf_set_boxes_cam0(c, j.corners_cam0, 2, boff, 1, S.Tcv, j.filter_visible, j.oriented, nullptr, nullptr, nullptr, nullptr);
+        else rc = lpf_set_boxes(c, nullptr, boff, 1, j.oriented);
+        if (rc) break;
+        lpf_outputs o;
+        memset(&o, 0, sizeof o);
+        o.summary = (lpf_frame_summary *)S.summary.p;
+        o.valid_idx = (int64_t *)S.valid_idx.p;
+        o.uv_valid = (int32_t *)S.uv_valid.p;
+        o.label_valid = (uint32_t *)S.label_valid.p;
+        if (j.n_masks > 0) { o.inst_idx = (int64_t *)S.inst_idx.p; o.inst_cap = S.inst_cap; }
+        o.count_mb = (int32_t *)S.count_mb.p;
+        memset(S.summary.p, 0, sizeof(lpf_frame_summary));
+        memset(S.count_mb.p, 0, std::max((size_t)j.n_masks * (size_t)j.n_boxes, (size_t)1) * 4);
+        if ((rc = lpf_run(c, j.pts, j.n_points, 1, &o))) break;
+        hipError_t e = hipEventRecord(S.done, c->stream);
+        if (e != hipSuccess) rc = fail(c, LPF_ERR_HIP, "lpf_frame_submit: hipEventRecord: %s", hipGetErrorString(e));
+    } while (0);
+    c->masks.drop();
+    c->frames_no_wait = false;
+    c->frames_inside = false;
+    if (rc) { S.state = lpf_frames::Slot::FAILED; S.status = rc; S.err = c->err; }
+    else S.state = lpf_frames::Slot::QUEUED;
+    return rc;
+}
+
+void frames_pump(lpf_ctx *c, int64_t until)
+{
+    lpf_frames *A = c->frames;
+    while (A->next_queue < A->next_ticket) {
+        lpf_frames::Slot &S = frame_slot(A, A->next_queue);
+        if (S.state == lpf_frames::Slot::STAGING) {
+            if (S.host_masks) {
+                std::unique_lock<std::mutex> lk(A->mu);
+                if (!S.staged) {
+                    if (A->next_queue > until) return;
+                    A->cv.wait(lk, [&S] { return S.staged; });
+                }
+                if (S.w_status != LPF_OK) { S.state = lpf_frames::Slot::FAILED; S.status = S.w_status; S.err = S.w_err; }
+            }
+            if (S.state == lpf_frames::Slot::STAGING) (void)frames_queue(c, S);
+        }
+        ++A->next_queue;
+    }
+}
+
+void frames_shutdown(lpf_ctx *c)
+{
+    lpf_frames *A = c->frames;
+    if (!A) return;
+    {
+        std::lock_guard<std::mutex> lk(A->mu);
+        A->stop = true;
+    }
+    A->cv.notify_all();
+    if (A->worker.joinable()) A->worker.join();
+    if (A->copy_stream) (void)hipStreamSynchronize(A->copy_stream);
+    (void)hipStreamSynchronize(c->stream);
+    for (auto &S : A->slots) {
+        if (S.d_masks) (void)hipFree(S.d_masks);
+        if (S.copied) (void)hipEventDestroy(S.copied);
+        if (S.done) (void)hipEventDestroy(S.done);
+        for (lpf_frames::Slot::Pin *b : {&S.summary, &S.valid_idx, &S.uv_valid, &S.label_valid, &S.inst_idx, &S.count_mb})
+            if (b->p) (void)hipHostFree(b->p);
+    }
+    if (A->copy_stream) (void)hipStreamDestroy(A->copy_stream);
+    delete A;
+    c->frames = nullptr;
+    c->frames_busy = 0;
+}
+
+}
+
+extern "C" {
+
+int lpf_frame_submit(lpf_ctx *c, const lpf_frame_job *j, const lpf_frame_extra *x, int64_t *ticket)
+{
+    if (!c) return LPF_ERR_ARG;
+    if (!j || !ticket) return fail(c, LPF_ERR_ARG, "lpf_frame_submit: job=%p ticket=%p", (const void *)j, (const void *)ticket);
+    *ticket = 0;
+    if (use_device(c)) return LPF_ERR_HIP;
+    if (c->capturing) return fail(c, LPF_ERR_STATE, "lpf_frame_submit cannot be captured into a graph (call it outside lpf_graph_begin ... lpf_graph_end)");
+    if (!c->have_camera) return fail(c, LPF_ERR_STATE, "lpf_set_camera has not been called");
+    if (c->pipe.fused) return fail(c, LPF_ERR_STATE, "lpf_frame_submit: a software-pipelined mode is on (lpf_set_pipelined(ctx, 0) first): frames in flight run in order");
+    lpf_frame_extra none;
+    memset(&none, 0, sizeof none);
+    const lpf_frame_extra &X = x ? *x : none;
+    if (j->n_points < 0 || j->n_points > 0x7fffffffll - LPF_SEG_QUANTUM || (j->n_points > 0 && !j->pts))
+        return fail(c, LPF_ERR_ARG, "lpf_frame_submit: n_points=%lld pts=%p", (long long)j->n_points, (const void *)j->pts);
+    if (j->n_masks < 0 || j->n_masks > LPF_MAX_MASKS || j->n_boxes < 0)
+        return fail(c, LPF_ERR_ARG, "lpf_frame_submit: n_masks=%d (0 .. LPF_MAX_MASKS = %d) n_boxes=%d", j->n_masks, LPF_MAX_MASKS, j->n_boxes);
+    if ((X.f32 != LPF_MASKS_U8 && X.f32 != LPF_MASKS_F32) || (X.masks_where != 0 && X.masks_where != 1) || X.binarize < 0 || X.binarize > 2 ||
+        X.erode_iters < 0 || X.reserved != 0 || X.reserved2 != 0)
+        return fail(c, LPF_ERR_ARG, "lpf_frame_submit: f32=%d (LPF_MASKS_U8 / LPF_MASKS_F32) masks_where=%d (0 host, 1 device) binarize=%d (0 .. 2) "
+                                    "erode_iters=%d reserved=%d, %d", X.f32, X.masks_where, X.binarize, X.erode_iters, X.reserved, X.reserved2);
+    if (j->n_masks > 0 && !X.masks && !j->masks) return fail(c, LPF_ERR_ARG, "lpf_frame_submit: n_masks=%d and no masks", j->n_masks);
+    if (X.masks && j->mask_rects) return fail(c, LPF_ERR_ARG, "lpf_frame_submit: mask_rects go with job->masks, not with the extra masks");
+    if (j->n_boxes > 0 && !X.corners_velo && !j->corners_cam0) return fail(c, LPF_ERR_ARG, "lpf_frame_submit: n_boxes=%d and no corners", j->n_boxes);
+    if (j->n_boxes > 0 && !X.corners_velo && !j->T_cam_to_velo) return fail(c, LPF_ERR_ARG, "lpf_frame_submit: T_cam_to_velo is NULL");
+    int rc;
+    if ((rc = frames_state(c))) return rc;
+    lpf_frames *A = c->frames;
+    if (c->frames_busy >= LPF_FRAME_SLOTS)
+        return fail(c, LPF_ERR_STATE, "lpf_frame_submit: every slot is busy (%d frames in flight): lpf_frame_collect ticket %lld first", c->frames_busy,
+                    (long long)A->next_collect);
+    frames_pump(c, A->next_ticket - 1);
+    lpf_frames::Slot &S = frame_slot(A, A->next_ticket);
+    const size_t n = (size_t)j->n_points, hw = (size_t)c->H * c->W;
+    const int64_t cap = j->out.inst_cap > 0 ? j->out.inst_cap : std::max<int64_t>(j->n_points, 1);
+    const bool host_masks = X.masks && j->n_masks > 0 && X.masks_where == 0, dev_masks = X.masks && j->n_masks > 0 && X.masks_where == 1;
+    const size_t mask_bytes = (size_t)j->n_masks * hw * (X.f32 == LPF_MASKS_F32 ? 4 : 1);
+    if ((rc = frames_pin(c, S.summary, sizeof(lpf_frame_summary))) || (rc = frames_pin(c, S.valid_idx, n * 8)) || (rc = frames_pin(c, S.uv_valid, n * 8)) ||
+        (rc = frames_pin(c, S.label_valid, n * 4)) || (rc = frames_pin(c, S.inst_idx, j->n_masks > 0 ? (size_t)cap * 8 : 0)) ||
+        (rc = frames_pin(c, S.count_mb, std::max((size_t)j->n_masks * (size_t)j->n_boxes, (size_t)1) * 4)))
+        return rc;
+    if (host_masks && (rc = frames_mask_buffer(c, S, mask_bytes))) return rc;
+    if (host_masks && !A->worker.joinable()) A->worker = std::thread(frames_worker, A, c->device);
+    S.job = *j;
+    S.x = X;
+    S.host_masks = host_masks; S.dev_masks = dev_masks;
+    S.inst_cap = cap;
+    S.corners.clear();
+    if (X.corners_velo && j->n_boxes > 0) S.corners.assign(X.corners_velo, X.corners_velo + (size_t)j->n_boxes * 24);
+    if (j->T_cam_to_velo) memcpy(S.Tcv, j->T_cam_to_velo, sizeof S.Tcv);
+    S.status = LPF_OK; S.err.clear();
+    S.ticket = A->next_ticket;
+    S.state = lpf_frames::Slot::STAGING;
+    if (host_masks) {
+        {
+            std::lock_guard<std::mutex> lk(A->mu);
+            S.src = X.masks; S.mask_bytes = mask_bytes;
+            S.staged = false; S.w_status = LPF_OK; S.w_err.clear();
+            A->posted.push_back((int)(S.ticket % LPF_FRAME_SLOTS));
+        }
+        A->cv.notify_all();
+    }
+    ++A->next_ticket;
+    ++c->frames_busy;
+    frames_pump(c, host_masks ? S.ticket - 1 : S.ticket);
+    if (!host_masks && S.state == lpf_frames::Slot::FAILED) {
+        rc = S.status;
+        c->err = S.err;
+        S.state = lpf_frames::Slot::FREE;
+        --A->next_ticket; --A->next_queue; --c->frames_busy;
+        return rc;
+    }
+    *ticket = S.ticket;
+    return LPF_OK;
+}
+
+int lpf_frame_poll(lpf_ctx *c, int64_t ticket, int *done)
+{
+    if (!c) return LPF_ERR_ARG;
+    if (!done) return fail(c, LPF_ERR_ARG, "lpf_frame_poll: done is NULL");
+    *done = 0;
+    lpf_frames *A = c->frames;
+    if (!A || ticket < A->next_collect || ticket >= A->next_ticket)
+        return fail(c, LPF_ERR_STATE, "lpf_frame_poll: ticket %lld is not in flight", (long long)ticket);
+    if (use_device(c)) return LPF_ERR_HIP;
+    frames_pump(c, 0);
+    const lpf_frames::Slot &S = frame_slot(A, ticket);
+    if (S.state == lpf_frames::Slot::FAILED) *done = 1;
+    else if (S.state == lpf_frames::Slot::QUEUED) {
+        if (hipEventQuery(S.done) == hipSuccess) *done = 1;
+        else (void)hipGetLastError();
+    }
+    return LPF_OK;
+}
+
+int lpf_frame_collect(lpf_ctx *c, int64_t ticket, lpf_frame_views *v)
+{
+    if (!c) return LPF_ERR_ARG;
+    if (!v) return fail(c, LPF_ERR_ARG, "lpf_frame_collect: views is NULL");
+    memset(v, 0, sizeof *v);
+    lpf_frames *A = c->frames;
+    if (!A || ticket <= 0 || ticket >= A->next_ticket)
+        return fail(c, LPF_ERR_STATE, "lpf_frame_collect: ticket %lld was never handed out", (long long)ticket);
+    if (ticket < A->next_collect) return fail(c, LPF_ERR_STATE, "lpf_frame_collect: ticket %lld has been collected already", (long long)ticket);
+    if (ticket > A->next_collect)
+        return fail(c, LPF_ERR_STATE, "lpf_frame_collect: ticket %lld is out of order: ticket %lld is the oldest in flight", (long long)ticket,
+                    (long long)A->next_collect);
+    if (use_device(c)) return LPF_ERR_HIP;
+    frames_pump(c, ticket);
+    lpf_frames::Slot &S = frame_slot(A, ticket);
+    int rc = LPF_OK;
+    if (S.state == lpf_frames::Slot::FAILED) {
+        rc = S.status;
+        c->err = S.err;
+    } else {
+        if (hipEventQuery(S.done) != hipSuccess) {
+            (void)hipGetLastError();
+            ++c->stats[0];
+            const hipError_t e = hipEventSynchronize(S.done);
+            if (e != hipSuccess) rc = fail(c, LPF_ERR_HIP, "lpf_frame_collect: hipEventSynchronize: %s", hipGetErrorString(e));
+        }
+        if (!rc) {
+            v->summary = (const lpf_frame_summary *)S.summary.p;
+            v->valid_idx = (const int64_t *)S.valid_idx.p;
+            v->uv_valid = (const int32_t *)S.uv_valid.p;
+            v->label_valid = (const uint32_t *)S.label_valid.p;
+            v->inst_idx = S.job.n_masks > 0 ? (const int64_t *)S.inst_idx.p : nullptr;
+            v->count_mb = (const int32_t *)S.count_mb.p;
+            v->n_points = S.job.n_points; v->inst_cap = S.inst_cap;
+            v->n_masks = S.job.n_masks; v->n_boxes = S.job.n_boxes;
+        }
+    }
+    S.state = lpf_frames::Slot::FREE;
+    ++A->next_collect;
+    --c->frames_busy;
+    return rc;
+}
+
+}
diff --git a/lidar_object_detection_amd/pipeline.py b/lidar_object_detection_amd/pipeline.py
--- a/lidar_object_detection_amd/pipeline.py
+++ b/lidar_object_detection_amd/pipeline.py
@@ -1,3 +1,4 @@
+import collections
 import contextlib
 import io
 import os
@@ -1774,24 +1775,76 @@
         sizes = [os.path.getsize(p) // 16 for p in scan_paths if os.path.isfile(p)]
         max_points = max(sizes + [1])
     ctx = get_context(device)
-    with ScanReader(ctx, scan_paths, n_buffers=n_buffers, max_points=max_points, box_paths=box_paths) as reader:
-        for i, path in enumerate(scan_paths):
-            if announce is not None:
-                announce(i, path)
-            inputs = inputs_for(i, path) if box_paths is None else None
-            try:
-                scan = next(reader)
-            except RuntimeError as e:
-                print(f"Failed to load frame {os.path.basename(path)}: {e}")
-                continue
-            if box_paths is not None:
-                inputs = inputs_for(i, path, scan)
-            if inputs is None:
-                continue
-            frame_id, masks, boxes, colors = inputs
-            yield run_frames([FrameInputs(frame_id, scan, masks, boxes, colors)], TrVeloToRect, camera, depth_max,
-                             min_points, use_oriented, erode_iters, v3_pipeline, device, ctx, gather_scans=gather,
-                             erosion_kernel_size=erosion_kernel_size)[0]
+    ctx.set_erosion_element(erosion_kernel_size)
+    H, W = camera.height, camera.width
+    ctx.set_camera(TrVeloToRect, camera.K, W, H, 0.0, float(depth_max))
+    keep = _native.LPF_FRAME_SLOTS - 1
+    flight = collections.deque()
+
+    def submit(f, m, pos, args, inst_cap=None):
+        flight.append((ctx.frame_submit(*args, inst_cap=inst_cap), f, m, pos, args))
+
+    def collect():
+        t, f, m, pos, args = flight.popleft()
+        r = ctx.frame_collect(t)
+        if not r["inst_overflow"]:
+            return [(f, _frame_result(f, r, m, pos, min_points, gather))]
+        later = []
+        while flight:
+            later += collect()
+        submit(f, m, pos, args, inst_cap=r["inst_need"])
+        return collect() + later
+
+    last = [None]
+
+    def emit(pairs):
+        for f, r in pairs:
+            if last[0] is not None and last[0] is not f.points:
+                last[0]._released = True
+            last[0] = f.points
+            yield r
+
+    with ScanReader(ctx, scan_paths, n_buffers=n_buffers + keep, max_points=max_points, box_paths=box_paths, keep=keep) as reader:
+        try:
+            for i, path in enumerate(scan_paths):
+                if announce is not None:
+                    announce(i, path)
+                inputs = inputs_for(i, path) if box_paths is None else None
+                while flight and reader._ticket + 1 - flight[0][1].points._ticket > keep:
+                    yield from emit(collect())
+                try:
+                    scan = next(reader)
+                except RuntimeError as e:
+                    print(f"Failed to load frame {os.path.basename(path)}: {e}")
+                    continue
+                if box_paths is not None:
+                    inputs = inputs_for(i, path, scan)
+                if inputs is None:
+                    continue
+                frame_id, masks, boxes, colors = inputs
+                f = FrameInputs(frame_id, scan, masks, boxes, colors)
+                stacks = None
+                if _compact_frame_masks([f], camera, ("rle", "ids")) is None:
+                    stacks, er, v3 = _frame_mask_stacks([f], camera, ctx, erode_iters, v3_pipeline, erosion_kernel_size)
+                if stacks is None or stacks[0].shape[0] > LPF_MAX_MASKS:
+                    while flight:
+                        yield from emit(collect())
+                    yield from emit([(f, run_frames([f], TrVeloToRect, camera, depth_max, min_points, use_oriented, erode_iters, v3_pipeline,
+                                                    device, ctx, gather_scans=gather, erosion_kernel_size=erosion_kernel_size)[0])])
+                    continue
+                m = stacks[0].shape[0]
+                corners, pos = _corners_velo(f.bboxes_3d)
+                submit(f, m, pos, (scan, _mask_batch(stacks, m, H, W, ctx) if m else None, corners, use_oriented, er, v3))
+                while len(flight) > keep:
+                    yield from emit(collect())
+            while flight:
+                yield from emit(collect())
+        finally:
+            while flight:
+                try:
+                    ctx.frame_collect(flight.popleft()[0])
+                except _native.LpfError:
+                    pass
 
 
 def sequence_setup(kitti360_path, seq=0, cam_id=0):
```

New measurement: 171.0 billion. No clear change (-0.6%).
